# JinfengX/PointCloudPDF

Measured on AMD Instinct MI355X. Metric: points/sec fwd+bwd (PT-v1 Seg50 + PDF U-decoder, 100k-pt scenes), higher is better.
Workload: dtype f32

## Files before the change

include/pdfops.h:

```cpp
#ifndef PDFOPS_H
#define PDFOPS_H

#ifdef __cplusplus
extern "C" {
#endif

#define PDF_OK 0
#define PDF_ERR_BAD_ARG (-1)
#define PDF_ERR_NSAMPLE (-2)
#define PDF_ERR_UNSUPPORTED (-3)
#define PDF_ERR_NOT_CONVERGED (-4)

#define PDF_ABI_VERSION 18
int pdf_abi_version(void);
const char *pdf_build_info(void);
int pdf_dist_fma_mode(void);
#define PDF_MMA_F32 0
#define PDF_MMA_F16 1
#define PDF_MMA_BF16 2

int pdf_knn_query(int m, int nsample, const float *xyz, const float *new_xyz,
                  const int *offset, const int *new_offset, int b,
                  int *idx, float *dist2, void *stream);

long pdf_knn_workspace_bytes(int b, int n, int m);
int pdf_knn_grid_supported(int nsample);
int pdf_knn_query_ws(int m, int nsample, int n, const float *xyz, const float *new_xyz, const int *offset,
                     const int *new_offset, int b, int *idx, float *dist2, void *workspace, long workspace_bytes,
                     void *stream);
int pdf_knn_grid_build(int n, const float *xyz, const int *offset, int b, void *workspace, long workspace_bytes, void *stream);
int pdf_knn_query_grid(int m, int nsample, int n, const float *xyz, const float *new_xyz, const int *offset, const int *new_offset, int b,
                       int *idx, float *dist2, void *workspace, long workspace_bytes, void *stream);
int pdf_knn_query_ws_counted(int m, int nsample, int n, const float *xyz, const float *new_xyz, const int *offset,
                             const int *new_offset, int b, int *idx, float *dist2, void *workspace, long workspace_bytes,
                             unsigned long long *pairs, void *stream);
int pdf_knn_query_list(int m, int nsample, const float *xyz, const float *new_xyz, const int *offset,
                       const int *new_offset, int b, int *idx, float *dist2, const int *qlist, const int *qcount,
                       void *stream);

int pdf_ball_query(int m, int nsample, float min_radius, float max_radius, const float *xyz, const float *new_xyz,
                   const int *offset, const int *new_offset, int b, int *idx, float *dist2, void *stream);

int pdf_random_ball_query(int m, int nsample, float min_radius, float max_radius, const int *order, const float *xyz,
                          const float *new_xyz, const int *offset, const int *new_offset, int b, int *idx, float *dist2,
                          void *stream);

int pdf_farthest_point_sampling(int b, int n, const float *xyz, const int *offset,
                                const int *new_offset, float *tmp, int *idx, void *stream);

int pdf_fps_reference_block_log2(int n);

long pdf_fps_workspace_bytes(int b, int n_total);
long pdf_fps_stats_offset(int b, int n_total);
int pdf_farthest_point_sampling_bucketed(int b, int n, int n_total, const float *xyz, const int *offset,
                                         const int *new_offset, void *workspace, long workspace_bytes,
                                         int *idx, void *stream);

int pdf_grouping_forward(int m, int nsample, int c, const float *input, const int *idx, float *output, void *stream);
int pdf_grouping_backward(int m, int nsample, int c, const float *grad_output, const int *idx, float *grad_input, void *stream);
int pdf_grouping_forward_ordered(int m, int nsample, int c, const float *input, const int *idx, const int *order, float *output, void *stream);
int pdf_group_forward_ordered(int m, int nsample, int c, int with_xyz, const float *feat, const float *xyz, const float *new_xyz,
                              const int *idx, const int *order, float *output, void *stream);
int pdf_interpolation_forward_ordered(int n, int c, int k, const float *input, const int *idx, const float *weight, const int *order,
                                      float *output, void *stream);
int pdf_subtraction_forward_ordered(int n, int nsample, int c, const float *input1, const float *input2, const int *idx, const int *order,
                                    float *output, void *stream);
// ... 59 lines not shown
                       float *running_mean, float *running_var, int training, float eps, float momentum, int relu,
                       float *coef, float *partial, float *y, void *stream);
int pdf_bn_act_backward(long n, int c, const float *gy, const float *x, const float *res, const float *coef,
                        int training, int relu, float *partial, float *sums, float *gx, float *gres, void *stream);
int pdf_bn_coef(long n, int c, const float *x, const float *gamma, const float *beta, float *running_mean,
                float *running_var, int training, float eps, float momentum, float *coef, float *partial, void *stream);
int pdf_bn_apply(long n, int c, const float *x, const float *res, const float *coef, int relu, float *y, void *stream);

long pdf_rowlin_partial_floats(long n, int o);
int pdf_rowlin_partial_rows(long n, int k, int o);
int pdf_rowlin_forward(long n, int k, int o, const float *x, long ldx, const float *w, int transpose_w,
                       const float *bias, const float *scale, const float *shift, int relu, float *y, long ldy,
                       int accumulate, float *partial, int mma_input, void *stream);
long pdf_rowlin_wgrad_ws_floats(long n, int k, int o, int ng);
int pdf_rowlin_wgrad(long n, int k, int o, const float *g, long ldg, const float *x, long ldx,
                     const float *scale, const float *shift, int relu, float *dw, float *db, float *ws, int mma_input, void *stream);
int pdf_bn_coef_from_partial(const float *partial, int rows, long n, int c, const float *gamma, const float *beta,
                             float *running_mean, float *running_var, float eps, float momentum, float *coef, void *stream);

int pdf_rowlin_multi(long n, int k, int o, int nin, int nout, const float *const *x, long ldx, const float *const *w,
                     int transpose_w, const float *const *bias, const float *scale, const float *shift, int relu,
                     float *const *y, long ldy, int accumulate, int mma_input, void *stream);
int pdf_rowlin_wgrad_multi(long n, int k, int o, int ng, const float *const *g, long ldg, const float *x, long ldx,
                           const float *scale, const float *shift, int relu, float *const *dw, float *const *db, float *ws, int mma_input, void *stream);
int pdf_rowlin_wgrad_group(long n, int k, int o, int ng, const float *const *g, long ldg, const float *const *x, long ldx,
                           const float *const *scale, const float *const *shift, const int *relu, float *const *dw,
                           float *const *db, float *ws, int mma_input, void *stream);

int pdf_kpconv_supported(int kp, int cin);
int pdf_kpconv_gather(int n, int m, int kp, int cin, const float *query, const float *support, const int *neighbors, const float *x,
                      const float *k_points, float extent, float *weighted, void *stream);
int pdf_kpconv_scatter(int n, int m, int kp, int cin, const float *query, const float *support, const int *neighbors,
                       const float *grad_weighted, const float *k_points, float extent, float *grad_x, void *stream);
int pdf_rowlin_dgrad_bstats(long n, int k, int o, int nin, const float *const *x, long ldx, const float *const *w, float *y, long ldy,
                            const float *bx, long ldb, const float *bcoef, int brelu, float *partial, int *partial_rows,
                            int mma_input, void *stream);
int pdf_rowlin_forward_bn(long n, int k, int o, const float *x, long ldx, const float *w, const float *bias, const float *scale,
                          const float *shift, int relu, float *y, long ldy, float *partial, const float *gamma, const float *beta,
                          float *running_mean, float *running_var, float eps, float momentum, float *coef, int mma_input, void *stream);
int pdf_bn_act_backward_presummed(long n, int c, const float *gy, const float *x, const float *coef, int training, int relu,
                                  const float *partial, int partial_rows, float *sums, float *gx, void *stream);

int pdf_bn_coef_eval_or_partial(const float *partial, int rows, long n, int c, const float *gamma, const float *beta,
                                float *running_mean, float *running_var, int training, float eps, float momentum,
                                float *coef, void *stream);
int pdf_block_pre_forward(long n, int c, void *const *p, int training, float eps, float momentum, int mma_input, void *stream);
int pdf_block_pre_backward(long n, int c, void *const *p, int training, int mma_input, void *stream);
int pdf_block_post_forward(long n, int c, void *const *p, int training, float eps, float momentum, int mma_input, void *stream);
int pdf_block_post_backward(long n, int c, void *const *p, int training, int mma_input, void *stream);
int pdf_bottleneck_forward(long n, int nsample, int c, void *const *p, int training, float eps, float momentum, int storage_bf16, int mma_input, void *stream);
int pdf_bottleneck_backward(long n, int nsample, int c, void *const *p, int training, int entry_base, int storage_bf16, int mma_input, void *stream);
int pdf_linbn_forward(long n, int k, int o, void *const *p, int training, int relu, float eps, float momentum, int mma_input, void *stream);
int pdf_linbn_backward(long n, int k, int o, void *const *p, int training, int relu, int mma_input, void *stream);

int pdf_rowlin_forward_roww(long n, int k, int o, const float *x, long ldx, const float *w, int transpose_w, float *y, long ldy,
                            int accumulate, const float *roww, long rws, int mma_input, void *stream);
int pdf_rowlin_wgrad_roww(long n, int k, int o, const float *g, long ldg, const float *x, long ldx, float *dw, const float *roww,
                          long rws, float *ws, int mma_input, void *stream);
int pdf_bn_bwd_sums(long n, int c, const float *gy, const float *x, const float *coef, int relu, float *partial, float *sums,
                    void *stream);

int pdf_td_supported(int nsample, int cin, int cout);
int pdf_td_tables(long m, int b, const float *p_src, const float *p_new, const int *idx, const int *new_offset, float *rel4, float *Z,
                  float *scene_sums, long n, const int *inv_off, const int *inv_entry, int entry_base,
                  void *stream);
long pdf_td_gram_floats(int cin);
long pdf_td_fwd_scratch_floats(long n, int cin);
long pdf_td_bwd_scratch_floats(long m, int cin, int cout);
int pdf_td_forward(long n, long m, int cin, int cout, void *const *p, int training, float eps, float momentum, int mma_input, void *stream);
int pdf_td_backward(long n, long m, int cin, int cout, void *const *p, int entry_base, int mma_input, void *stream);

int pdf_seg_sum_rows(long n, int c, const float *src, const int *inv_off, const int *inv_entry, int entry_base, float scale, float *out,
                     void *stream);
int pdf_seg_sum_rows_own(long n, int c, int nsample, const float *src, const int *inv_off, const int *inv_entry, int entry_base, float scale,
                         const int *order, float *out, float *out_own, void *stream);
int pdf_seg_sum_rows_strided(long n, int c, const float *src, long src_stride, const int *inv_off, const int *inv_entry, int entry_base,
                             float scale, float *out, void *stream);
int pdf_seg_sum_rows_x(long n, int c, const float *src, long src_stride, int src_bf16, const int *inv_off, const int *inv_entry, int entry_base,
                       float scale, float *out, void *stream);
int pdf_seg_sum_weighted_x(long n, int c, int nsample, int w_c, const float *src, const float *w, int w_bf16, const int *inv_off,
                           const int *inv_entry, int entry_base, const int *order, float *out, void *stream);
int pdf_seg_sum_weighted_ordered(long n, int c, int nsample, int w_c, const float *src, const float *w, const int *inv_off,
                                 const int *inv_entry, int entry_base, const int *order, float *out, void *stream);
int pdf_seg_sum_weighted(long n, int c, int nsample, int w_c, const float *src, const float *w, const int *inv_off, const int *inv_entry,
                         int entry_base, float *out, void *stream);

long pdf_ce_workspace_floats(void);
int pdf_ce_forward(long n, int c, const float *logits, const long *target, long ignore, float *grad, float *acc, float *loss,
                   void *stream);
int pdf_ce_backward(long n, int c, const float *dlogits, const float *acc, const float *gy, float *grad_out, void *stream);

#define PDF_REDUCE_NONE 0
#define PDF_REDUCE_MEAN 1
#define PDF_REDUCE_SUM 2
long pdf_criteria_workspace_floats(int c);
int pdf_ce_ex_forward(long n, int c, const float *logits, const long *target, const float *weight, float label_smoothing, int reduction,
                      long ignore, float *grad, float *acc, float *loss, void *stream);
int pdf_ce_ex_backward(long n, int c, const float *dlogits, const float *acc, const float *gy, int reduction, float *grad_out, void *stream);
int pdf_focal_forward(long n, int c, const float *logits, const long *target, const float *alpha_vec, float alpha, float gamma, int reduction,
                      long ignore, float *grad, float *acc, float *loss, void *stream);
int pdf_focal_backward(long n, int c, const float *dlogits, const float *acc, const float *gy, float *grad_out, void *stream);
int pdf_dice_forward(long n, int c, const float *logits, const long *target, float smooth, float exponent, long ignore, float *prob,
                     float *acc, float *loss, void *stream);
int pdf_dice_backward(long n, int c, const float *prob, const long *target, long ignore, float exponent, const float *acc, const float *gy,
                      float *grad_out, void *stream);
int pdf_bfocal_forward(long n, const float *pred, const float *target, float alpha, float gamma, int logits, int reduce, float *grad,
// ... 289 lines not shown
```

pointcloudpdf_amd/_native.py:

```python
import ctypes
import os
import threading

import torch

_HERE = os.path.dirname(os.path.abspath(__file__))
DIST_FMA = int(os.environ.get("PDFOPS_DIST_FMA", "0") or 0)
if DIST_FMA not in (0, 1, 2):
    raise RuntimeError(f"PDFOPS_DIST_FMA={DIST_FMA}: expected 0 (as written), 1 or 2 (csrc/pdfops_common.h)")


def library_path(dist_fma=0):
    return os.path.join(_HERE, "lib", "libpdfops.so" if not dist_fma else f"libpdfops_fma{int(dist_fma)}.so")


LIB_PATH = library_path(DIST_FMA)
ABI_VERSION = 18

c_int = ctypes.c_int
c_long = ctypes.c_long
c_void_p = ctypes.c_void_p
c_float = ctypes.c_float
c_double = ctypes.c_double

_PROTOS = {
    "knn_query": "iippppipp",
    "ball_query": "iiffppppipp",
    "random_ball_query": "iiffpppppipp",
    "farthest_point_sampling": "iippppp",
    "grouping_forward": "iiippp",
    "grouping_backward": "iiippp",
    "interpolation_forward": "iiipppp",
    "interpolation_backward": "iiipppp",
    "subtraction_forward": "iiipppp",
    "subtraction_backward": "iiipppp",
    "aggregation_forward": "iiiippppp",
    "aggregation_backward": "iiiipppppppp",
    "attention_relation_step_forward": "iiipppppp",
    "attention_relation_step_backward": "iiippppppppp",
    "attention_fusion_step_forward": "iiippppp",
    "attention_fusion_step_backward": "iiippppppp",
    "attention_step1_forward_v2": "iiiiippppp",
    "attention_step1_backward_v2": "iiiiippppppp",
    "dot_prod_with_idx_forward_v3": "iiiiipppppppp",
    "dot_prod_with_idx_backward_v3": "iiiiipppppppppppp",
    "attention_step2_with_rel_pos_value_forward_v2": "iiiiippppppp",
    "attention_step2_with_rel_pos_value_backward_v2": "iiiiipppppppppp",
    "segment_softmax_forward": "iiippp",
    "segment_softmax_backward": "iiipppp",
}
_HIP_ONLY_PROTOS = {
    "grid_hash": "lippdddippp",
    "grid_hash_f64": "lippdddppp",
    "philox4x64": "llllp",
    "aug_bounds": "ippppp",
    "aug_points": "ilpipppppp",
    "aug_keys": "ilpplp",
    "aug_elastic_noise": "ilpplp",
    "aug_elastic_blur": "ilpppi",
    "aug_elastic_apply": "ilpppppdpp",
    "radius_neighbors_self": "iifppipppl",
    "radius_neighbors_self_adaptive": "iiffppippppl",
    "vote_accumulate": "lipppppp",
    "fragment_bounds": "lliiipppppp",
    "fragment_gather": "lliiipppppipppppppp",
    "fragment_vote": "lliiippppppppp",
    "graph_forest": "lipppppipppl",
    "gmm2_1d": "ipppidd",
    "dot_prod_with_idx_forward_v3_l": "iiiiipppppppp",
    "dot_prod_with_idx_backward_v3_l": "iiiiipppppppppppp",
# ... 612 lines not shown
        lib.pdf_spconv_wgrad_ws_floats.argtypes = [c_long, c_int, c_int, c_int]
        lib.pdf_spconv_colsum_ws_floats.restype = c_long
        lib.pdf_spconv_colsum_ws_floats.argtypes = [c_int]
        lib.pdf_incr_kl_workspace_floats.restype = c_long
        lib.pdf_incr_kl_workspace_floats.argtypes = []
        lib.pdf_incr_kl_forward.restype = c_int
        lib.pdf_incr_kl_forward.argtypes = [c_long, c_int, c_int, c_void_p, c_void_p, c_void_p, c_long, ctypes.c_float, ctypes.c_float,
                                            c_void_p, c_void_p, c_void_p, c_void_p]
        lib.pdf_incr_kl_backward.restype = c_int
        lib.pdf_incr_kl_backward.argtypes = [c_long, c_int, c_void_p, c_void_p, c_void_p, c_void_p, c_void_p]
        lib.pdf_lovasz_workspace_bytes.restype = c_long
        lib.pdf_lovasz_workspace_bytes.argtypes = [c_long, c_int]
        lib.pdf_lovasz_forward.restype = c_int
        lib.pdf_lovasz_forward.argtypes = [c_long, c_int, c_void_p, c_void_p, c_long, c_void_p, c_void_p, c_void_p, c_void_p, c_void_p, c_void_p]
        lib.pdf_lovasz_backward.restype = c_int
        lib.pdf_lovasz_backward.argtypes = [c_long, c_int, c_void_p, c_void_p, ctypes.c_float, c_void_p, c_void_p]
        lib.pdf_openset_metrics_workspace_bytes.restype = c_long
        lib.pdf_openset_metrics_workspace_bytes.argtypes = [c_long, c_int]
        lib.pdf_openset_metrics.restype = c_int
        lib.pdf_openset_metrics.argtypes = [c_long, c_int, c_void_p, c_void_p, c_void_p, c_void_p, c_long, c_void_p, c_int, c_void_p, c_void_p,
                                            c_void_p, c_void_p]
        lib.pdf_knn_rel_moments.restype = c_int
        lib.pdf_knn_rel_moments.argtypes = [c_int, c_long, c_int, c_void_p, c_void_p, c_void_p, c_void_p, c_void_p, c_void_p]
        lib.pdf_knn_rel_moments_ws_doubles.restype = c_long
        lib.pdf_knn_rel_moments_ws_doubles.argtypes = [c_int, c_long]
        lib.pdf_knn_rel_moments_q.restype = c_int
        lib.pdf_knn_rel_moments_q.argtypes = [c_int, c_long, c_int, c_void_p, c_void_p, c_void_p, c_void_p, c_void_p, c_void_p, c_void_p]
        class CopySeg(ctypes.Structure):
            _fields_ = [("src", c_void_p), ("dst", c_void_p), ("nbytes", c_long), ("src_offset", c_void_p), ("sub", c_void_p),
                        ("sub_const", c_int), ("src_elems", c_int)]

        self.CopySeg = CopySeg
        lib.pdf_stage_copy.restype = c_int
        lib.pdf_stage_copy.argtypes = [c_int, c_void_p, c_void_p]
        lib.pdf_scene_morton_keys.restype = c_int
        lib.pdf_scene_morton_keys.argtypes = [c_long, c_int, c_void_p, c_void_p, c_void_p, c_void_p, c_void_p]
        lib.pdf_sgd_chunk.restype = c_int
        lib.pdf_sgd_chunk.argtypes = []
        lib.pdf_sgd_step.restype = c_int
        lib.pdf_sgd_step.argtypes = [c_int, c_void_p, c_void_p, ctypes.c_float, ctypes.c_float, ctypes.c_float, c_void_p, c_void_p]
        lib.pdf_grad_unscale.restype = c_int
        lib.pdf_grad_unscale.argtypes = [c_int, c_void_p, c_void_p, c_void_p, c_void_p, c_void_p]
        lib.pdf_scaler_update.restype = c_int
        lib.pdf_scaler_update.argtypes = [c_void_p, c_void_p, c_void_p, c_void_p, ctypes.c_float, ctypes.c_float, c_int, c_void_p]
        lib.pdf_adam_step.restype = c_int
        lib.pdf_adam_step.argtypes = [c_int, c_int, c_void_p, c_void_p, ctypes.c_double, ctypes.c_double, ctypes.c_double, ctypes.c_double,
                                      ctypes.c_double, c_int, c_void_p, c_void_p]
        lib.pdf_adam_grad_unscale.restype = c_int
        lib.pdf_adam_grad_unscale.argtypes = [c_int, c_void_p, c_void_p, c_void_p, c_void_p, c_void_p]
        lib.pdf_linbn_forward.restype = c_int
        lib.pdf_linbn_forward.argtypes = [c_long, c_int, c_int, c_void_p, c_int, c_int, ctypes.c_float, ctypes.c_float, c_int, c_void_p]
        lib.pdf_linbn_backward.restype = c_int
        lib.pdf_linbn_backward.argtypes = [c_long, c_int, c_int, c_void_p, c_int, c_int, c_int, c_void_p]
        lib.pdf_bottleneck_forward.restype = c_int
        lib.pdf_bottleneck_forward.argtypes = [c_long, c_int, c_int, c_void_p, c_int, ctypes.c_float, ctypes.c_float, c_int, c_int, c_void_p]
        lib.pdf_bottleneck_backward.restype = c_int
        lib.pdf_bottleneck_backward.argtypes = [c_long, c_int, c_int, c_void_p, c_int, c_int, c_int, c_int, c_void_p]
        for nm in ("pre_backward", "post_backward"):
            f = getattr(lib, "pdf_block_" + nm)
            f.restype = c_int
            f.argtypes = [c_long, c_int, c_void_p, c_int, c_int, c_void_p]
        lib.pdf_rowlin_multi.restype = c_int
        lib.pdf_rowlin_multi.argtypes = [c_long, c_int, c_int, c_int, c_int, c_void_p, c_long, c_void_p, c_int, c_void_p, c_void_p, c_void_p,
                                         c_int, c_void_p, c_long, c_int, c_int, c_void_p]
        lib.pdf_kpconv_supported.restype = c_int
        lib.pdf_kpconv_supported.argtypes = [c_int, c_int]
        for nm in ("pdf_kpconv_gather", "pdf_kpconv_scatter"):
            f = getattr(lib, nm)
            f.restype = c_int
            f.argtypes = [c_int, c_int, c_int, c_int, c_void_p, c_void_p, c_void_p, c_void_p, c_void_p, ctypes.c_float, c_void_p, c_void_p]
        lib.pdf_rowlin_wgrad_group.restype = c_int
        lib.pdf_rowlin_wgrad_group.argtypes = [c_long, c_int, c_int, c_int, c_void_p, c_long, c_void_p, c_long, c_void_p, c_void_p, c_void_p,
                                               c_void_p, c_void_p, c_void_p, c_int, c_void_p]
        lib.pdf_rowlin_wgrad_multi.restype = c_int
        lib.pdf_rowlin_wgrad_multi.argtypes = [c_long, c_int, c_int, c_int, c_void_p, c_long, c_void_p, c_long, c_void_p, c_void_p, c_int,
                                               c_void_p, c_void_p, c_void_p, c_int, c_void_p]
        lib.pdf_rowlin_wgrad_ws_floats.restype = c_long
        lib.pdf_rowlin_wgrad_ws_floats.argtypes = [c_long, c_int, c_int, c_int]
        lib.pdf_rowlin_dgrad_bstats.restype = c_int
        lib.pdf_rowlin_dgrad_bstats.argtypes = [c_long, c_int, c_int, c_int, c_void_p, c_long, c_void_p, c_void_p, c_long, c_void_p, c_long,
                                                c_void_p, c_int, c_void_p, ctypes.POINTER(c_int), c_int, c_void_p]
        lib.pdf_bn_act_backward_presummed.restype = c_int
        lib.pdf_bn_act_backward_presummed.argtypes = [c_long, c_int, c_void_p, c_void_p, c_void_p, c_int, c_int, c_void_p, c_int, c_void_p,
                                                      c_void_p, c_void_p]
        lib.pdf_rowlin_partial_floats.restype = c_long
        lib.pdf_rowlin_partial_floats.argtypes = [c_long, c_int]
        lib.pdf_rowlin_partial_rows.restype = c_int
        lib.pdf_rowlin_partial_rows.argtypes = [c_long, c_int, c_int]
        lib.pdf_rowlin_forward.restype = c_int
        lib.pdf_rowlin_forward.argtypes = [c_long, c_int, c_int, c_void_p, c_long, c_void_p, c_int, c_void_p, c_void_p, c_void_p,
                                           c_int, c_void_p, c_long, c_int, c_void_p, c_int, c_void_p]
        lib.pdf_rowlin_wgrad.restype = c_int
        lib.pdf_rowlin_wgrad.argtypes = [c_long, c_int, c_int, c_void_p, c_long, c_void_p, c_long, c_void_p, c_void_p, c_int,
                                         c_void_p, c_void_p, c_void_p, c_int, c_void_p]
        lib.pdf_bn_coef_from_partial.restype = c_int
        lib.pdf_bn_coef_from_partial.argtypes = [c_void_p, c_int, c_long, c_int, c_void_p, c_void_p, c_void_p, c_void_p,
                                                 ctypes.c_float, ctypes.c_float, c_void_p, c_void_p]
        lib.pdf_bn_coef.restype = c_int
        lib.pdf_bn_coef.argtypes = [c_long, c_int, c_void_p, c_void_p, c_void_p, c_void_p, c_void_p, c_int, ctypes.c_float,
                                    ctypes.c_float, c_void_p, c_void_p, c_void_p]
        lib.pdf_bn_apply.restype = c_int
        lib.pdf_bn_apply.argtypes = [c_long, c_int, c_void_p, c_void_p, c_void_p, c_int, c_void_p, c_void_p]
        lib.pdf_bn_supported.restype = c_int
        lib.pdf_bn_supported.argtypes = [c_int]
        lib.pdf_bn_partial_floats.restype = c_long
        lib.pdf_bn_partial_floats.argtypes = [c_long, c_int]
# ... 1695 lines not shown
```

pointcloudpdf_amd/csrc/block.hip:

```cpp
#include "pdfops_common.h"

namespace {
struct Err {
    int rc = 0;
    Err &operator<<(int r) { if (rc == 0 && r != 0) rc = r; return *this; }
};

}

extern "C" int pdf_bn_coef_eval_or_partial(const float *partial, int rows, long n, int c, const float *gamma, const float *beta,
                                           float *running_mean, float *running_var, int training, float eps, float momentum,
                                           float *coef, void *stream) {
    if (training) return pdf_bn_coef_from_partial(partial, rows, n, c, gamma, beta, running_mean, running_var, eps, momentum, coef, stream);
    return pdf_bn_coef(n, c, nullptr, gamma, beta, running_mean, running_var, 0, eps, momentum, coef, nullptr, stream);
}

extern "C" int pdf_block_pre_forward(long n, int c, void *const *p, int training, float eps, float momentum, int mma_input, void *stream) {
    if (n < 1 || !p) return PDF_ERR_BAD_ARG;
    if (!pdf_bn_supported(c)) return PDF_ERR_UNSUPPORTED;
    const float *x = (const float *)p[0], *W1 = (const float *)p[1], *g1 = (const float *)p[2], *b1 = (const float *)p[3];
    float *rm1 = (float *)p[4], *rv1 = (float *)p[5];
    float *z1 = (float *)p[12], *coef1 = (float *)p[13], *partial = (float *)p[17];
    Err e;
    if (training) {
        e << pdf_rowlin_forward_bn(n, c, c, x, c, W1, nullptr, nullptr, nullptr, 0, z1, c, partial, g1, b1, rm1, rv1, eps, momentum, coef1, mma_input, stream);
    } else {
        e << pdf_rowlin_forward(n, c, c, x, c, W1, 0, nullptr, nullptr, nullptr, 0, z1, c, 0, nullptr, mma_input, stream);
        e << pdf_bn_coef_eval_or_partial(partial, 0, n, c, g1, b1, rm1, rv1, 0, eps, momentum, coef1, stream);
    }
    const float *xs[1] = {z1}, *ws[3] = {(const float *)p[6], (const float *)p[8], (const float *)p[10]};
    const float *bs[3] = {(const float *)p[7], (const float *)p[9], (const float *)p[11]};
    float *ys[3] = {(float *)p[14], (float *)p[15], (float *)p[16]};
    e << pdf_rowlin_multi(n, c, c, 1, 3, xs, c, ws, 0, bs, coef1, coef1 + c, 1, ys, c, 0, mma_input, stream);
    return e.rc;
}

static bool inkernel_bn() {
    static const bool on = [] { const char *v = getenv("PDFOPS_INKERNEL_BN"); return !(v && v[0] == '0'); }();
    return on;
}
static bool dgrad_bstats() {
    static const bool on = [] { const char *v = getenv("PDFOPS_DGRAD_BSTATS"); return !(v && v[0] == '0'); }();
    return on;
}

static int block_pre_backward(long n, int c, void *const *p, int training, int accumulate_gx, int mma_input, void *stream, bool defer_wgrad = false) {
    if (n < 1 || !p || !p[14]) return PDF_ERR_BAD_ARG;
    const float *x = (const float *)p[0], *z1 = (const float *)p[1], *coef1 = (const float *)p[2], *W1 = (const float *)p[3];
    float *gx = (float *)p[10], *grads = (float *)p[11], *dy = (float *)p[12], *partial = (float *)p[13], *wslab = (float *)p[14];
    const long cc = (long)c * c;
    float *dW1 = grads, *db1 = grads + cc, *dqkv = db1 + 2 * c;
    Err e;
    const float *gs[3] = {(const float *)p[7], (const float *)p[8], (const float *)p[9]};
// ... 121 lines not shown
                               (float *)p[40], (float *)p[32], storage_bf16, (const int *)p[49], (const double *)p[46], stream);
    void *pre[15] = {p[1], p[2], p[3], p[4], p[5], p[6], p[7], p[35], p[36], p[37], p[29], p[30], p[45], p[40], ws_pre};
    e << block_pre_backward(n, c, pre, training, 1, mma_input, stream, group);
    if (group && e.rc == 0) {
        const long cc = (long)c * c;
        float *gpre = (float *)p[30], *gpost = (float *)p[31];
        float *dW1 = gpre, *dqkv = gpre + cc + 2 * c, *dW3 = gpost;
        const float *coef1 = (const float *)p[3], *coef2 = (const float *)p[26];
        const float *g[5] = {(const float *)p[34], (const float *)p[35], (const float *)p[36], (const float *)p[37], (const float *)p[45]};
        const float *x[5] = {(const float *)p[24], (const float *)p[2], (const float *)p[2], (const float *)p[2], (const float *)p[1]};
        const float *sc[5] = {coef2, coef1, coef1, coef1, nullptr}, *sh[5] = {coef2 + c, coef1 + c, coef1 + c, coef1 + c, nullptr};
        const int relu[5] = {1, 1, 1, 1, 0};
        float *dw[5] = {dW3, dqkv, dqkv + (cc + c), dqkv + 2 * (cc + c), dW1};
        float *db[5] = {nullptr, dqkv + cc, dqkv + (cc + c) + cc, dqkv + 2 * (cc + c) + cc, nullptr};
        const int rc = pdf_rowlin_wgrad_group(n, c, c, 5, g, c, x, c, sc, sh, relu, dw, db, ws_post, mma_input, stream);
        if (rc == PDF_ERR_UNSUPPORTED) {
            e << pdf_rowlin_wgrad(n, c, c, g[0], c, x[0], c, sc[0], sh[0], 1, dw[0], nullptr, ws_post, mma_input, stream);
            e << pdf_rowlin_wgrad_multi(n, c, c, 3, g + 1, c, x[1], c, sc[1], sh[1], 1, dw + 1, db + 1, ws_pre, mma_input, stream);
            e << pdf_rowlin_wgrad(n, c, c, g[4], c, x[4], c, nullptr, nullptr, 0, dw[4], nullptr, ws_pre, mma_input, stream);
        } else {
            e << rc;
        }
    }
    return e.rc;
}

extern "C" int pdf_linbn_forward(long n, int k, int o, void *const *p, int training, int relu, float eps, float momentum, int mma_input, void *stream) {
    if (n < 1 || !p) return PDF_ERR_BAD_ARG;
    if (!pdf_bn_supported(o)) return PDF_ERR_UNSUPPORTED;
    Err e;
    float *z = (float *)p[7], *coef = (float *)p[8], *partial = (float *)p[10];
    if (training) {
        e << pdf_rowlin_forward_bn(n, k, o, (const float *)p[0], k, (const float *)p[1], (const float *)p[2], nullptr, nullptr, 0, z, o, partial,
                                   (const float *)p[3], (const float *)p[4], (float *)p[5], (float *)p[6], eps, momentum, coef, mma_input, stream);
    } else {
        e << pdf_rowlin_forward(n, k, o, (const float *)p[0], k, (const float *)p[1], 0, (const float *)p[2], nullptr, nullptr, 0, z, o, 0, nullptr, mma_input, stream);
        e << pdf_bn_coef_eval_or_partial(partial, 0, n, o, (const float *)p[3], (const float *)p[4], (float *)p[5], (float *)p[6], 0, eps, momentum, coef, stream);
    }
    e << pdf_bn_apply(n, o, z, nullptr, coef, relu, (float *)p[9], stream);
    return e.rc;
}

extern "C" int pdf_linbn_backward(long n, int k, int o, void *const *p, int training, int relu, int mma_input, void *stream) {
    if (n < 1 || !p || !p[9]) return PDF_ERR_BAD_ARG;
    float *grads = (float *)p[6], *gz = (float *)p[7];
    const long ok = (long)o * k;
    Err e;
    e << pdf_bn_act_backward(n, o, (const float *)p[0], (const float *)p[2], nullptr, (const float *)p[3], training, relu, (float *)p[8],
                             grads + ok + o, gz, nullptr, stream);
    if (p[5]) e << pdf_rowlin_forward(n, o, k, gz, o, (const float *)p[4], 1, nullptr, nullptr, nullptr, 0, (float *)p[5], k, 0, nullptr, mma_input, stream);
    e << pdf_rowlin_wgrad(n, k, o, gz, o, (const float *)p[1], k, nullptr, nullptr, 0, grads, grads + ok, (float *)p[9], mma_input, stream);
    return e.rc;
}
```

pointcloudpdf_amd/csrc/fused_layer.hip:

```cpp
#include "fused_layer.h"
#include <algorithm>
#include <cstdlib>

namespace fl {

__host__ __device__ constexpr int tile_stride(int c) { return c / 8 > 32 ? 65 : 33; }
__host__ __device__ constexpr int aux_stride(int c) { return c / 8 <= 16 ? 17 : c / 8 + 1; }
constexpr int MAX_BLOCKS = 512;
static inline int env_blocks(const char *name, int dflt) {
    const char *v = getenv(name);
    const int x = v ? atoi(v) : 0;
    return x > 0 ? x : dflt;
}

struct WaveLds {
    float *tile;
    float *qtile;
    int *rowid;
    float *aux;
    int ts, as;
};

__device__ __forceinline__ void stage_rows(const WaveLds &L, const float *__restrict__ table, int C, int c0, int lane) {
    const int sub = lane >> 3, col = (lane & 7) * 4;
// ... 752 lines not shown
        const Row R = load_row<K>(A, tile, lane);
        if (!R.valid) continue;
        const float *g3 = A.G3 + (size_t)R.row * 3;
#pragma unroll
        for (int a = 0; a < 3; ++a) {
            const float that = (R.t1[a] - A.mean[a]) * A.rstd[a];
            const float gt1 = A.sp[a] * (g3[a] - A.sums[a] * A.inv_rows - that * A.sums[3 + a] * A.inv_rows);
            acc[a] += gt1;
#pragma unroll
            for (int b = 0; b < 3; ++b) acc[3 + a * 3 + b] += gt1 * R.rel[b];
        }
    }
    __shared__ float stage[WPB * 16];
    block_row(stage, 16, [&](RowAcc o) {
#pragma unroll
        for (int e = 0; e < 12; ++e) {
            const float v = pdf_wave_sum_f32(acc[e]);
            if (lane == 0) o[e] = v;
        }
        if (lane == 0) { o[12] = 0.f; o[13] = 0.f; o[14] = 0.f; o[15] = 0.f; }
    });
    store_row(stage, b4_width(), A.partial + (size_t)blockIdx.x * b4_width());
}

constexpr int RED_RL = 16, RED_THREADS = 16 * RED_RL, RED_B = 16;
__device__ __forceinline__ double strided_sum(const float *__restrict__ src, size_t stride, int rl, int rows) {
    double s0 = 0.0, s1 = 0.0, s2 = 0.0, s3 = 0.0;
    for (int r = rl; r < rows; r += RED_B * RED_RL) {
        float v[RED_B];
#pragma unroll
        for (int t = 0; t < RED_B; ++t) v[t] = src[(size_t)min(r + t * RED_RL, rows - 1) * stride];
#pragma unroll
        for (int t = 0; t < RED_B; ++t) v[t] = (r + t * RED_RL < rows) ? v[t] : 0.f;
#pragma unroll
        for (int t = 0; t < RED_B; t += 4) { s0 += (double)v[t]; s1 += (double)v[t + 1]; s2 += (double)v[t + 2]; s3 += (double)v[t + 3]; }
    }
    return (s0 + s1) + (s2 + s3);
}

__device__ __forceinline__ double wave_rows_sum(double v) {
    v += __shfl_xor(v, 16, 64);
    v += __shfl_xor(v, 32, 64);
    return v;
}
constexpr int RED_WAVES = RED_THREADS / 64;

struct BnpClosed {
    const double *mom;
    cfloat_p Wp1, bp1, sp, mean, rstd;
    double rows;
    int col_g;
    float *out4;
};
__global__ __launch_bounds__(RED_THREADS) void k_colsum(const float *__restrict__ partial, int rows, int width, int stride, float *__restrict__ out,
                                                        BnpClosed bc) {
    __shared__ double red[RED_WAVES][17];
    if (blockIdx.x * 16 >= (unsigned)width) {
        __shared__ double col[16];
        const int cl = threadIdx.x & 15, rl = threadIdx.x >> 4;
        const int c = cl < 6 ? cl : bc.col_g + (cl - 6);
        const double v = wave_rows_sum(cl < 15 ? strided_sum(partial + c, (size_t)stride, rl, rows) : 0.0);
        if ((threadIdx.x & 63) < 16) red[threadIdx.x >> 6][cl] = v;
        __syncthreads();
        if (threadIdx.x < 16) {
            double s = 0.0;
#pragma unroll
            for (int k = 0; k < RED_WAVES; ++k) s += red[k][threadIdx.x];
            col[threadIdx.x] = s;
        }
        __syncthreads();
        if (threadIdx.x < 12) {
            const double S[3] = {bc.mom[0], bc.mom[1], bc.mom[2]};
            const double M[3][3] = {{bc.mom[3], bc.mom[4], bc.mom[5]}, {bc.mom[4], bc.mom[6], bc.mom[7]}, {bc.mom[5], bc.mom[7], bc.mom[8]}};
            const int a = threadIdx.x < 3 ? (int)threadIdx.x : ((int)threadIdx.x - 3) / 3, b = threadIdx.x < 3 ? 0 : ((int)threadIdx.x - 3) % 3;
            const double w[3] = {(double)bc.Wp1[a * 3], (double)bc.Wp1[a * 3 + 1], (double)bc.Wp1[a * 3 + 2]};
            const double d = (double)bc.bp1[a] - (double)bc.mean[a], rs = (double)bc.rstd[a], sp = (double)bc.sp[a], R = bc.rows;
            const double s_a = col[a], u_a = col[3 + a];
            double r;
            if (threadIdx.x < 3) {
                const double sum_that = rs * (w[0] * S[0] + w[1] * S[1] + w[2] * S[2] + R * d);
                r = sp * (-(u_a / R) * sum_that);
            } else {
                const double T = rs * (w[0] * M[0][b] + w[1] * M[1][b] + w[2] * M[2][b] + d * S[b]);
                r = sp * (col[6 + 3 * a + b] - s_a * S[b] / R - u_a * T / R);
            }
            bc.out4[threadIdx.x] = (float)r;
        } else if (threadIdx.x < 16) {
            bc.out4[threadIdx.x] = 0.f;
        }
        return;
    }
    const int cl = threadIdx.x & 15, rl = threadIdx.x >> 4;
    const int col = blockIdx.x * 16 + cl;
    const double v = wave_rows_sum(col < width ? strided_sum(partial + col, (size_t)stride, rl, rows) : 0.0);
    if ((threadIdx.x & 63) < 16) red[threadIdx.x >> 6][cl] = v;
    __syncthreads();
    if (rl != 0 || col >= width) return;
    double s = 0.0;
#pragma unroll
    for (int k = 0; k < RED_WAVES; ++k) s += red[k][cl];
    out[col] = (float)s;
}

__global__ __launch_bounds__(RED_THREADS) void k_bn_finalize(const float *__restrict__ partial, int rows, int nch, double count,
                              const float *__restrict__ gamma, const float *__restrict__ beta, float eps, float momentum,
                              float *__restrict__ running_mean, float *__restrict__ running_var,
                              float *__restrict__ scale, float *__restrict__ shift, float *__restrict__ mean_out,
                              float *__restrict__ rstd_out) {
    __shared__ double red[2][RED_WAVES][17];
    const int cl = threadIdx.x & 15, rl = threadIdx.x >> 4;
    const int ch = blockIdx.x * 16 + cl;
    const double a = wave_rows_sum(ch < nch ? strided_sum(partial + ch, 2 * (size_t)nch, rl, rows) : 0.0);
    const double b = wave_rows_sum(ch < nch ? strided_sum(partial + nch + ch, 2 * (size_t)nch, rl, rows) : 0.0);
    if ((threadIdx.x & 63) < 16) { red[0][threadIdx.x >> 6][cl] = a; red[1][threadIdx.x >> 6][cl] = b; }
    __syncthreads();
    if (rl != 0 || ch >= nch) return;
    double s = 0.0, ss = 0.0;
#pragma unroll
    for (int k = 0; k < RED_WAVES; ++k) { s += red[0][k][cl]; ss += red[1][k][cl]; }
    const double mean = s / count;
    double var = ss / count - mean * mean;
    if (var < 0.0) var = 0.0;
    const float rstd = (float)(1.0 / sqrt(var + (double)eps));
    const float sc = gamma[ch] * rstd;
    scale[ch] = sc;
    shift[ch] = beta[ch] - (float)mean * sc;
    mean_out[ch] = (float)mean;
    rstd_out[ch] = rstd;
    if (running_mean) {
        const double unbiased = count > 1.0 ? var * count / (count - 1.0) : var;
        running_mean[ch] = (1.f - momentum) * running_mean[ch] + momentum * (float)mean;
        running_var[ch] = (1.f - momentum) * running_var[ch] + momentum * (float)unbiased;
    }
}

__global__ void k_bn_eval(int nch, const float *__restrict__ gamma, const float *__restrict__ beta, float eps,
                          const float *__restrict__ running_mean, const float *__restrict__ running_var,
                          float *__restrict__ scale, float *__restrict__ shift, float *__restrict__ mean_out,
                          float *__restrict__ rstd_out) {
    const int ch = blockIdx.x * blockDim.x + threadIdx.x;
    if (ch >= nch) return;
    const float rstd = 1.0f / sqrtf(running_var[ch] + eps);
    const float sc = gamma[ch] * rstd;
    scale[ch] = sc;
    shift[ch] = beta[ch] - running_mean[ch] * sc;
    if (mean_out) { mean_out[ch] = running_mean[ch]; rstd_out[ch] = rstd; }
}

void launch_bn_finalize(const float *partial, int rows, int nch, double count, const float *gamma, const float *beta, float eps,
                        float momentum, float *running_mean, float *running_var, float *scale, float *shift, float *mean_out,
                        float *rstd_out, hipStream_t s) {
    k_bn_finalize<<<pdf_divup(nch, 16), RED_THREADS, 0, s>>>(partial, rows, nch, count, gamma, beta, eps, momentum, running_mean, running_var,
                                                     scale, shift, mean_out, rstd_out);
}
void launch_bn_eval(int nch, const float *gamma, const float *beta, float eps, const float *running_mean, const float *running_var,
                    float *scale, float *shift, float *mean_out, float *rstd_out, hipStream_t s) {
    k_bn_eval<<<pdf_divup(nch, 64), 64, 0, s>>>(nch, gamma, beta, eps, running_mean, running_var, scale, shift, mean_out, rstd_out);
}
void launch_colsum(const float *partial, int rows, int width, float *out, hipStream_t s) {
    BnpClosed none;
    none.mom = nullptr; none.out4 = nullptr; none.rows = 0.0; none.col_g = 0;
    none.Wp1 = none.bp1 = none.sp = none.mean = none.rstd = as_const(nullptr);
    k_colsum<<<pdf_divup(width, 16), RED_THREADS, 0, s>>>(partial, rows, width, width, out, none);
}

template <typename KernelT>
static inline void allow_lds(KernelT kernel, size_t lds) {
    if (lds > 64 * 1024) (void)hipFuncSetAttribute(reinterpret_cast<const void *>(kernel), hipFuncAttributeMaxDynamicSharedMemorySize, (int)lds);
}

static inline int grid_for_points(long n, int cap) {
    static const int env_cap = env_blocks("PDFOPS_PT_BLOCKS_MFMA", 0);
    if (env_cap > 0) cap = env_cap;
    long g = (n + WPB - 1) / WPB;
    if (g > cap) g = cap;
    if (g < 1) g = 1;
    return (int)g;
}

enum Pass { P3 = 0, B1 = 1, B2 = 2, B3 = 3, P2 = 4 };
static inline int pass_grid(Pass pass, long n, int dflt_cap) {
    static const int env_cap[5] = {env_blocks("PDFOPS_PT_CAP_P3", 0), env_blocks("PDFOPS_PT_CAP_B1", 0), env_blocks("PDFOPS_PT_CAP_B2", 0),
                                   env_blocks("PDFOPS_PT_CAP_B3", 0), env_blocks("PDFOPS_PT_CAP_P2", 0)};
    return grid_for_points(n, env_cap[pass] > 0 ? env_cap[pass] : dflt_cap);
}

static inline int grid_for_tiles(long ntiles) {
    static const int cap = env_blocks("PDFOPS_PT_BLOCKS_FWD", MAX_BLOCKS);
    long g = (ntiles + WPB - 1) / WPB;
    if (g > cap) g = cap;
    if (g < 1) g = 1;
    return (int)g;
}

}

extern "C" long pdf_pt_layer_partial_floats(int n, int nsample, int c) {
    const long ntiles = ((long)n * nsample + 63) / 64;
    const int g = flm::supported(nsample, c) ? fl::grid_for_points(n, fl::MAX_BLOCKS) : fl::grid_for_tiles(ntiles);
    return (long)g * fl::WPB * 2 * (c > 3 ? c : 3);
}

extern "C" int pdf_pt_layer_supported(int nsample, int c) {
    return ((nsample == 8 || nsample == 16) && (c == 32 || c == 64 || c == 128)) || (nsample == 16 && c == 256) ||
           (c == 512 && flm::supported(nsample, c));
}

namespace fl {

template <int C, int K>
int forward_impl(LayerArgs A, int training, float eps, float momentum, const float *const *bn_params, float *const *bn_buffers,
                 float *bn, float *saved, int *out_stat_rows, hipStream_t s) {
    constexpr int CS = C / 8;
    const long rows = (long)A.N * K;
    const long ntiles = (rows + 63) / 64;
    const int grid = flm::supported(K, C) ? grid_for_points(A.N, MAX_BLOCKS) : grid_for_tiles(ntiles);
// ... 222 lines not shown
```

pointcloudpdf_amd/csrc/gather_ops.hip:

```cpp
#include "pdfops_common.h"

namespace {

constexpr int GB = 256;

template <int V> struct VecT;
template <> struct VecT<1> { using type = float; };
template <> struct VecT<2> { using type = float2; };
template <> struct VecT<4> { using type = float4; };

template <int V> __device__ __forceinline__ typename VecT<V>::type vzero();
template <> __device__ __forceinline__ float vzero<1>() { return 0.f; }
template <> __device__ __forceinline__ float2 vzero<2>() { return make_float2(0.f, 0.f); }
template <> __device__ __forceinline__ float4 vzero<4>() { return make_float4(0.f, 0.f, 0.f, 0.f); }

__device__ __forceinline__ float vget(const float &v, int) { return v; }
__device__ __forceinline__ float vget(const float2 &v, int i) { return i == 0 ? v.x : v.y; }
__device__ __forceinline__ float vget(const float4 &v, int i) { return i == 0 ? v.x : i == 1 ? v.y : i == 2 ? v.z : v.w; }
__device__ __forceinline__ void vset(float &v, int, float x) { v = x; }
__device__ __forceinline__ void vset(float2 &v, int i, float x) { if (i == 0) v.x = x; else v.y = x; }
__device__ __forceinline__ void vset(float4 &v, int i, float x) {
    if (i == 0) v.x = x; else if (i == 1) v.y = x; else if (i == 2) v.z = x; else v.w = x;
}

// ... 288 lines not shown
#pragma unroll
    for (int u = 0; u < U; ++u) v[u] = input[(unsigned long)max(src[u], 0) * cv + col[u]];
#pragma unroll
    for (int u = 0; u < U; ++u)
        if (live[u]) st_stream(output + dst[u], src[u] >= 0 ? v[u] : (v4f)(0.f));
}

template <int U>
__global__ __launch_bounds__(GB) void sub_fwd_ord(unsigned total, FastDiv cvd, FastDiv rowd, int nsample, const int *__restrict__ order,
                                                  const v4f *__restrict__ input1, const v4f *__restrict__ input2,
                                                  const int *__restrict__ idx, v4f *__restrict__ output) {
    const unsigned cv = cvd.d, blk = xcd_chunked_block(blockIdx.x, gridDim.x);
    const unsigned w0 = blk * (GB * U) + threadIdx.x;
    v4f a[U], b[U];
    unsigned long dst[U], row[U];
    unsigned col[U], sq[U], jn[U], q[U];
    int src[U];
    bool live[U];
#pragma unroll
    for (int u = 0; u < U; ++u) {
        const unsigned w = w0 + u * GB;
        live[u] = w < total;
        sq[u] = fdiv(live[u] ? w : 0u, rowd);
        const unsigned rem = (live[u] ? w : 0u) - sq[u] * rowd.d;
        jn[u] = fdiv(rem, cvd); col[u] = rem - jn[u] * cv;
    }
#pragma unroll
    for (int u = 0; u < U; ++u) { q[u] = order ? (unsigned)order[sq[u]] : sq[u]; row[u] = (unsigned long)q[u] * nsample + jn[u]; }
#pragma unroll
    for (int u = 0; u < U; ++u) { src[u] = idx[row[u]]; dst[u] = row[u] * cv + col[u]; a[u] = input1[(unsigned long)q[u] * cv + col[u]]; }
#pragma unroll
    for (int u = 0; u < U; ++u) b[u] = input2[(unsigned long)max(src[u], 0) * cv + col[u]];
#pragma unroll
    for (int u = 0; u < U; ++u)
        if (live[u]) st_stream(output + dst[u], a[u] - (src[u] >= 0 ? b[u] : (v4f)(0.f)));
}

template <int K>
__global__ __launch_bounds__(GB) void interp_fwd_ord(unsigned total, FastDiv cvd, const int *__restrict__ order, const v4f *__restrict__ input,
                                                     const int *__restrict__ idx, const float *__restrict__ weight, v4f *__restrict__ output) {
    const unsigned cv = cvd.d, blk = xcd_chunked_block(blockIdx.x, gridDim.x);
    const unsigned w = blk * GB + threadIdx.x;
    if (w >= total) return;
    const unsigned sq = fdiv(w, cvd), col = w - sq * cv, r = order ? (unsigned)order[sq] : sq;
    int j[K]; float wt[K]; v4f v[K];
#pragma unroll
    for (int i = 0; i < K; ++i) { j[i] = idx[(unsigned long)r * K + i]; wt[i] = weight[(unsigned long)r * K + i]; }
#pragma unroll
    for (int i = 0; i < K; ++i) v[i] = input[(unsigned long)max(j[i], 0) * cv + col];
    v4f acc = (v4f)(0.f);
#pragma unroll
    for (int i = 0; i < K; ++i) acc += (j[i] >= 0 ? v[i] : (v4f)(0.f)) * wt[i];
    st_stream(output + (unsigned long)r * cv + col, acc);
}

__global__ __launch_bounds__(GB) void agg_fwd_ord(unsigned total, FastDiv cvd, int nsample, unsigned wv, const int *__restrict__ order,
                                                  const v4f *__restrict__ input, const v4f *__restrict__ position,
                                                  const v4f *__restrict__ weight, const int *__restrict__ idx, v4f *__restrict__ output) {
    const unsigned cv = cvd.d, blk = xcd_chunked_block(blockIdx.x, gridDim.x);
    const unsigned w = blk * GB + threadIdx.x;
    if (w >= total) return;
    const unsigned sq = fdiv(w, cvd), col = w - sq * cv, wcol = col % wv, r = order ? (unsigned)order[sq] : sq;
    v4f acc = (v4f)(0.f);
    const unsigned long base = (unsigned long)r * nsample;
    int s = 0;
    for (; s + 4 <= nsample; s += 4) {
        int j[4]; v4f in[4], pos[4], wt[4];
#pragma unroll
        for (int t = 0; t < 4; ++t) j[t] = idx[base + s + t];
#pragma unroll
        for (int t = 0; t < 4; ++t) {
            in[t] = input[(unsigned long)max(j[t], 0) * cv + col];
            pos[t] = __builtin_nontemporal_load(position + (base + s + t) * cv + col);
            wt[t] = weight[(base + s + t) * wv + wcol];
        }
#pragma unroll
        for (int t = 0; t < 4; ++t) acc += ((j[t] >= 0 ? in[t] : (v4f)(0.f)) + pos[t]) * wt[t];
    }
    for (; s < nsample; ++s) {
        const int j = idx[base + s];
        const v4f in = input[(unsigned long)max(j, 0) * cv + col];
        acc += ((j >= 0 ? in : (v4f)(0.f)) + __builtin_nontemporal_load(position + (base + s) * cv + col)) * weight[(base + s) * wv + wcol];
    }
    output[(unsigned long)r * cv + col] = acc;
}

template <int U>
__global__ __launch_bounds__(GB) void group_fwd_rows_ord(unsigned total, FastDiv pd, FastDiv nsd, FastDiv qd , int c,
                                                         int with_xyz, const int *__restrict__ order, const float *__restrict__ feat,
                                                         const float *__restrict__ xyz, const float *__restrict__ new_xyz,
                                                         const int *__restrict__ idx, float *__restrict__ output) {
    typedef float u4f __attribute__((ext_vector_type(4), aligned(4)));
    const unsigned pieces = pd.d, cv = c >> 2, oc = c + (with_xyz ? 3 : 0), sh = with_xyz ? 3u : 0u;
    const unsigned blk = xcd_chunked_block(blockIdx.x, gridDim.x);
    const unsigned w0 = blk * (GB * U) + threadIdx.x;
    v4f v[U];
    float *o[U];
    unsigned q[U], m[U], sq[U], jn[U];
    unsigned long r[U];
    int j[U];
    float dx[U][3];
    bool live[U];
#pragma unroll
    for (int u = 0; u < U; ++u) {
        const unsigned w = w0 + u * GB;
        live[u] = w < total;
// ... 317 lines not shown
                                                                            c, order, feat, xyz, new_xyz, idx, output);
        else group_fwd_lds<4, 4><<<(m + ppb - 1) / ppb, GB, lds, s>>>((unsigned)m, ppb, mk_fastdiv((unsigned)nsample), mk_fastdiv((unsigned)(nsample * oc / 4)), c,
                                                                    order, feat, xyz, new_xyz, idx, output);
        return pdf_launch_status();
    }
    if (c % 4 == 0 && rows * (c / 4 + 1) < (1L << 31)) {
        const unsigned pieces = (unsigned)(c / 4 + (with_xyz ? 1 : 0)), total = (unsigned)(rows * pieces);
        constexpr int U = 4;
        group_fwd_rows_ord<U><<<(total + GB * U - 1) / (GB * U), GB, 0, s>>>(total, mk_fastdiv(pieces), mk_fastdiv(nsample), mk_fastdiv(nsample * pieces),
                                                                           c, with_xyz, order, feat, xyz, new_xyz, idx, output);
        return pdf_launch_status();
    }
    if (rows * oc < (1L << 31)) {
        const unsigned total = (unsigned)(rows * oc), total4 = (total + 3) / 4;
        group_fwd32<<<grid_for(total4), GB, 0, s>>>(total4, total, mk_fastdiv(oc), mk_fastdiv(nsample), c, with_xyz, feat, xyz, new_xyz, idx, output);
        return pdf_launch_status();
    }
    group_fwd_kernel<<<grid_for(rows * oc), GB, 0, s>>>(rows, nsample, c, with_xyz, feat, xyz, new_xyz, idx, output);
    return pdf_launch_status();
}

extern "C" int pdf_group_forward(int m, int nsample, int c, int with_xyz, const float *feat, const float *xyz,
                                 const float *new_xyz, const int *idx, float *output, void *stream) {
    return pdf_group_forward_ordered(m, nsample, c, with_xyz, feat, xyz, new_xyz, idx, nullptr, output, stream);
}

extern "C" int pdf_group_backward(int m, int nsample, int c, int with_xyz, const float *grad_output, const int *idx,
                                  float *grad_feat, void *stream) {
    if (m == 0) return PDF_OK;
    if (m < 0 || nsample < 1 || c < 1 || !grad_output || !idx || !grad_feat) return PDF_ERR_BAD_ARG;
    hipStream_t s = static_cast<hipStream_t>(stream);
    const long rows = (long)m * nsample;
    group_bwd_kernel<<<grid_for(rows * c), GB, 0, s>>>(rows, c, with_xyz, grad_output, idx, grad_feat);
    return pdf_launch_status();
}

extern "C" int pdf_interpolation_forward_ordered(int n, int c, int k, const float *input, const int *idx, const float *weight, const int *order,
                                                 float *output, void *stream) {
    if (n == 0) return PDF_OK;
    if (n < 0 || c < 1 || k < 1 || !input || !idx || !weight || !output) return PDF_ERR_BAD_ARG;
    hipStream_t s = static_cast<hipStream_t>(stream);
    const int v = pick_vec(c);
    if (v == 4 && (long)n * (c / 4) < (1L << 31) && (long)n * k < (1L << 31)) {
        const unsigned total = (unsigned)((long)n * (c / 4));
        const FastDiv cvd = mk_fastdiv(c / 4);
        if (k == 3) interp_fwd_ord<3><<<(total + GB - 1) / GB, GB, 0, s>>>(total, cvd, order, (const v4f *)input, idx, weight, (v4f *)output);
        else interp_fwd32<0><<<grid_for(total), GB, 0, s>>>(total, cvd, k, (const v4f *)input, idx, weight, (v4f *)output);
        return pdf_launch_status();
    }
    DISPATCH_VEC(v, (interp_fwd_kernel<V><<<grid_for((long)n * (c / V)), GB, 0, s>>>(n, c / V, k, input, idx, weight, output)));
    return pdf_launch_status();
}

extern "C" int pdf_interpolation_forward(int n, int c, int k, const float *input, const int *idx, const float *weight, float *output, void *stream) {
    return pdf_interpolation_forward_ordered(n, c, k, input, idx, weight, nullptr, output, stream);
}

extern "C" int pdf_interpolation_backward(int n, int c, int k, const float *grad_output, const int *idx, const float *weight, float *grad_input, void *stream) {
    if (n == 0) return PDF_OK;
    if (n < 0 || c < 1 || k < 1 || !grad_output || !idx || !weight || !grad_input) return PDF_ERR_BAD_ARG;
    hipStream_t s = static_cast<hipStream_t>(stream);
    const int v = 1;
    DISPATCH_VEC(v, (interp_bwd_kernel<V><<<grid_for((long)n * (c / V)), GB, 0, s>>>(n, c / V, k, grad_output, idx, weight, grad_input)));
    return pdf_launch_status();
}

extern "C" int pdf_interpolation_weights(int n, int k, const float *dist2, float *weight, void *stream) {
    if (n == 0) return PDF_OK;
    if (n < 0 || k < 1 || !dist2 || !weight) return PDF_ERR_BAD_ARG;
    hipStream_t s = static_cast<hipStream_t>(stream);
    interp_weights_kernel<<<grid_for(n), GB, 0, s>>>(n, k, dist2, weight);
    return pdf_launch_status();
}

extern "C" int pdf_subtraction_forward_ordered(int n, int nsample, int c, const float *input1, const float *input2, const int *idx,
                                               const int *order, float *output, void *stream) {
    if (n == 0) return PDF_OK;
    if (n < 0 || nsample < 1 || c < 1 || !input1 || !input2 || !idx || !output) return PDF_ERR_BAD_ARG;
    hipStream_t s = static_cast<hipStream_t>(stream);
    const int v = pick_vec(c);
    const long rows = (long)n * nsample;
    if (v == 4 && rows * (c / 4) < (1L << 31)) {
        constexpr int U = 4;
        const unsigned total = (unsigned)(rows * (c / 4));
        sub_fwd_ord<U><<<(total + GB * U - 1) / (GB * U), GB, 0, s>>>(total, mk_fastdiv(c / 4), mk_fastdiv((unsigned)nsample * (c / 4)), nsample, order,
                                                                     (const v4f *)input1, (const v4f *)input2, idx, (v4f *)output);
        return pdf_launch_status();
    }
    DISPATCH_VEC(v, (sub_fwd_kernel<V><<<grid_for(rows * (c / V)), GB, 0, s>>>(rows, nsample, c / V, input1, input2, idx, output)));
    return pdf_launch_status();
}

extern "C" int pdf_subtraction_forward(int n, int nsample, int c, const float *input1, const float *input2, const int *idx, float *output, void *stream) {
    return pdf_subtraction_forward_ordered(n, nsample, c, input1, input2, idx, nullptr, output, stream);
}

extern "C" int pdf_subtraction_backward(int n, int nsample, int c, const int *idx, const float *grad_output, float *grad_input1, float *grad_input2, void *stream) {
    if (n == 0) return PDF_OK;
    if (n < 0 || nsample < 1 || c < 1 || !idx || !grad_output || !grad_input1) return PDF_ERR_BAD_ARG;
    hipStream_t s = static_cast<hipStream_t>(stream);
    const int v = grad_input2 ? 1 : pick_vec(c);
    DISPATCH_VEC(v, (sub_bwd_kernel<V><<<grid_for((long)n * (c / V)), GB, 0, s>>>(n, nsample, c / V, idx, grad_output, grad_input1, grad_input2)));
    return pdf_launch_status();
}

extern "C" int pdf_aggregation_forward_ordered(int n, int nsample, int c, int w_c, const float *input, const float *position,
// ... 45 lines not shown
```

pointcloudpdf_amd/csrc/pdfops_common.h:

```cpp
#pragma once
#include <hip/hip_runtime.h>
#include <stdint.h>
#include <atomic>
#include "../../include/pdfops.h"

#define PDF_WAVE 64
#define PDF_MAX_DEVICES_LDS 64

static inline int pdf_launch_status() {
    hipError_t e = hipGetLastError();
    return e == hipSuccess ? PDF_OK : (int)e;
}

struct PdfLdsLimit { std::atomic<int> state[PDF_MAX_DEVICES_LDS]; };
static inline bool pdf_lds_limit_raised(PdfLdsLimit &site, const void *kernel, int bytes) {
    int dev = 0;
    if (hipGetDevice(&dev) != hipSuccess || dev < 0 || dev >= PDF_MAX_DEVICES_LDS) return hipFuncSetAttribute(kernel, hipFuncAttributeMaxDynamicSharedMemorySize, bytes) == hipSuccess;
    int st = site.state[dev].load(std::memory_order_acquire);
    if (st == 0) {
        st = hipFuncSetAttribute(kernel, hipFuncAttributeMaxDynamicSharedMemorySize, bytes) == hipSuccess ? 1 : 2;
        if (st == 2) (void)hipGetLastError();
        site.state[dev].store(st, std::memory_order_release);
    }
    return st == 1;
// ... 39 lines not shown
        v = w > v ? w : v;
    }
    return v;
}
__device__ __forceinline__ float pdf_wave_sum_f32(float v) {
#pragma unroll
    for (int o = 32; o >= 1; o >>= 1) v += __shfl_xor(v, o, 64);
    return v;
}

#ifndef PDF_DIST_FMA
#define PDF_DIST_FMA 0
#endif
__host__ __device__ __forceinline__ float pdf_sqdist3(float dx, float dy, float dz) {
#if PDF_DIST_FMA == 1
    return __builtin_fmaf(dz, dz, __builtin_fmaf(dy, dy, dx * dx));
#elif PDF_DIST_FMA == 2
    return __builtin_fmaf(dz, dz, __builtin_fmaf(dx, dx, dy * dy));
#else
    return dx * dx + dy * dy + dz * dz;
#endif
}

__device__ __forceinline__ unsigned pdf_f32_ordered(float f) {
    unsigned u = __float_as_uint(f);
    return (u & 0x80000000u) ? ~u : (u | 0x80000000u);
}

__device__ __forceinline__ void pdf_atomic_add(float *p, float v) {
    __hip_atomic_fetch_add(p, v, __ATOMIC_RELAXED, __HIP_MEMORY_SCOPE_AGENT);
}

#define PDF_XCDS 8
__device__ __forceinline__ unsigned pdf_xcd_chunked_block(unsigned b, unsigned g) {
    const unsigned q = g / PDF_XCDS, r = g % PDF_XCDS, x = b % PDF_XCDS;
    return (x < r ? x * (q + 1) : r * (q + 1) + (x - r) * q) + b / PDF_XCDS;
}

struct PdfRowsBn {
    const float *rows; int nrows; int c; double count;
    const float *gamma, *beta; float *running_mean, *running_var; float eps, momentum;
    float *coef;
    unsigned long long *gran;
    unsigned *sync;
};
#define PDF_HO_WORDS(c) (2 * (size_t)(c) * 2 + 4)
#define PDF_HO_FLOATS PDF_HO_WORDS(1024)
int pdf_rowlin_forward_stats_ho(long n, int k, int o, const float *x, long ldx, const float *w, const float *bias, const float *scale,
                                const float *shift, int relu, float *y, long ldy, float *rows_out, void *handoff, int *rows, int mma_input,
                                void *stream);
int pdf_bn_apply_rows(long n, int c, const float *x, const float *res, const float *rows, int nrows, const float *gamma, const float *beta,
                      float *running_mean, float *running_var, float eps, float momentum, float *coef, void *handoff, int relu, float *y,
                      void *stream);

__device__ __forceinline__ void pdf_handoff_zero(unsigned long long *gran, int c, unsigned *sync) {
    for (int e = threadIdx.x; e < 2 * c; e += blockDim.x) gran[e] = 0ull;
    if (threadIdx.x == 0) sync[0] = 0u;
}

template <int NT>
__device__ __forceinline__ void pdf_bn_reduce_slice(const PdfRowsBn &b, int sl, double *lds_red) {
    constexpr int RL = NT / 16;
    const int c = b.c, cl = threadIdx.x & 15, rl = threadIdx.x >> 4;
    const int ch = sl * 16 + cl;
    double s = 0.0, ss = 0.0;
    if (ch < c) {
        const float *p0 = b.rows + ch, *p1 = b.rows + c + ch;
        const size_t stride = 2 * (size_t)c;
        for (int r = rl; r < b.nrows; r += 8 * RL) {
            float v0[8], v1[8];
#pragma unroll
            for (int t = 0; t < 8; ++t) {
                const int rr = r + t * RL < b.nrows ? r + t * RL : b.nrows - 1;
                v0[t] = p0[(size_t)rr * stride]; v1[t] = p1[(size_t)rr * stride];
            }
#pragma unroll
            for (int t = 0; t < 8; ++t) {
                const bool ok = r + t * RL < b.nrows;
                s += ok ? (double)v0[t] : 0.0; ss += ok ? (double)v1[t] : 0.0;
            }
        }
    }
    __syncthreads();
    lds_red[(0 * RL + rl) * 17 + cl] = s;
    lds_red[(1 * RL + rl) * 17 + cl] = ss;
    __syncthreads();
    if (rl == 0 && ch < c) {
        double a = 0.0, q = 0.0;
        for (int k = 0; k < RL; ++k) { a += lds_red[(0 * RL + k) * 17 + cl]; q += lds_red[(1 * RL + k) * 17 + cl]; }
        const double mean = a / b.count;
        double var = q / b.count - mean * mean;
        if (var < 0.0) var = 0.0;
        const float rstd = (float)(1.0 / sqrt(var + (double)b.eps));
        const float sc = b.gamma[ch] * rstd, sh = b.beta[ch] - (float)mean * sc;
        b.coef[ch] = sc; b.coef[c + ch] = sh; b.coef[2 * c + ch] = (float)mean; b.coef[3 * c + ch] = rstd;
        if (b.running_mean && b.sync != nullptr) {
            const double unbiased = b.count > 1.0 ? var * b.count / (b.count - 1.0) : var;
            b.running_mean[ch] = (1.f - b.momentum) * b.running_mean[ch] + b.momentum * (float)mean;
            b.running_var[ch] = (1.f - b.momentum) * b.running_var[ch] + b.momentum * (float)unbiased;
        }
        __hip_atomic_store(b.gran + ch, (1ull << 32) | (unsigned long long)__float_as_uint(sc), __ATOMIC_RELAXED, __HIP_MEMORY_SCOPE_AGENT);
        __hip_atomic_store(b.gran + c + ch, (1ull << 32) | (unsigned long long)__float_as_uint(sh), __ATOMIC_RELAXED, __HIP_MEMORY_SCOPE_AGENT);
    }
}

template <int NT>
// ... 22 lines not shown
```

pointcloudpdf_amd/csrc/pointwise.hip:

```cpp
#include "pdfops_common.h"
#include <cstdlib>

namespace pw {

constexpr int PB = 256;
constexpr int MAXB = 1024;

static inline int grid_rows(long n, int c) {
    const long rows_per_block = (long)PB * 4 / c > 0 ? (long)PB * 4 / c : 1;
    static const int short_rows = [] { const char *v = getenv("PDFOPS_BN_ROWS_SHORT"); const int x = v ? atoi(v) : 0; return x > 0 ? x : 4; }();
    const long per = n * c >= (1L << 22) ? 8 : short_rows;
    long g = (n + rows_per_block * per - 1) / (rows_per_block * per);
    if (g > MAXB) g = MAXB;
    if (g < 1) g = 1;
    return (int)g;
}

__global__ __launch_bounds__(PB) void k_bn_stats(long n, int c, const float *__restrict__ x, float *partial) {
    extern __shared__ float red[];
    const int tpr = c / 4;
    const int rpb = PB / tpr;
    const int tr = threadIdx.x / tpr, tc = threadIdx.x % tpr;
    float s[4] = {0.f, 0.f, 0.f, 0.f}, ss[4] = {0.f, 0.f, 0.f, 0.f};
    if (tr < rpb) {
// ... 1 lines not shown
            const float4 v = *reinterpret_cast<const float4 *>(x + r * c + tc * 4);
            s[0] += v.x; s[1] += v.y; s[2] += v.z; s[3] += v.w;
            ss[0] += v.x * v.x; ss[1] += v.y * v.y; ss[2] += v.z * v.z; ss[3] += v.w * v.w;
        }
    }
#pragma unroll
    for (int k = 0; k < 4; ++k) { red[threadIdx.x * 8 + k] = s[k]; red[threadIdx.x * 8 + 4 + k] = ss[k]; }
    __syncthreads();
    if (threadIdx.x < tpr) {
#pragma unroll
        for (int k = 0; k < 8; ++k) {
            float a = 0.f;
            for (int rr = 0; rr < rpb; ++rr) a += red[(rr * tpr + threadIdx.x) * 8 + k];
            const int ch = threadIdx.x * 4 + (k & 3);
            partial[(size_t)blockIdx.x * 2 * c + (k < 4 ? ch : c + ch)] = a;
        }
    }
}

template <bool RES>
__global__ __launch_bounds__(PB) void k_bn_apply(long n4, int c4, const float4 *__restrict__ x, const float4 *__restrict__ scale,
                                                 const float4 *__restrict__ shift, const float4 *__restrict__ res, int relu,
                                                 float4 *__restrict__ y) {
    for (long e = (long)blockIdx.x * PB + threadIdx.x; e < n4; e += (long)gridDim.x * PB) {
        const int cc = (int)(e % c4);
        const float4 v = x[e], sc = scale[cc], sh = shift[cc];
        const float4 r = RES ? res[e] : make_float4(0.f, 0.f, 0.f, 0.f);
        float4 o = make_float4(v.x * sc.x + sh.x + r.x, v.y * sc.y + sh.y + r.y, v.z * sc.z + sh.z + r.z, v.w * sc.w + sh.w + r.w);
        if (relu) { o.x = fmaxf(o.x, 0.f); o.y = fmaxf(o.y, 0.f); o.z = fmaxf(o.z, 0.f); o.w = fmaxf(o.w, 0.f); }
        y[e] = o;
    }
}

template <bool RES>
__global__ __launch_bounds__(PB) void k_bn_apply_rows(long n4, int c4, const float4 *__restrict__ x, PdfRowsBn b, const float4 *__restrict__ res,
                                                      int relu, float4 *__restrict__ y) {
    extern __shared__ __attribute__((aligned(16))) float lds[];
    const int c = 4 * c4;
    double *red = reinterpret_cast<double *>(lds + 2 * c);
    unsigned *word = reinterpret_cast<unsigned *>(red + 2 * (PB / 16) * 17);
    pdf_bn_coef_inkernel<PB>(b, lds, red, word);
    const float4 *scale = reinterpret_cast<const float4 *>(lds), *shift = reinterpret_cast<const float4 *>(lds + c);
    for (long e = (long)blockIdx.x * PB + threadIdx.x; e < n4; e += (long)gridDim.x * PB) {
        const int cc = (int)(e % c4);
        const float4 v = x[e], sc = scale[cc], sh = shift[cc];
        const float4 r = RES ? res[e] : make_float4(0.f, 0.f, 0.f, 0.f);
        float4 o = make_float4(v.x * sc.x + sh.x + r.x, v.y * sc.y + sh.y + r.y, v.z * sc.z + sh.z + r.z, v.w * sc.w + sh.w + r.w);
        if (relu) { o.x = fmaxf(o.x, 0.f); o.y = fmaxf(o.y, 0.f); o.z = fmaxf(o.z, 0.f); o.w = fmaxf(o.w, 0.f); }
        y[e] = o;
    }
}

template <bool RES>
__global__ __launch_bounds__(PB) void k_bn_bwd_reduce(long n, int c, const float *__restrict__ gy, const float *__restrict__ x,
                                                      const float *__restrict__ res, const float *__restrict__ scale,
                                                      const float *__restrict__ shift, const float *__restrict__ mean,
                                                      const float *__restrict__ rstd, int relu, float *partial) {
    extern __shared__ float red[];
    const int tpr = c / 4, rpb = PB / tpr;
    const int tr = threadIdx.x / tpr, tc = threadIdx.x % tpr;
    float s[4] = {0.f, 0.f, 0.f, 0.f}, sx[4] = {0.f, 0.f, 0.f, 0.f};
    if (tr < rpb) {
        float sc[4], sh[4], mu[4], rs[4];
#pragma unroll
        for (int k = 0; k < 4; ++k) { sc[k] = scale[tc * 4 + k]; sh[k] = shift[tc * 4 + k]; mu[k] = mean[tc * 4 + k]; rs[k] = rstd[tc * 4 + k]; }
        for (long r = (long)blockIdx.x * rpb + tr; r < n; r += (long)gridDim.x * rpb) {
            const float4 g4 = *reinterpret_cast<const float4 *>(gy + r * c + tc * 4);
            const float4 x4 = *reinterpret_cast<const float4 *>(x + r * c + tc * 4);
            const float4 r4 = RES ? *reinterpret_cast<const float4 *>(res + r * c + tc * 4) : make_float4(0.f, 0.f, 0.f, 0.f);
            const float g[4] = {g4.x, g4.y, g4.z, g4.w}, xv[4] = {x4.x, x4.y, x4.z, x4.w}, rv[4] = {r4.x, r4.y, r4.z, r4.w};
#pragma unroll
            for (int k = 0; k < 4; ++k) {
                const float pre = xv[k] * sc[k] + sh[k] + rv[k];
                const float gm = (!relu || pre > 0.f) ? g[k] : 0.f;
                s[k] += gm;
                sx[k] += gm * ((xv[k] - mu[k]) * rs[k]);
            }
        }
    }
#pragma unroll
    for (int k = 0; k < 4; ++k) { red[threadIdx.x * 8 + k] = s[k]; red[threadIdx.x * 8 + 4 + k] = sx[k]; }
    __syncthreads();
    if (threadIdx.x < tpr) {
#pragma unroll
        for (int k = 0; k < 8; ++k) {
            float a = 0.f;
            for (int rr = 0; rr < rpb; ++rr) a += red[(rr * tpr + threadIdx.x) * 8 + k];
            const int ch = threadIdx.x * 4 + (k & 3);
            partial[(size_t)blockIdx.x * 2 * c + (k < 4 ? ch : c + ch)] = a;
        }
    }
}

template <bool RES>
__global__ __launch_bounds__(PB) void k_bn_bwd_apply(long n4, int c4, const float4 *__restrict__ gy, const float4 *__restrict__ x,
                                                     const float4 *__restrict__ res, const float4 *__restrict__ scale,
                                                     const float4 *__restrict__ shift, const float4 *__restrict__ mean,
                                                     const float4 *__restrict__ rstd, const float4 *__restrict__ sums, float inv_n,
                                                     int relu, float4 *__restrict__ gx, float4 *__restrict__ gres) {
    for (long e = (long)blockIdx.x * PB + threadIdx.x; e < n4; e += (long)gridDim.x * PB) {
        const int cc = (int)(e % c4);
        const float4 g4 = gy[e], x4 = x[e], sc = scale[cc], sh = shift[cc], mu = mean[cc], rs = rstd[cc];
        const float4 s1 = sums[cc], s2 = sums[c4 + cc];
        const float4 r4 = RES ? res[e] : make_float4(0.f, 0.f, 0.f, 0.f);
        float4 gm, o;
#define PW_ONE(f)                                                                     \
        {                                                                             \
            const float pre = x4.f * sc.f + sh.f + r4.f;                              \
            gm.f = (!relu || pre > 0.f) ? g4.f : 0.f;                                 \
            const float xh = (x4.f - mu.f) * rs.f;                                    \
            o.f = sc.f * (gm.f - s1.f * inv_n - xh * s2.f * inv_n);                   \
        }
        PW_ONE(x) PW_ONE(y) PW_ONE(z) PW_ONE(w)
#undef PW_ONE
        gx[e] = o;
        if (gres) gres[e] = gm;
    }
}

template <bool RES>
__global__ __launch_bounds__(PB) void k_bn_bwd_eval(long n4, int c4, const float4 *__restrict__ gy, const float4 *__restrict__ x,
                                                    const float4 *__restrict__ res, const float4 *__restrict__ scale,
                                                    const float4 *__restrict__ shift, int relu, float4 *__restrict__ gx,
                                                    float4 *__restrict__ gres) {
    for (long e = (long)blockIdx.x * PB + threadIdx.x; e < n4; e += (long)gridDim.x * PB) {
        const int cc = (int)(e % c4);
        const float4 g4 = gy[e], x4 = x[e], sc = scale[cc], sh = shift[cc];
        const float4 r4 = RES ? res[e] : make_float4(0.f, 0.f, 0.f, 0.f);
        float4 gm;
        gm.x = (!relu || x4.x * sc.x + sh.x + r4.x > 0.f) ? g4.x : 0.f;
        gm.y = (!relu || x4.y * sc.y + sh.y + r4.y > 0.f) ? g4.y : 0.f;
        gm.z = (!relu || x4.z * sc.z + sh.z + r4.z > 0.f) ? g4.z : 0.f;
        gm.w = (!relu || x4.w * sc.w + sh.w + r4.w > 0.f) ? g4.w : 0.f;
        gx[e] = make_float4(gm.x * sc.x, gm.y * sc.y, gm.z * sc.z, gm.w * sc.w);
        if (gres) gres[e] = gm;
    }
}

static inline int grid_elems(long n4) {
    long g = (n4 + PB - 1) / PB;
    if (g > 2048) g = 2048;
    if (g < 1) g = 1;
    return (int)g;
}

}

namespace fl {
void launch_bn_finalize(const float *partial, int rows, int nch, double count, const float *gamma, const float *beta, float eps,
                        float momentum, float *running_mean, float *running_var, float *scale, float *shift, float *mean_out,
                        float *rstd_out, hipStream_t s);
void launch_bn_eval(int nch, const float *gamma, const float *beta, float eps, const float *running_mean, const float *running_var,
                    float *scale, float *shift, float *mean_out, float *rstd_out, hipStream_t s);
void launch_colsum(const float *partial, int rows, int width, float *out, hipStream_t s);
}

extern "C" int pdf_bn_supported(int c) { return c >= 4 && c % 4 == 0 && c <= 1024 && (1024 % c == 0); }
extern "C" long pdf_bn_partial_floats(long n, int c) { return (long)pw::grid_rows(n, c) * 2 * c + (long)PDF_HO_FLOATS; }

extern "C" int pdf_bn_act_forward(long n, int c, const float *x, const float *res, const float *gamma, const float *beta,
                                  float *running_mean, float *running_var, int training, float eps, float momentum,
                                  int relu, float *coef, float *partial, float *y, void *stream) {
    if (n < 1 || !x || !gamma || !beta || !coef || !y) return PDF_ERR_BAD_ARG;
    if (!pdf_bn_supported(c)) return PDF_ERR_UNSUPPORTED;
    hipStream_t s = static_cast<hipStream_t>(stream);
    float *scale = coef, *shift = coef + c, *mean = coef + 2 * c, *rstd = coef + 3 * c;
    if (training) {
        if (!partial) return PDF_ERR_BAD_ARG;
        const int g = pw::grid_rows(n, c);
        pw::k_bn_stats<<<g, pw::PB, pw::PB * 8 * sizeof(float), s>>>(n, c, x, partial);
// ... 6 lines not shown
    (res ? pw::k_bn_apply<true> : pw::k_bn_apply<false>)<<<pw::grid_elems(n4), pw::PB, 0, s>>>(n4, c / 4, reinterpret_cast<const float4 *>(x),
                                                        reinterpret_cast<const float4 *>(scale), reinterpret_cast<const float4 *>(shift),
                                                        reinterpret_cast<const float4 *>(res), relu, reinterpret_cast<float4 *>(y));
    return pdf_launch_status();
}

static int bn_act_backward(long n, int c, const float *gy, const float *x, const float *res, const float *coef,
                           int training, int relu, float *partial, float *sums, int sums_zeroed, float *gx, float *gres, void *stream,
                           int presummed = 0) {
    (void)sums_zeroed;
    if (n < 1 || !gy || !x || !coef || !partial || !sums || !gx) return PDF_ERR_BAD_ARG;
    if (!pdf_bn_supported(c)) return PDF_ERR_UNSUPPORTED;
    hipStream_t s = static_cast<hipStream_t>(stream);
    const float *scale = coef, *shift = coef + c, *mean = coef + 2 * c, *rstd = coef + 3 * c;
    const int g = pw::grid_rows(n, c);
    const long n4 = n * (c / 4);
    if (presummed > 0) {
        fl::launch_colsum(partial, presummed, 2 * c, sums, s);
    } else {
        (res ? pw::k_bn_bwd_reduce<true> : pw::k_bn_bwd_reduce<false>)<<<g, pw::PB, pw::PB * 8 * sizeof(float), s>>>(
            n, c, gy, x, res, scale, shift, mean, rstd, relu, partial);
        fl::launch_colsum(partial, g, 2 * c, sums, s);
    }
#define F4(p) reinterpret_cast<const float4 *>(p)
    if (training)
        (res ? pw::k_bn_bwd_apply<true> : pw::k_bn_bwd_apply<false>)<<<pw::grid_elems(n4), pw::PB, 0, s>>>(n4, c / 4, F4(gy), F4(x), F4(res), F4(scale), F4(shift), F4(mean), F4(rstd),
                                                                F4(sums), (float)(1.0 / (double)n), relu, reinterpret_cast<float4 *>(gx),
                                                                reinterpret_cast<float4 *>(gres));
    else
        (res ? pw::k_bn_bwd_eval<true> : pw::k_bn_bwd_eval<false>)<<<pw::grid_elems(n4), pw::PB, 0, s>>>(n4, c / 4, F4(gy), F4(x), F4(res), F4(scale), F4(shift), relu,
                                                               reinterpret_cast<float4 *>(gx), reinterpret_cast<float4 *>(gres));
#undef F4
    return pdf_launch_status();
}

extern "C" int pdf_bn_act_backward(long n, int c, const float *gy, const float *x, const float *res, const float *coef,
                                   int training, int relu, float *partial, float *sums, float *gx, float *gres, void *stream) {
    return bn_act_backward(n, c, gy, x, res, coef, training, relu, partial, sums, 0, gx, gres, stream);
}
extern "C" int pdf_bn_act_backward_presummed(long n, int c, const float *gy, const float *x, const float *coef, int training, int relu,
                                             const float *partial, int partial_rows, float *sums, float *gx, void *stream) {
    if (partial_rows < 1 || !partial) return PDF_ERR_BAD_ARG;
    return bn_act_backward(n, c, gy, x, nullptr, coef, training, relu, const_cast<float *>(partial), sums, 0, gx, nullptr, stream, partial_rows);
}
extern "C" int pdf_bn_coef_from_partial(const float *partial, int rows, long n, int c, const float *gamma, const float *beta,
                                        float *running_mean, float *running_var, float eps, float momentum, float *coef,
                                        void *stream) {
    if (!partial || rows < 1 || n < 1 || c < 1 || !gamma || !beta || !coef) return PDF_ERR_BAD_ARG;
    fl::launch_bn_finalize(partial, rows, c, (double)n, gamma, beta, eps, momentum, running_mean, running_var, coef, coef + c,
                           coef + 2 * c, coef + 3 * c, static_cast<hipStream_t>(stream));
    return pdf_launch_status();
}

extern "C" int pdf_bn_apply(long n, int c, const float *x, const float *res, const float *coef, int relu, float *y, void *stream) {
    if (n < 1 || !x || !coef || !y) return PDF_ERR_BAD_ARG;
    if (!pdf_bn_supported(c)) return PDF_ERR_UNSUPPORTED;
    const long n4 = n * (c / 4);
    (res ? pw::k_bn_apply<true> : pw::k_bn_apply<false>)<<<pw::grid_elems(n4), pw::PB, 0, static_cast<hipStream_t>(stream)>>>(
        n4, c / 4, reinterpret_cast<const float4 *>(x), reinterpret_cast<const float4 *>(coef), reinterpret_cast<const float4 *>(coef + c),
        reinterpret_cast<const float4 *>(res), relu, reinterpret_cast<float4 *>(y));
    return pdf_launch_status();
}

int pdf_bn_apply_rows(long n, int c, const float *x, const float *res, const float *rows, int nrows, const float *gamma, const float *beta,
                      float *running_mean, float *running_var, float eps, float momentum, float *coef, void *handoff, int relu, float *y,
                      void *stream) {
    if (n < 1 || !x || !rows || nrows < 1 || !gamma || !beta || !coef || !handoff || !y) return PDF_ERR_BAD_ARG;
    if (!pdf_bn_supported(c)) return PDF_ERR_UNSUPPORTED;
    PdfRowsBn b;
    b.rows = rows; b.nrows = nrows; b.c = c; b.count = (double)n; b.gamma = gamma; b.beta = beta; b.running_mean = running_mean;
    b.running_var = running_var; b.eps = eps; b.momentum = momentum; b.coef = coef;
    b.gran = static_cast<unsigned long long *>(handoff); b.sync = reinterpret_cast<unsigned *>(b.gran + 2 * (size_t)c);
    const long n4 = n * (c / 4);
    const size_t lds = sizeof(float) * 2 * c + sizeof(double) * 2 * (pw::PB / 16) * 17 + 16;
    (res ? pw::k_bn_apply_rows<true> : pw::k_bn_apply_rows<false>)<<<pw::grid_elems(n4), pw::PB, lds, static_cast<hipStream_t>(stream)>>>(
        n4, c / 4, reinterpret_cast<const float4 *>(x), b, reinterpret_cast<const float4 *>(res), relu, reinterpret_cast<float4 *>(y));
    return pdf_launch_status();
}

extern "C" int pdf_bn_coef(long n, int c, const float *x, const float *gamma, const float *beta, float *running_mean,
                           float *running_var, int training, float eps, float momentum, float *coef, float *partial, void *stream) {
    if (n < 1 || !gamma || !beta || !coef) return PDF_ERR_BAD_ARG;
    if (!pdf_bn_supported(c)) return PDF_ERR_UNSUPPORTED;
    hipStream_t s = static_cast<hipStream_t>(stream);
    if (training) {
        if (!partial || !x) return PDF_ERR_BAD_ARG;
        const int g = pw::grid_rows(n, c);
        pw::k_bn_stats<<<g, pw::PB, pw::PB * 8 * sizeof(float), s>>>(n, c, x, partial);
        fl::launch_bn_finalize(partial, g, c, (double)n, gamma, beta, eps, momentum, running_mean, running_var, coef, coef + c, coef + 2 * c, coef + 3 * c, s);
    } else {
        if (!running_mean || !running_var) return PDF_ERR_BAD_ARG;
        fl::launch_bn_eval(c, gamma, beta, eps, running_mean, running_var, coef, coef + c, coef + 2 * c, coef + 3 * c, s);
    }
    return pdf_launch_status();
}

extern "C" int pdf_bn_bwd_sums(long n, int c, const float *gy, const float *x, const float *coef, int relu, float *partial, float *sums,
                               void *stream) {
    if (n < 1 || !gy || !x || !coef || !partial || !sums) return PDF_ERR_BAD_ARG;
    if (!pdf_bn_supported(c)) return PDF_ERR_UNSUPPORTED;
    hipStream_t s = static_cast<hipStream_t>(stream);
    const int g = pw::grid_rows(n, c);
    pw::k_bn_bwd_reduce<false><<<g, pw::PB, pw::PB * 8 * sizeof(float), s>>>(n, c, gy, x, nullptr, coef, coef + c, coef + 2 * c, coef + 3 * c, relu, partial);
    fl::launch_colsum(partial, g, 2 * c, sums, s);
    return pdf_launch_status();
}
// ... 1 lines not shown
```

pointcloudpdf_amd/csrc/rowlin.hip:

```cpp
#include "pdfops_common.h"
#include <cstdlib>

namespace rl {

typedef float f32x16 __attribute__((ext_vector_type(16)));
constexpr int BM = 128, BN = 64, BK = 32, LDT = 33;

struct FwdArgs {
    long N;
    int K, O;
    const float *X; long ldx;
    const float *W; long wso, wsk;
    const float *bias;
    const float *scale, *shift;
    int relu;
    float *Y; long ldy;
    int accumulate;
    float *partial;
};

template <bool PRE, bool STATS>
__global__ __launch_bounds__(256) void k_rowlin(FwdArgs a) {
    __shared__ float xs[BM * LDT];
    __shared__ float ws[BN * LDT];
// ... 99 lines not shown
    float sc = 1.f, sh = 0.f;
    if (PRE && cv) { sc = a.scale[cc]; sh = a.shift[cc]; }
    const long rb = (long)blockIdx.x * a.rows_per_block;
    const long re = min(rb + a.rows_per_block, a.N);
    f32x16 acc;
#pragma unroll
    for (int r = 0; r < 16; ++r) acc[r] = 0.f;
    float gsum = 0.f;
    for (long r0 = rb + 8 * wave; r0 < re; r0 += 32) {
        float g[4], x[4];
#pragma unroll
        for (int u = 0; u < 4; ++u) {
            const long r = r0 + 2 * u + par;
            g[u] = (r < re && ov) ? a.G[r * a.ldg + oc] : 0.f;
            float v = 0.f;
            if (r < re && cv) {
                v = a.X[r * a.ldx + cc];
                if (PRE) { v = v * sc + sh; if (a.relu) v = fmaxf(v, 0.f); }
            }
            x[u] = v;
        }
#pragma unroll
        for (int u = 0; u < 4; ++u) {
            acc = __builtin_amdgcn_mfma_f32_32x32x2f32(g[u], x[u], acc, 0, 0, 0);
            gsum += g[u];
        }
    }
    __shared__ float comb[4][1024 + 32];
#pragma unroll
    for (int r = 0; r < 16; ++r) {
        const int i = (r & 3) + 8 * (r >> 2) + 4 * (lane >> 5);
        comb[wave][i * 32 + ch] = acc[r];
    }
    gsum += __shfl_xor(gsum, 32, 64);
    if (lane < 32) comb[wave][1024 + ch] = gsum;
    __syncthreads();
    const size_t sidx = blockIdx.x, nsl = gridDim.x;
    float *slab = a.slab + ((size_t)blockIdx.y * nsl + sidx) * 1024;
#pragma unroll
    for (int e = threadIdx.x; e < 1024; e += 256) slab[e] = ((comb[0][e] + comb[1][e]) + comb[2][e]) + comb[3][e];
    if (a.db && c0 == 0 && threadIdx.x < 32)
        a.bslab[((size_t)(o0 / 32) * nsl + sidx) * 32 + threadIdx.x] =
            ((comb[0][1024 + threadIdx.x] + comb[1][1024 + threadIdx.x]) + comb[2][1024 + threadIdx.x]) + comb[3][1024 + threadIdx.x];
}

}

namespace rl2 {
int try_forward(long n, int k, int o, int nin, int nout, const float *const *x, long ldx, const float *const *w, int transpose_w,
                const float *const *bias, const float *scale, const float *shift, int relu, float *const *y, long ldy,
                int accumulate, float *partial, int mma, hipStream_t s, const float *roww = nullptr, long rws = 0, const float *bx = nullptr,
                long ldb = 0, const float *bcoef = nullptr, int brelu = 0, int *partial_rows = nullptr, long ldw = 0, void *handoff = nullptr);
long stats_rows_floats(long n, int o);
int try_wgrad(long n, int k, int o, int ng, const float *const *g, long ldg, const float *x, long ldx, const float *scale,
              const float *shift, int relu, float *const *dw, float *const *db, float *ws, int mma, hipStream_t s, const float *roww = nullptr, long rws = 0);
long wgrad_ws_floats(long n, int k, int o, int ng);
constexpr int WG_MAXG = 5;
struct RArgs {
    const float *slab, *bslab;
    float *dW[WG_MAXG], *db[WG_MAXG];
    int B, tiles_k, tiles, otiles, split, K, O;
};
int try_wgrad_group(long n, int k, int o, int ng, const float *const *g, long ldg, const float *const *x, long ldx, const float *const *scale,
                    const float *const *shift, const int *relu, float *const *dw, float *const *db, float *ws, int mma, hipStream_t s);
void launch_slab_reduce(const RArgs &a, int ng, bool any_bias, hipStream_t s);
int stats_rows(long n);
}

static inline void tiled_wg_plan(long n, int k, int o, int *blocks_oc, long *split, long *rows_per_block) {
    *blocks_oc = ((o + 31) / 32) * ((k + 31) / 32);
    long sp = (2048 + *blocks_oc - 1) / *blocks_oc;
    const long max_split = (n + 255) / 256;
    if (sp > max_split) sp = max_split;
    if (sp < 1) sp = 1;
    *rows_per_block = ((n + sp - 1) / sp + 31) / 32 * 32;
    *split = (n + *rows_per_block - 1) / *rows_per_block;
}

static inline bool rowlin_streams(int k, int o) {
    return (k == 32 || k == 64 || k == 128 || k == 256 || k == 512) && o % 16 == 0 && getenv("PDFOPS_ROWLIN_TILED") == nullptr;
}

extern "C" int pdf_rowlin_partial_rows(long n, int k, int o) {
    return rowlin_streams(k, o) ? rl2::stats_rows(n) : (int)((n + rl::BM - 1) / rl::BM);
}
extern "C" long pdf_rowlin_partial_floats(long n, int o) {
    const long a = (n + rl::BM - 1) / rl::BM * 2 * (long)o, b = rl2::stats_rows_floats(n, o);
    return (a > b ? a : b) + (long)PDF_HO_FLOATS;
}

extern "C" int pdf_rowlin_forward(long n, int k, int o, const float *x, long ldx, const float *w, int transpose_w,
                                  const float *bias, const float *scale, const float *shift, int relu, float *y, long ldy,
                                  int accumulate, float *partial, int mma_input, void *stream) {
    if (mma_input < 0 || mma_input > 2) return PDF_ERR_BAD_ARG;
    if (n < 1 || k < 1 || o < 1 || !x || !w || !y || ldx < k || ldy < o) return PDF_ERR_BAD_ARG;
    if (rowlin_streams(k, o)) {
        if (rl2::try_forward(n, k, o, 1, 1, &x, ldx, &w, transpose_w, &bias, scale, shift, relu, &y, ldy, accumulate, partial,
                             mma_input, static_cast<hipStream_t>(stream)))
            return pdf_launch_status();
        if (partial) return PDF_ERR_BAD_ARG;
    }
    if (!transpose_w && !partial && !scale && k == 1024 && rowlin_streams(512, o) && !(ldx & 3) && !(ldy & 3)) {
        const float *xs[2] = {x, x + 512}, *ws[2] = {w, w + 512};
        if (rl2::try_forward(n, 512, o, 2, 1, xs, ldx, ws, 0, &bias, nullptr, nullptr, 0, &y, ldy, accumulate, nullptr, mma_input, static_cast<hipStream_t>(stream),
                             nullptr, 0, nullptr, 0, nullptr, 0, nullptr, k))
            return pdf_launch_status();
    }
    rl::FwdArgs a;
    a.N = n; a.K = k; a.O = o; a.X = x; a.ldx = ldx; a.W = w;
    a.wso = transpose_w ? 1 : k; a.wsk = transpose_w ? o : 1;
    a.bias = bias; a.scale = scale; a.shift = shift; a.relu = relu; a.Y = y; a.ldy = ldy; a.accumulate = accumulate;
    a.partial = partial;
    const dim3 grid((unsigned)((n + rl::BM - 1) / rl::BM), (unsigned)((o + rl::BN - 1) / rl::BN));
    hipStream_t s = static_cast<hipStream_t>(stream);
    const bool pre = scale != nullptr, stats = partial != nullptr;
    if (pre && stats) rl::k_rowlin<true, true><<<grid, 256, 0, s>>>(a);
    else if (pre) rl::k_rowlin<true, false><<<grid, 256, 0, s>>>(a);
    else if (stats) rl::k_rowlin<false, true><<<grid, 256, 0, s>>>(a);
    else rl::k_rowlin<false, false><<<grid, 256, 0, s>>>(a);
    return pdf_launch_status();
}

extern "C" long pdf_rowlin_wgrad_ws_floats(long n, int k, int o, int ng) {
    if (n < 1 || k < 1 || o < 1 || ng < 1) return 0;
    int blocks_oc; long split, rpb;
    tiled_wg_plan(n, k, o, &blocks_oc, &split, &rpb);
    const long tiled = (long)blocks_oc * split * 4 * 1024 + (long)((o + 31) / 32) * split * 4 * 32;
    const long streaming = rowlin_streams(k, o) ? rl2::wgrad_ws_floats(n, k, o, ng) : 0;
    return tiled > streaming ? tiled : streaming;
}

extern "C" int pdf_bn_coef_from_partial(const float *partial, int rows, long n, int c, const float *gamma, const float *beta,
                                        float *running_mean, float *running_var, float eps, float momentum, float *coef, void *stream);

extern "C" int pdf_rowlin_forward_bn(long n, int k, int o, const float *x, long ldx, const float *w, const float *bias, const float *scale,
                                     const float *shift, int relu, float *y, long ldy, float *partial, const float *gamma, const float *beta,
                                     float *running_mean, float *running_var, float eps, float momentum, float *coef, int mma_input, void *stream) {
    if (mma_input < 0 || mma_input > 2) return PDF_ERR_BAD_ARG;
    if (n < 1 || k < 1 || o < 1 || !x || !w || !y || !partial || !gamma || !beta || !coef || ldx < k || ldy < o) return PDF_ERR_BAD_ARG;
    if (rowlin_streams(k, o)) {
        int rows = 0;
        if (rl2::try_forward(n, k, o, 1, 1, &x, ldx, &w, 0, &bias, scale, shift, relu, &y, ldy, 0, partial, mma_input, static_cast<hipStream_t>(stream),
                             nullptr, 0, nullptr, 0, nullptr, 0, &rows)) {
            return pdf_bn_coef_from_partial(partial, rows, n, o, gamma, beta, running_mean, running_var, eps, momentum, coef, stream);
        }
    }
    const int rc = pdf_rowlin_forward(n, k, o, x, ldx, w, 0, bias, scale, shift, relu, y, ldy, 0, partial, mma_input, stream);
    if (rc) return rc;
    return pdf_bn_coef_from_partial(partial, pdf_rowlin_partial_rows(n, k, o), n, o, gamma, beta, running_mean, running_var, eps, momentum, coef, stream);
}

int pdf_rowlin_forward_stats_ho(long n, int k, int o, const float *x, long ldx, const float *w, const float *bias, const float *scale,
                                const float *shift, int relu, float *y, long ldy, float *rows_out, void *handoff, int *rows, int mma_input,
                                void *stream) {
    if (!rowlin_streams(k, o)) return PDF_ERR_UNSUPPORTED;
    if (!rl2::try_forward(n, k, o, 1, 1, &x, ldx, &w, 0, &bias, scale, shift, relu, &y, ldy, 0, rows_out, mma_input, static_cast<hipStream_t>(stream),
                          nullptr, 0, nullptr, 0, nullptr, 0, rows, 0, handoff))
        return PDF_ERR_UNSUPPORTED;
    return pdf_launch_status();
}

extern "C" int pdf_rowlin_wgrad(long n, int k, int o, const float *g, long ldg, const float *x, long ldx,
                                const float *scale, const float *shift, int relu, float *dw, float *db, float *ws, int mma_input, void *stream) {
    if (mma_input < 0 || mma_input > 2) return PDF_ERR_BAD_ARG;
    if (n < 1 || k < 1 || o < 1 || !g || !x || !dw || !ws || ldg < o || ldx < k) return PDF_ERR_BAD_ARG;
    if (rowlin_streams(k, o) && rl2::try_wgrad(n, k, o, 1, &g, ldg, x, ldx, scale, shift, relu, &dw, &db, ws, mma_input, static_cast<hipStream_t>(stream)))
        return pdf_launch_status();
    rl::WArgs a;
    a.N = n; a.K = k; a.O = o; a.G = g; a.ldg = ldg; a.X = x; a.ldx = ldx; a.scale = scale; a.shift = shift; a.relu = relu;
    a.dW = dw; a.db = db;
    int blocks_oc; long split;
    tiled_wg_plan(n, k, o, &blocks_oc, &split, &a.rows_per_block);
    a.slab = ws;
    a.bslab = ws + (size_t)blocks_oc * split * 1024;
    const dim3 grid((unsigned)split, (unsigned)blocks_oc);
    hipStream_t s = static_cast<hipStream_t>(stream);
    if (scale) rl::k_wgrad<true><<<grid, 256, 0, s>>>(a);
    else rl::k_wgrad<false><<<grid, 256, 0, s>>>(a);
    rl2::RArgs r;
    r.slab = a.slab; r.bslab = a.bslab; r.B = 32; r.tiles_k = (k + 31) / 32; r.tiles = blocks_oc; r.otiles = (o + 31) / 32; r.split = (int)split;
    r.K = k; r.O = o;
    r.dW[0] = dw; r.db[0] = db; r.dW[1] = r.dW[2] = nullptr; r.db[1] = r.db[2] = nullptr;
    rl2::launch_slab_reduce(r, 1, db != nullptr, s);
    return pdf_launch_status();
}

extern "C" int pdf_rowlin_multi(long n, int k, int o, int nin, int nout, const float *const *x, long ldx, const float *const *w,
                                int transpose_w, const float *const *bias, const float *scale, const float *shift, int relu,
                                float *const *y, long ldy, int accumulate, int mma_input, void *stream) {
    if (mma_input < 0 || mma_input > 2) return PDF_ERR_BAD_ARG;
    if (n < 1 || k < 1 || o < 1 || !x || !w || !y || nin < 1 || nout < 1 || nin > 3 || nout > 3 || (nin > 1 && nout > 1)) return PDF_ERR_BAD_ARG;
    if (rowlin_streams(k, o) && rl2::try_forward(n, k, o, nin, nout, x, ldx, w, transpose_w, bias, scale, shift, relu, y, ldy, accumulate,
                                                 nullptr, mma_input, static_cast<hipStream_t>(stream)))
        return pdf_launch_status();
    int rc = 0;
    if (nin == 1) {
        for (int i = 0; i < nout && rc == 0; ++i)
            rc = pdf_rowlin_forward(n, k, o, x[0], ldx, w[i], transpose_w, bias ? bias[i] : nullptr, scale, shift, relu, y[i], ldy, accumulate, nullptr, mma_input, stream);
    } else {
        for (int i = 0; i < nin && rc == 0; ++i)
            rc = pdf_rowlin_forward(n, k, o, x[i], ldx, w[i], transpose_w, (i == 0 && bias) ? bias[0] : nullptr, scale, shift, relu, y[0], ldy,
                                    accumulate || i > 0, nullptr, mma_input, stream);
    }
    return rc;
}

extern "C" int pdf_rowlin_dgrad_bstats(long n, int k, int o, int nin, const float *const *x, long ldx, const float *const *w, float *y, long ldy,
                                       const float *bx, long ldb, const float *bcoef, int brelu, float *partial, int *partial_rows,
                                       int mma_input, void *stream) {
    if (mma_input < 0 || mma_input > 2) return PDF_ERR_BAD_ARG;
    if (n < 1 || k < 1 || o < 1 || !x || !w || !y || nin < 1 || nin > 3 || !bx || !bcoef || !partial || !partial_rows) return PDF_ERR_BAD_ARG;
    if (!rowlin_streams(k, o)) return PDF_ERR_UNSUPPORTED;
    float *ys[1] = {y};
    if (!rl2::try_forward(n, k, o, nin, 1, x, ldx, w, 1, nullptr, nullptr, nullptr, 0, ys, ldy, 0, partial, mma_input, static_cast<hipStream_t>(stream),
                          nullptr, 0, bx, ldb, bcoef, brelu, partial_rows))
        return PDF_ERR_UNSUPPORTED;
    return pdf_launch_status();
}

extern "C" int pdf_rowlin_wgrad_multi(long n, int k, int o, int ng, const float *const *g, long ldg, const float *x, long ldx,
                                      const float *scale, const float *shift, int relu, float *const *dw, float *const *db,
                                      float *ws, int mma_input, void *stream) {
    if (mma_input < 0 || mma_input > 2) return PDF_ERR_BAD_ARG;
    if (n < 1 || k < 1 || o < 1 || ng < 1 || ng > 3 || !g || !x || !dw || !ws) return PDF_ERR_BAD_ARG;
    if (rowlin_streams(k, o) && rl2::try_wgrad(n, k, o, ng, g, ldg, x, ldx, scale, shift, relu, dw, db, ws, mma_input, static_cast<hipStream_t>(stream)))
        return pdf_launch_status();
    int rc = 0;
    for (int i = 0; i < ng && rc == 0; ++i) rc = pdf_rowlin_wgrad(n, k, o, g[i], ldg, x, ldx, scale, shift, relu, dw[i], db ? db[i] : nullptr, ws, mma_input, stream);
    return rc;
}

extern "C" int pdf_rowlin_wgrad_group(long n, int k, int o, int ng, const float *const *g, long ldg, const float *const *x, long ldx,
                                      const float *const *scale, const float *const *shift, const int *relu, float *const *dw,
                                      float *const *db, float *ws, int mma_input, void *stream) {
    if (mma_input < 0 || mma_input > 2) return PDF_ERR_BAD_ARG;
    if (n < 1 || k < 1 || o < 1 || ng < 1 || ng > rl2::WG_MAXG || !g || !x || !scale || !shift || !relu || !dw || !ws) return PDF_ERR_BAD_ARG;
    for (int i = 0; i < ng; ++i) if (!g[i] || !x[i] || !dw[i] || (scale[i] && !shift[i])) return PDF_ERR_BAD_ARG;
    if (!rowlin_streams(k, o) || !rl2::try_wgrad_group(n, k, o, ng, g, ldg, x, ldx, scale, shift, relu, dw, db, ws, mma_input, static_cast<hipStream_t>(stream)))
        return PDF_ERR_UNSUPPORTED;
// ... 23 lines not shown
```

pointcloudpdf_amd/csrc/rowlin2.hip:

```cpp
#define RL2_MAIN_TU
#include "rowlin2_impl.h"

namespace rl2 {
template int try_forward_mp<0>(long, int, int, int, int, const float *const *, long, const float *const *, int, const float *const *, const float *,
                               const float *, int, float *const *, long, int, float *, hipStream_t, const float *, long, const float *, long,
                               const float *, int, int *, long, void *);
template int try_wgrad_mp<0>(long, int, int, int, const float *const *, long, const float *, long, const float *, const float *, int,
                             float *const *, float *const *, float *, hipStream_t, const float *, long);
template int try_wgrad_group_mp<0>(long, int, int, int, const float *const *, long, const float *const *, long, const float *const *, const float *const *, const int *,
                                   float *const *, float *const *, float *, hipStream_t);
extern template int try_wgrad_group_mp<1>(long, int, int, int, const float *const *, long, const float *const *, long, const float *const *, const float *const *, const int *,
                                   float *const *, float *const *, float *, hipStream_t);
extern template int try_wgrad_group_mp<2>(long, int, int, int, const float *const *, long, const float *const *, long, const float *const *, const float *const *, const int *,
                                   float *const *, float *const *, float *, hipStream_t);
extern template int try_forward_mp<1>(long, int, int, int, int, const float *const *, long, const float *const *, int, const float *const *, const float *,
                                      const float *, int, float *const *, long, int, float *, hipStream_t, const float *, long, const float *, long,
                                      const float *, int, int *, long, void *);
extern template int try_forward_mp<2>(long, int, int, int, int, const float *const *, long, const float *const *, int, const float *const *, const float *,
                                      const float *, int, float *const *, long, int, float *, hipStream_t, const float *, long, const float *, long,
                                      const float *, int, int *, long, void *);
extern template int try_wgrad_mp<1>(long, int, int, int, const float *const *, long, const float *, long, const float *, const float *, int,
                                    float *const *, float *const *, float *, hipStream_t, const float *, long);
extern template int try_wgrad_mp<2>(long, int, int, int, const float *const *, long, const float *, long, const float *, const float *, int,
                                    float *const *, float *const *, float *, hipStream_t, const float *, long);

int try_forward(long n, int k, int o, int nin, int nout, const float *const *x, long ldx, const float *const *w, int transpose_w,
                const float *const *bias, const float *scale, const float *shift, int relu, float *const *y, long ldy,
                int accumulate, float *partial, int mma, hipStream_t s, const float *roww, long rws, const float *bx, long ldb, const float *bcoef,
                int brelu, int *partial_rows, long ldw, void *handoff) {
#define RL2_FWD(MP_) try_forward_mp<MP_>(n, k, o, nin, nout, x, ldx, w, transpose_w, bias, scale, shift, relu, y, ldy, accumulate, partial, s, roww, rws, \
                                         bx, ldb, bcoef, brelu, partial_rows, ldw, handoff)
    switch (mma) {
    case 1: return RL2_FWD(1);
    case 2: return RL2_FWD(2);
    default: return RL2_FWD(0);
    }
#undef RL2_FWD
}

int try_wgrad(long n, int k, int o, int ng, const float *const *g, long ldg, const float *x, long ldx, const float *scale,
              const float *shift, int relu, float *const *dw, float *const *db, float *ws, int mma, hipStream_t s, const float *roww, long rws) {
    switch (mma) {
    case 1: return try_wgrad_mp<1>(n, k, o, ng, g, ldg, x, ldx, scale, shift, relu, dw, db, ws, s, roww, rws);
    case 2: return try_wgrad_mp<2>(n, k, o, ng, g, ldg, x, ldx, scale, shift, relu, dw, db, ws, s, roww, rws);
    default: return try_wgrad_mp<0>(n, k, o, ng, g, ldg, x, ldx, scale, shift, relu, dw, db, ws, s, roww, rws);
    }
}

int try_wgrad_group(long n, int k, int o, int ng, const float *const *g, long ldg, const float *const *x, long ldx, const float *const *scale,
                    const float *const *shift, const int *relu, float *const *dw, float *const *db, float *ws, int mma, hipStream_t s) {
    switch (mma) {
    case 1: return try_wgrad_group_mp<1>(n, k, o, ng, g, ldg, x, ldx, scale, shift, relu, dw, db, ws, s);
    case 2: return try_wgrad_group_mp<2>(n, k, o, ng, g, ldg, x, ldx, scale, shift, relu, dw, db, ws, s);
    default: return try_wgrad_group_mp<0>(n, k, o, ng, g, ldg, x, ldx, scale, shift, relu, dw, db, ws, s);
    }
}
}
```

pointcloudpdf_amd/csrc/rowlin2_bf16.hip:

```cpp
#include "rowlin2_impl.h"

namespace rl2 {
template int try_forward_mp<2>(long, int, int, int, int, const float *const *, long, const float *const *, int, const float *const *, const float *,
                               const float *, int, float *const *, long, int, float *, hipStream_t, const float *, long, const float *, long,
                               const float *, int, int *, long, void *);
template int try_wgrad_mp<2>(long, int, int, int, const float *const *, long, const float *, long, const float *, const float *, int,
                             float *const *, float *const *, float *, hipStream_t, const float *, long);
template int try_wgrad_group_mp<2>(long, int, int, int, const float *const *, long, const float *const *, long, const float *const *, const float *const *, const int *,
                                   float *const *, float *const *, float *, hipStream_t);
}
```

pointcloudpdf_amd/csrc/rowlin2_f16.hip:

```cpp
#include "rowlin2_impl.h"

namespace rl2 {
template int try_forward_mp<1>(long, int, int, int, int, const float *const *, long, const float *const *, int, const float *const *, const float *,
                               const float *, int, float *const *, long, int, float *, hipStream_t, const float *, long, const float *, long,
                               const float *, int, int *, long, void *);
template int try_wgrad_mp<1>(long, int, int, int, const float *const *, long, const float *, long, const float *, const float *, int,
                             float *const *, float *const *, float *, hipStream_t, const float *, long);
template int try_wgrad_group_mp<1>(long, int, int, int, const float *const *, long, const float *const *, long, const float *const *, const float *const *, const int *,
                                   float *const *, float *const *, float *, hipStream_t);
}
```

pointcloudpdf_amd/csrc/rowlin2_impl.h:

```cpp
#pragma once
#include "pdfops_common.h"
#include <algorithm>
#include <cstdlib>
#include <cstring>

namespace rl2 {

typedef float f32x4 __attribute__((ext_vector_type(4)));

typedef _Float16 h16x4 __attribute__((ext_vector_type(4)));
typedef __bf16 b16x4 __attribute__((ext_vector_type(4)));
typedef short s16x4 __attribute__((ext_vector_type(4)));
template <int MP> struct Mma;
template <> struct Mma<0> {
    typedef f32x4 frag;
    static __device__ __forceinline__ frag cvt(f32x4 v) { return v; }
};
template <> struct Mma<1> {
    typedef h16x4 frag;
    static __device__ __forceinline__ frag cvt(f32x4 v) { return __builtin_convertvector(v, h16x4); }
    static __device__ __forceinline__ f32x4 mma(frag a, frag b, f32x4 acc) { return __builtin_amdgcn_mfma_f32_16x16x16f16(a, b, acc, 0, 0, 0); }
};
template <> struct Mma<2> {
    typedef s16x4 frag;
// ... 414 lines not shown
            for (int t = 0; t < 4; ++t)
#pragma unroll
                for (int c = 0; c < VW; ++c) {
                    gsum[c] += gv[t][c];
#pragma unroll
                    for (int c2 = 0; c2 < VW; ++c2)
                        acc[c][c2] = __builtin_amdgcn_mfma_f32_16x16x4f32(gv[t][c], xv[t][c2], acc[c][c2], 0, 0, 0);
                }
        } else {
            typename Mma<MP>::frag ga[VW], xa[VW];
#pragma unroll
            for (int c = 0; c < VW; ++c) {
                gsum[c] += (gv[0][c] + gv[1][c]) + (gv[2][c] + gv[3][c]);
                ga[c] = Mma<MP>::cvt(f32x4{gv[0][c], gv[1][c], gv[2][c], gv[3][c]});
                xa[c] = Mma<MP>::cvt(f32x4{xv[0][c], xv[1][c], xv[2][c], xv[3][c]});
            }
#pragma unroll
            for (int c = 0; c < VW; ++c)
#pragma unroll
                for (int c2 = 0; c2 < VW; ++c2) acc[c][c2] = Mma<MP>::mma(ga[c], xa[c2], acc[c][c2]);
        }
    }
#pragma unroll
    for (int c = 0; c < VW; ++c)
#pragma unroll
        for (int c2 = 0; c2 < VW; ++c2)
#pragma unroll
            for (int r = 0; r < 4; ++r) red[wave][(VW * (4 * nq + r) + c) * B + VW * li + c2] = acc[c][c2][r];
    float *db = a.db[blockIdx.z];
    const bool want_db = db && kb == 0;
    if (want_db) {
#pragma unroll
        for (int c = 0; c < VW; ++c) {
            float g = gsum[c];
            g += __shfl_xor(g, 16, 64);
            g += __shfl_xor(g, 32, 64);
            if (nq == 0) redb[wave][VW * li + c] = g;
        }
    }
    __syncthreads();
    float *slab = a.slab + (((size_t)blockIdx.z * gridDim.y + blockIdx.y) * gridDim.x + blockIdx.x) * (B * B);
    for (int e = threadIdx.x; e < B * B; e += 256) slab[e] = (red[0][e] + red[1][e]) + (red[2][e] + red[3][e]);
    if (want_db && threadIdx.x < B)
        a.bslab[(((size_t)blockIdx.z * (a.O / B) + ob / B) * gridDim.x + blockIdx.x) * B + threadIdx.x] =
            (redb[0][threadIdx.x] + redb[1][threadIdx.x]) + (redb[2][threadIdx.x] + redb[3][threadIdx.x]);
}

struct RArgs {
    const float *slab, *bslab;
    float *dW[WG_MAXG], *db[WG_MAXG];
    int B, tiles_k, tiles, otiles, split, K, O;
};
void launch_slab_reduce(const RArgs &a, int ng, bool any_bias, hipStream_t s);
template <int L>
__global__ __launch_bounds__(64 * L) void k_slab_reduce(RArgs a) {
    __shared__ float red[L][64];
    const int e = threadIdx.x & 63, l = threadIdx.x >> 6, z = blockIdx.z;
    const int ei = blockIdx.x * 64 + e;
    const bool bias = (int)blockIdx.y >= a.tiles;
    const int t = bias ? (int)blockIdx.y - a.tiles : (int)blockIdx.y;
    const int len = bias ? a.B : a.B * a.B;
    if (bias && (int)blockIdx.x * 64 >= len) return;
    const float *src = bias ? a.bslab + ((size_t)z * a.otiles + t) * a.split * a.B : a.slab + ((size_t)z * a.tiles + t) * a.split * (size_t)(a.B * a.B);
    float s = 0.f;
    if (ei < len) {
        int k = l;
        for (; k + 3 * L < a.split; k += 4 * L) {
            const float v0 = src[(size_t)k * len + ei], v1 = src[(size_t)(k + L) * len + ei];
            const float v2 = src[(size_t)(k + 2 * L) * len + ei], v3 = src[(size_t)(k + 3 * L) * len + ei];
            s = (((s + v0) + v1) + v2) + v3;
        }
        for (; k < a.split; k += L) s += src[(size_t)k * len + ei];
    }
    red[l][e] = s;
    __syncthreads();
    if (l != 0 || ei >= len) return;
#pragma unroll
    for (int k = 1; k < L; ++k) s += red[k][e];
    if (bias) {
        const int o = t * a.B + ei;
        if (a.db[z] && o < a.O) a.db[z][o] = s;
    } else {
        const int o = (t / a.tiles_k) * a.B + ei / a.B, kk = (t % a.tiles_k) * a.B + ei % a.B;
        if (o < a.O && kk < a.K) a.dW[z][(size_t)o * a.K + kk] = s;
    }
}

#ifdef RL2_MAIN_TU
void launch_slab_reduce(const RArgs &a, int ng, bool any_bias, hipStream_t s) {
    const dim3 grid((unsigned)((a.B * a.B + 63) / 64), (unsigned)(a.tiles + (any_bias ? a.otiles : 0)), (unsigned)ng);
    if (a.split > 32) k_slab_reduce<16><<<grid, 64 * 16, 0, s>>>(a);
    else if (a.split > 4) k_slab_reduce<4><<<grid, 64 * 4, 0, s>>>(a);
    else k_slab_reduce<1><<<grid, 64, 0, s>>>(a);
}
#endif

struct WgPlan { int vw, b, nblk; long split, rows_per_block; };
static WgPlan wg_plan(long n, int k, int o, int ng) {
    WgPlan p;
    p.vw = (k % 64 == 0 && o % 64 == 0) ? 4 : ((k % 32 == 0 && o % 32 == 0) ? 2 : 0);
    p.b = 16 * p.vw;
    if (!p.vw) { p.nblk = 0; p.split = 0; p.rows_per_block = 0; return p; }
    p.nblk = (o / p.b) * (k / p.b) * ng;
    static const int target = [] { const char *v = getenv("PDFOPS_WG_BLOCKS"); const int x = v ? atoi(v) : 0; return x > 0 ? x : 512; }();
    long split = (target + p.nblk - 1) / p.nblk;
    const long max_split = (n + 255) / 256;
    if (split > max_split) split = max_split;
    if (split < 1) split = 1;
    p.rows_per_block = ((n + split - 1) / split + 63) / 64 * 64;
    p.split = (n + p.rows_per_block - 1) / p.rows_per_block;
    return p;
}
#ifdef RL2_MAIN_TU
long wgrad_ws_floats(long n, int k, int o, int ng) {
    const WgPlan p = wg_plan(n, k, o, ng);
    if (!p.vw) return 0;
    return (long)p.nblk * p.split * p.b * p.b + (long)ng * (o / p.b) * p.split * p.b;
}
#endif

static inline bool aligned16(const void *p) { return (reinterpret_cast<uintptr_t>(p) & 15) == 0; }

constexpr long GROUP_MAX_ROWS = 16384;
static bool group_form_wanted(const FwdArgs &a, int k, int blocks) {
    if (blocks % GROUP_GN) return false;
    if (const char *f = getenv("PDFOPS_RL_FORM")) {
        if (!strcmp(f, "slab")) return false;
        if (!strcmp(f, "group")) return true;
    }
    return a.N <= GROUP_MAX_ROWS && !(k == 128 && blocks * 16 > a.O);
}

template <int K, int GN, int NIN, bool PRE, int ST, int MP>
static bool launch_group_kernel(const FwdArgs &a, dim3 grid, hipStream_t s) {
    constexpr int lds = group_lds_bytes<K, GN, NIN, MP>();
    static PdfLdsLimit site;
    if (!pdf_lds_limit_raised(site, reinterpret_cast<const void *>(&k_fwd_group<K, GN, NIN, PRE, ST, MP>), lds)) return false;
    k_fwd_group<K, GN, NIN, PRE, ST, MP><<<grid, 256, lds, s>>>(a);
    return true;
}

template <int K, int GN, int NIN, int MP>
static bool launch_fwd_group(const FwdArgs &a, int blocks, int gx, hipStream_t s) {
    const bool pre = a.scale != nullptr, stats = a.partial != nullptr, bst = stats && a.bx != nullptr;
    const dim3 grid((unsigned)gx, (unsigned)(blocks / GN));
    if (bst) return launch_group_kernel<K, GN, NIN, false, 2, MP>(a, grid, s);
// ... 37 lines not shown
    if (nin < 1 || nout < 1 || (nin > 1 && nout > 1) || nin > 3 || nout > 3) return 0;
    if (nin == 2 && (scale || bx)) return 0;
    if (partial && !bx && (nin != 1 || nout != 1)) return 0;
    if (bx && (!partial || nout != 1 || scale || !bcoef || (ldb & 3) || !aligned16(bx) || !aligned16(bcoef))) return 0;
    if ((ldx & 3) || (ldy & 3) || (o & 15)) return 0;
    for (int i = 0; i < (nin > 1 ? nin : nout); ++i) if (!aligned16(w[i])) return 0;
    if (scale && (!aligned16(scale) || !aligned16(shift))) return 0;
    for (int i = 0; i < nin; ++i) if (!aligned16(x[i])) return 0;
    for (int i = 0; i < nout; ++i) if (!aligned16(y[i])) return 0;
    FwdArgs a;
    a.N = n; a.O = o; a.ldx = ldx; a.ldy = ldy; a.scale = scale; a.shift = shift; a.relu = relu; a.accumulate = accumulate;
    a.partial = partial; a.roww = roww; a.rws = rws;
    a.bx = bx; a.ldb = ldb; a.bcoef = bcoef; a.brelu = brelu;
    a.ho_gran = static_cast<unsigned long long *>(handoff);
    a.ho_sync = handoff ? reinterpret_cast<unsigned *>(a.ho_gran + 2 * (size_t)o) : nullptr;
    a.wso = transpose_w ? 1 : (ldw ? ldw : k); a.wsk = transpose_w ? o : 1;
    for (int i = 0; i < 3; ++i) {
        a.X[i] = i < nin ? x[i] : nullptr;
        a.W[i] = i < (nin > 1 ? nin : nout) ? w[i] : nullptr;
        a.bias[i] = (bias && i < nout) ? bias[i] : nullptr;
        a.Y[i] = i < nout ? y[i] : nullptr;
    }
    const int cols = o * nout;
#define PDF_RL2(K_, NOB_, NIN_) do { if (cols % (NOB_ * 16) == 0) { \
        const int r_ = launch_fwd<K_, NOB_, NIN_, MP>(a, cols / (NOB_ * 16), s); \
        if (partial_rows) *partial_rows = r_; \
        return 1; } } while (0)
    if (nin == 1) {
        switch (k) {
        case 32: if (!partial) PDF_RL2(32, 6, 1); PDF_RL2(32, 2, 1); PDF_RL2(32, 1, 1); break;
        case 64: PDF_RL2(64, 4, 1); PDF_RL2(64, 1, 1); break;
        case 128: if (!bx) PDF_RL2(128, 4, 1); else PDF_RL2(128, 2, 1); PDF_RL2(128, 1, 1); break;
        case 256: PDF_RL2(256, 2, 1); PDF_RL2(256, 1, 1); break;
        case 512: PDF_RL2(512, 1, 1); break;
        default: break;
        }
    } else if (nin == 2) {
        if (k == 512) PDF_RL2(512, 1, 2);
    } else if (nin == 3) {
        switch (k) {
        case 32: PDF_RL2(32, 2, 3); break;
        case 64: PDF_RL2(64, 2, 3); break;
        case 128: PDF_RL2(128, 1, 3); break;
        case 256: PDF_RL2(256, 1, 3); break;
        default: break;
        }
    }
#undef PDF_RL2
    return 0;
}

template <int MP>
int try_wgrad_mp(long n, int k, int o, int ng, const float *const *g, long ldg, const float *x, long ldx, const float *scale,
                 const float *shift, int relu, float *const *dw, float *const *db, float *ws, hipStream_t s, const float *roww, long rws) {
    if (ng < 1 || ng > 3 || !ws) return 0;
    const WgPlan p = wg_plan(n, k, o, ng);
    const int vw = p.vw;
    if (!vw) return 0;
    if ((ldg % vw) || (ldx % vw) || !aligned16(x)) return 0;
    if (scale && (!aligned16(scale) || !aligned16(shift))) return 0;
    for (int i = 0; i < ng; ++i) if (!aligned16(g[i])) return 0;
    WArgs a;
    a.N = n; a.K = k; a.O = o; a.ldg = ldg; a.X = x; a.ldx = ldx; a.scale = scale; a.shift = shift; a.relu = relu; a.roww = roww; a.rws = rws;
    a.per_z = 0;
    bool any_bias = false;
    for (int i = 0; i < WG_MAXG; ++i) {
        a.G[i] = i < ng ? g[i] : nullptr; a.dW[i] = i < ng ? dw[i] : nullptr; a.db[i] = (db && i < ng) ? db[i] : nullptr;
        a.Xz[i] = nullptr; a.scalez[i] = a.shiftz[i] = nullptr; a.reluz[i] = 0;
        any_bias = any_bias || a.db[i] != nullptr;
    }
    const int b = p.b;
    a.rows_per_block = p.rows_per_block;
    a.slab = ws;
    a.bslab = ws + (size_t)p.nblk * p.split * b * b;
    const dim3 grid((unsigned)p.split, (unsigned)((o / b) * (k / b)), (unsigned)ng);
#define PDF_WG(VW_) do { \
        if (roww) { if (scale) k_wg<VW_, true, true, MP><<<grid, 256, 0, s>>>(a); else k_wg<VW_, false, true, MP><<<grid, 256, 0, s>>>(a); } \
        else      { if (scale) k_wg<VW_, true, false, MP><<<grid, 256, 0, s>>>(a); else k_wg<VW_, false, false, MP><<<grid, 256, 0, s>>>(a); } } while (0)
    if (vw == 4) PDF_WG(4); else PDF_WG(2);
#undef PDF_WG
    RArgs r;
    r.slab = a.slab; r.bslab = a.bslab; r.B = b; r.tiles_k = k / b; r.tiles = (o / b) * (k / b); r.otiles = o / b; r.split = (int)p.split; r.K = k; r.O = o;
    for (int i = 0; i < WG_MAXG; ++i) { r.dW[i] = a.dW[i]; r.db[i] = a.db[i]; }
    launch_slab_reduce(r, ng, any_bias, s);
    return 1;
}

template <int MP>
int try_wgrad_group_mp(long n, int k, int o, int ng, const float *const *g, long ldg, const float *const *x, long ldx,
                       const float *const *scale, const float *const *shift, const int *relu, float *const *dw, float *const *db,
                       float *ws, hipStream_t s) {
    if (ng < 1 || ng > WG_MAXG || !ws) return 0;
    const WgPlan p = wg_plan(n, k, o, ng);
    const int vw = p.vw;
    if (!vw) return 0;
    if ((ldg % vw) || (ldx % vw)) return 0;
    for (int i = 0; i < ng; ++i) {
        if (!aligned16(g[i]) || !aligned16(x[i])) return 0;
        if (scale[i] && (!aligned16(scale[i]) || !aligned16(shift[i]))) return 0;
    }
    WArgs a;
    a.N = n; a.K = k; a.O = o; a.ldg = ldg; a.X = nullptr; a.ldx = ldx; a.scale = a.shift = nullptr; a.relu = 0; a.roww = nullptr; a.rws = 0;
    a.per_z = 1;
    bool any_bias = false;
    for (int i = 0; i < WG_MAXG; ++i) {
        const bool on = i < ng;
        a.G[i] = on ? g[i] : nullptr; a.Xz[i] = on ? x[i] : nullptr;
        a.scalez[i] = on ? scale[i] : nullptr; a.shiftz[i] = on ? shift[i] : nullptr; a.reluz[i] = on ? relu[i] : 0;
        a.dW[i] = on ? dw[i] : nullptr; a.db[i] = (on && db) ? db[i] : nullptr;
        any_bias = any_bias || a.db[i] != nullptr;
    }
    const int b = p.b;
    a.rows_per_block = p.rows_per_block;
    a.slab = ws;
    a.bslab = ws + (size_t)p.nblk * p.split * b * b;
    const dim3 grid((unsigned)p.split, (unsigned)((o / b) * (k / b)), (unsigned)ng);
    if (vw == 4) k_wg<4, true, false, MP><<<grid, 256, 0, s>>>(a); else k_wg<2, true, false, MP><<<grid, 256, 0, s>>>(a);
    RArgs r;
    r.slab = a.slab; r.bslab = a.bslab; r.B = b; r.tiles_k = k / b; r.tiles = (o / b) * (k / b); r.otiles = o / b; r.split = (int)p.split; r.K = k; r.O = o;
    for (int i = 0; i < WG_MAXG; ++i) { r.dW[i] = a.dW[i]; r.db[i] = a.db[i]; }
    launch_slab_reduce(r, ng, any_bias, s);
    return 1;
}

#ifdef RL2_MAIN_TU
int stats_rows(long n) { return fwd_row_blocks(n); }
#endif

}
```

pointcloudpdf_amd/dense.py:

```python
import ctypes
import os
from ctypes import c_void_p

import torch

def _amp_fwd(fn):
    import functools

    from . import _native
    inner = torch.amp.custom_fwd(fn, device_type="cuda", cast_inputs=torch.float32)

    @functools.wraps(fn)
    def wrapped(ctx, *args, **kwargs):
        ctx._pdf_mma = _native.current_mma_input()
        return inner(ctx, *args, **kwargs)

    return wrapped


def _amp_bwd(fn):
    import functools

    from . import _native
    inner = torch.amp.custom_bwd(fn, device_type="cuda")
# ... 675 lines not shown
        if rc != 0:
            raise RuntimeError(f"pdf_linbn_forward failed with status {rc}")
        ctx.save_for_backward(x, z, coef, W)
        ctx.cfg = (training, relu, b is not None)
        return y

    @staticmethod
    @_amp_bwd
    def backward(ctx, gy):
        x, z, coef, W = ctx.saved_tensors
        training, relu, has_bias = ctx.cfg
        be = _be()
        lib = be.lib
        n, k = x.shape
        o = W.shape[0]
        e = lambda *shape: torch.empty(shape, dtype=torch.float32, device=x.device)
        need_gx = ctx.needs_input_grad[3]
        gx = e(n, k) if need_gx else None
        grads, gz = e(o * k + 3 * o), e(n, o)
        partial = e(int(lib.pdf_bn_partial_floats(n, o)))
        gy = gy.contiguous()
        ws = be.wgrad_workspace(n, k, o, 1, x.device)
        ptrs = [gy.data_ptr(), x.data_ptr(), z.data_ptr(), coef.data_ptr(), W.data_ptr(), gx.data_ptr() if need_gx else None, grads.data_ptr(),
                gz.data_ptr(), partial.data_ptr(), ws.data_ptr()]
        rc = lib.pdf_linbn_backward(n, k, o, (c_void_p * len(ptrs))(*ptrs), int(training), int(relu), _mma(), be._stream())
        if rc != 0:
            raise RuntimeError(f"pdf_linbn_backward failed with status {rc}")
        ok = o * k
        return (None, None, None, gx, grads[:ok].view(o, k), grads[ok:ok + o] if has_bias else None, grads[ok + 2 * o:ok + 3 * o], grads[ok + o:ok + 2 * o])


LINBN = True


def linbn_ok(lin, bn, x):
    if not LINBN:
        return False
    if not (x.is_cuda and x.dim() == 2 and x.dtype == torch.float32 and x.is_contiguous() and type(bn) is torch.nn.BatchNorm1d and bn.affine
            and bn.track_running_stats and bn.momentum is not None):
        return False
    k, o = lin.in_features, lin.out_features
    if k not in (32, 64, 128, 256, 512) or o % 16 or not _be().bn_supported(o):
        return False
    if torch.is_grad_enabled() and not bn.training and any(p.requires_grad for p in list(lin.parameters()) + list(bn.parameters())):
        return False
    return True


def linear_bn_act(lin, bn, x, relu):
    y = _LinBnFn.apply(lin, bn, relu, x, lin.weight, lin.bias, bn.weight, bn.bias)
    if bn.training:
        bump_counters([bn.num_batches_tracked])
    return y
```

pointcloudpdf_amd/point_transformer.py:

```python
import os

import torch

import torch.nn as nn
import torch.nn.functional as F

from . import _native, pointops
from . import dense
from .dense import _amp_bwd, _amp_fwd, bn_act as _bn_act, linear as _lin
from .geometry import Geometry, tag_of
from .registry import MODELS


def _seq(seq, x):
    mods = list(seq)
    i = 0
    while i < len(mods):
        m = mods[i]
        if (isinstance(m, nn.Linear) and i + 1 < len(mods) and isinstance(mods[i + 1], nn.BatchNorm1d) and x.dim() == 2
                and dense.linbn_ok(m, mods[i + 1], x)):
            relu = i + 2 < len(mods) and isinstance(mods[i + 2], nn.ReLU)
            x = dense.linear_bn_act(m, mods[i + 1], x, relu)
            i += 3 if relu else 2
            continue
# ... 200 lines not shown
    def backward(ctx, g):
        if ctx.offset is None:
            return torch.cat([(g[i:i + 1] / n).expand(n, -1) for i, n in enumerate(ctx.sizes)], 0), None, None
        g = g.contiguous()
        out = torch.empty((ctx.n, g.shape[1]), dtype=g.dtype, device=g.device)
        _native.backend_for(g)._call("scene_repeat_rows", len(ctx.sizes), ctx.offset, ctx.n, g.shape[1], g, 1, out)
        return out, None, None


class _RowsPerScene(torch.autograd.Function):

    @staticmethod
    @_amp_fwd
    def forward(ctx, rows, offset, sizes_dev, sizes_host, total):
        ctx.sizes = [int(v) for v in sizes_host]
        be = _scene_rows_kernels(rows)
        if be is None:
            ctx.offset = None
            return torch.repeat_interleave(rows, sizes_dev, dim=0, output_size=total)
        rows = rows.contiguous()
        ctx.offset = offset = offset.int().contiguous()
        out = torch.empty((total, rows.shape[1]), dtype=rows.dtype, device=rows.device)
        be._call("scene_repeat_rows", len(ctx.sizes), offset, total, rows.shape[1], rows, 0, out)
        return out

    @staticmethod
    @_amp_bwd
    def backward(ctx, g):
        if ctx.offset is None:
            return torch.cat([ch.sum(0, keepdim=True) for ch in g.split(ctx.sizes, dim=0)], 0), None, None, None, None
        g = g.contiguous()
        out = torch.empty((len(ctx.sizes), g.shape[1]), dtype=g.dtype, device=g.device)
        _native.backend_for(g)._call("scene_sum_rows", len(ctx.sizes), ctx.offset, g.shape[1], g, g.shape[1], 0, out)
        return out, None, None, None, None


class TransitionUp(nn.Module):

    def __init__(self, in_planes, out_planes=None):
        super().__init__()
        if out_planes is None:
            self.linear1 = nn.Sequential(nn.Linear(2 * in_planes, in_planes), nn.BatchNorm1d(in_planes), nn.ReLU(inplace=True))
            self.linear2 = nn.Sequential(nn.Linear(in_planes, in_planes), nn.ReLU(inplace=True))
        else:
            self.linear1 = nn.Sequential(nn.Linear(out_planes, out_planes), nn.BatchNorm1d(out_planes), nn.ReLU(inplace=True))
            self.linear2 = nn.Sequential(nn.Linear(in_planes, out_planes), nn.BatchNorm1d(out_planes), nn.ReLU(inplace=True))

    @staticmethod
    def _scene_sizes(p, o):
        tag = tag_of(p)
        ends = tag[0].offset_host(tag[1]) if tag is not None else [int(v) for v in o.detach().cpu().tolist()]
        return [ends[0]] + [ends[i] - ends[i - 1] for i in range(1, len(ends))]

    def forward(self, pxo1, pxo2=None):
        if pxo2 is None:
            p, x, o = pxo1
            sizes = self._scene_sizes(p, o)
            means = _SceneMean.apply(x, o, sizes)
            ctx = _seq(self.linear2, means)
            tag = tag_of(p)
            sizes_dev = tag[0].sizes(tag[1]) if tag is not None else torch.diff(o.long(), prepend=o.new_zeros(1).long())
            rep = _RowsPerScene.apply(ctx, o, sizes_dev, sizes, x.shape[0])
            x = _seq(self.linear1, torch.cat((x, rep), 1))
        else:
            p1, x1, o1 = pxo1
            p2, x2, o2 = pxo2
            x = _seq(self.linear1, x1) + pointops.interpolation(p2, p1, _seq(self.linear2, x2), o2, o1)
        return x


class Bottleneck(nn.Module):

    expansion = 1

    def __init__(self, in_planes, planes, share_planes=8, nsample=16):
        super().__init__()
        self.linear1 = nn.Linear(in_planes, planes, bias=False)
        self.bn1 = nn.BatchNorm1d(planes)
        self.transformer = PointTransformerLayer(planes, planes, share_planes, nsample)
        self.bn2 = nn.BatchNorm1d(planes)
        self.linear3 = nn.Linear(planes, planes * self.expansion, bias=False)
        self.bn3 = nn.BatchNorm1d(planes * self.expansion)
        self.relu = nn.ReLU(inplace=True)

    def _apply(self, fn, *a, **kw):
        self.__dict__.pop("_pdf_params", None)
        return super()._apply(fn, *a, **kw)

    matrix_core = os.environ.get("PDFOPS_MATRIX_CORE", "1") != "0"

    def forward(self, pxo):
        p, x, o = pxo
        identity = x
        t = self.transformer
        if self.matrix_core and dense.fused_ok(x, self.bn1, self.bn2, self.bn3):
            return [p, dense.bottleneck(self, p, x, o), o]
        x = _bn_act(self.bn1, _lin(self.linear1, x), None, True)
        x = _bn_act(self.bn2, self.transformer([p, x, o]), None, True)
        x = _bn_act(self.bn3, _lin(self.linear3, x), identity, True)
        return [p, x, o]


class PointTransformerSeg(nn.Module):

    def __init__(self, block, blocks, in_channels=6, num_classes=13):
        super().__init__()
        self.in_channels = in_channels
        self.in_planes, planes = in_channels, [32, 64, 128, 256, 512]
        share_planes = 8
        stride, nsample = [1, 4, 4, 4, 4], [8, 16, 16, 16, 16]
        self.strides, self.nsamples = stride, nsample
        for i in range(5):
            setattr(self, f"enc{i + 1}", self._make_enc(block, planes[i], blocks[i], share_planes, stride[i], nsample[i]))
        for i in range(4, -1, -1):
            setattr(self, f"dec{i + 1}", self._make_dec(block, planes[i], 1, share_planes, nsample[i], is_head=(i == 4)))
        self.cls = nn.Sequential(
            nn.Linear(planes[0], planes[0]), nn.BatchNorm1d(planes[0]), nn.ReLU(inplace=True), nn.Linear(planes[0], num_classes)
        )
        self._last_geometry = None

# ... 60 lines not shown
```

Baseline: 13.84 million.

## Fuse TransitionUp decoder join into paired linear+BN kernels with fused interpolation

Adds a fused TransitionUp path for the two-input decoder join. Both linear layers run their forward passes, and their BatchNorm finalize steps are merged into one launch. A single join kernel then applies BN+ReLU to both branches, interpolates the coarse branch and adds the result. Backward likewise pairs the BN-backward, colsum and slab-reduce wgrad launches across both branches. The aim is to cut kernel launches and the intermediate activation round-trips for BN outputs and the interpolation. The cost is a fairly large new code path with a fallback when its conditions are not met.

```diff
diff --git a/include/pdfops.h b/include/pdfops.h
--- a/include/pdfops.h
+++ b/include/pdfops.h
@@ -11,7 +11,7 @@
 #define PDF_ERR_UNSUPPORTED (-3)
 #define PDF_ERR_NOT_CONVERGED (-4)
 
-#define PDF_ABI_VERSION 18
+#define PDF_ABI_VERSION 19
 int pdf_abi_version(void);
 const char *pdf_build_info(void);
 int pdf_dist_fma_mode(void);
@@ -177,6 +177,13 @@
 int pdf_bottleneck_backward(long n, int nsample, int c, void *const *p, int training, int entry_base, int storage_bf16, int mma_input, void *stream);
 int pdf_linbn_forward(long n, int k, int o, void *const *p, int training, int relu, float eps, float momentum, int mma_input, void *stream);
 int pdf_linbn_backward(long n, int k, int o, void *const *p, int training, int relu, int mma_input, void *stream);
+int pdf_transition_up_supported(int k1, int k2, int o);
+int pdf_transition_up_forward(long n1, int k1, long n2, int k2, int o, void *const *p, int training, float eps, float momentum, int mma_input,
+                              void *stream);
+int pdf_transition_up_backward(long n1, int k1, long n2, int k2, int o, void *const *p, int entry_base, int mma_input, void *stream);
+int pdf_bn_coef_from_partial2(int rows0, long n0, int c0, int rows1, long n1, int c1, void *const *p, float eps, float momentum, void *stream);
+int pdf_bn_act_backward2(long n0, int c0, long n1, int c1, void *const *p, int relu, void *stream);
+int pdf_rowlin_wgrad2(long n0, int k0, int o0, long n1, int k1, int o1, void *const *p, int mma_input, void *stream);
 
 int pdf_rowlin_forward_roww(long n, int k, int o, const float *x, long ldx, const float *w, int transpose_w, float *y, long ldy,
                             int accumulate, const float *roww, long rws, int mma_input, void *stream);
diff --git a/pointcloudpdf_amd/_native.py b/pointcloudpdf_amd/_native.py
--- a/pointcloudpdf_amd/_native.py
+++ b/pointcloudpdf_amd/_native.py
@@ -15,7 +15,7 @@
 
 
 LIB_PATH = library_path(DIST_FMA)
-ABI_VERSION = 18
+ABI_VERSION = 19
 
 c_int = ctypes.c_int
 c_long = ctypes.c_long
@@ -734,6 +734,18 @@
         lib.pdf_linbn_forward.argtypes = [c_long, c_int, c_int, c_void_p, c_int, c_int, ctypes.c_float, ctypes.c_float, c_int, c_void_p]
         lib.pdf_linbn_backward.restype = c_int
         lib.pdf_linbn_backward.argtypes = [c_long, c_int, c_int, c_void_p, c_int, c_int, c_int, c_void_p]
+        lib.pdf_transition_up_supported.restype = c_int
+        lib.pdf_transition_up_supported.argtypes = [c_int, c_int, c_int]
+        lib.pdf_transition_up_forward.restype = c_int
+        lib.pdf_transition_up_forward.argtypes = [c_long, c_int, c_long, c_int, c_int, c_void_p, c_int, ctypes.c_float, ctypes.c_float, c_int, c_void_p]
+        lib.pdf_transition_up_backward.restype = c_int
+        lib.pdf_transition_up_backward.argtypes = [c_long, c_int, c_long, c_int, c_int, c_void_p, c_int, c_int, c_void_p]
+        lib.pdf_bn_coef_from_partial2.restype = c_int
+        lib.pdf_bn_coef_from_partial2.argtypes = [c_int, c_long, c_int, c_int, c_long, c_int, c_void_p, ctypes.c_float, ctypes.c_float, c_void_p]
+        lib.pdf_bn_act_backward2.restype = c_int
+        lib.pdf_bn_act_backward2.argtypes = [c_long, c_int, c_long, c_int, c_void_p, c_int, c_void_p]
+        lib.pdf_rowlin_wgrad2.restype = c_int
+        lib.pdf_rowlin_wgrad2.argtypes = [c_long, c_int, c_int, c_long, c_int, c_int, c_void_p, c_int, c_void_p]
         lib.pdf_bottleneck_forward.restype = c_int
         lib.pdf_bottleneck_forward.argtypes = [c_long, c_int, c_int, c_void_p, c_int, ctypes.c_float, ctypes.c_float, c_int, c_int, c_void_p]
         lib.pdf_bottleneck_backward.restype = c_int
diff --git a/pointcloudpdf_amd/csrc/block.hip b/pointcloudpdf_amd/csrc/block.hip
--- a/pointcloudpdf_amd/csrc/block.hip
+++ b/pointcloudpdf_amd/csrc/block.hip
@@ -1,4 +1,5 @@
 #include "pdfops_common.h"
+#include <initializer_list>
 
 namespace {
 struct Err {
@@ -226,3 +227,75 @@
     e << pdf_rowlin_wgrad(n, k, o, gz, o, (const float *)p[1], k, nullptr, nullptr, 0, grads, grads + ok, (float *)p[9], mma_input, stream);
     return e.rc;
 }
+
+extern "C" int pdf_transition_up_supported(int k1, int k2, int o) {
+    return pdf_rowlin_streams(k1, o) && pdf_rowlin_streams(k2, o) && k1 % 32 == 0 && k2 % 32 == 0 && o % 32 == 0 && pdf_bn_supported(o);
+}
+static bool tu_aligned(void *const *p, std::initializer_list<int> which) {
+    uintptr_t all = 0;
+    for (int i : which) all |= reinterpret_cast<uintptr_t>(p[i]);
+    return (all & 15) == 0;
+}
+static bool tu_sizes_ok(long n1, long n2, int o) {
+    return n1 * (o / 4) < (1L << 31) && n2 * (o / 4) < (1L << 31) && n1 * 3 < (1L << 31);
+}
+
+extern "C" int pdf_transition_up_forward(long n1, int k1, long n2, int k2, int o, void *const *p, int training, float eps, float momentum,
+                                         int mma_input, void *stream) {
+    if (n1 < 1 || n2 < 1 || !p || mma_input < 0 || mma_input > 2) return PDF_ERR_BAD_ARG;
+    for (int i = 0; i < 24; ++i)
+        if (!p[i] && i != 2 && i != 9 && i != 16) return PDF_ERR_BAD_ARG;
+    if (!training || !pdf_transition_up_supported(k1, k2, o) || !tu_sizes_ok(n1, n2, o) || !tu_aligned(p, {0, 1, 7, 8, 17, 18, 20, 21, 23})) return PDF_ERR_UNSUPPORTED;
+    Err e;
+    PdfBnFinalize2 f;
+    const long n[2] = {n1, n2};
+    const int k[2] = {k1, k2};
+    for (int i = 0; i < 2; ++i) {
+        void *const *t = p + 7 * i;
+        float *z = (float *)p[17 + 3 * i], *partial = (float *)p[19 + 3 * i];
+        e << pdf_rowlin_forward(n[i], k[i], o, (const float *)t[0], k[i], (const float *)t[1], 0, (const float *)t[2], nullptr, nullptr, 0, z, o, 0, partial,
+                                mma_input, stream);
+        f.partial[i] = partial; f.rows[i] = pdf_rowlin_partial_rows(n[i], k[i], o); f.nch[i] = o; f.count[i] = (double)n[i];
+        f.gamma[i] = (const float *)t[3]; f.beta[i] = (const float *)t[4]; f.running_mean[i] = (float *)t[5]; f.running_var[i] = (float *)t[6];
+        f.coef[i] = (float *)p[18 + 3 * i];
+    }
+    f.split = 0;
+    if (e.rc) return e.rc;
+    e << pdf_bn_finalize2(f, eps, momentum, stream);
+    e << pdf_tu_join(n1, o, (const float *)p[17], (const float *)p[18], (const float *)p[20], (const float *)p[21], (const int *)p[14],
+                     (const float *)p[15], (const int *)p[16], (float *)p[23], stream);
+    return e.rc;
+}
+
+extern "C" int pdf_transition_up_backward(long n1, int k1, long n2, int k2, int o, void *const *p, int entry_base, int mma_input, void *stream) {
+    if (n1 < 1 || n2 < 1 || !p || mma_input < 0 || mma_input > 2) return PDF_ERR_BAD_ARG;
+    for (int i = 0; i < 24; ++i)
+        if (!p[i] && i != 12 && i != 13 && i != 14) return PDF_ERR_BAD_ARG;
+    if (!pdf_transition_up_supported(k1, k2, o) || !tu_sizes_ok(n1, n2, o) || !tu_aligned(p, {0, 1, 2, 3, 5, 6, 7, 15, 16, 17, 18, 19})) return PDF_ERR_UNSUPPORTED;
+    const float *g = (const float *)p[0];
+    float *g2 = (float *)p[17];
+    const long n[2] = {n1, n2};
+    const int k[2] = {k1, k2};
+    Err e;
+    e << pdf_seg_sum_weighted_ordered(n2, o, 3, 1, g, (const float *)p[9], (const int *)p[10], (const int *)p[11], entry_base, (const int *)p[12], g2, stream);
+    if (e.rc) return e.rc;
+    PdfBnBwd2 b;
+    PdfWgrad2 w;
+    for (int i = 0; i < 2; ++i) {
+        void *const *t = p + 1 + 4 * i;
+        float *grads = (float *)p[15 + i];
+        const long ok = (long)o * k[i];
+        b.n[i] = n[i]; b.c[i] = o; b.gy[i] = i ? g2 : g; b.x[i] = (const float *)t[1]; b.coef[i] = (const float *)t[2];
+        b.partial[i] = (float *)p[20 + i]; b.sums[i] = grads + ok + o; b.gx[i] = (float *)p[18 + i];
+        w.n[i] = n[i]; w.k[i] = k[i]; w.o[i] = o; w.g[i] = b.gx[i]; w.x[i] = (const float *)t[0]; w.dw[i] = grads; w.db[i] = grads + ok;
+        w.ws[i] = (float *)p[22 + i];
+    }
+    b.split = 0;
+    e << pdf_bn_backward2(b, 1, stream);
+    for (int i = 0; i < 2; ++i)
+        if (p[13 + i])
+            e << pdf_rowlin_forward(n[i], o, k[i], b.gx[i], o, (const float *)p[4 + 4 * i], 1, nullptr, nullptr, nullptr, 0, (float *)p[13 + i], k[i], 0, nullptr,
+                                    mma_input, stream);
+    e << pdf_rowlin_wgrad_pair(w, mma_input, stream);
+    return e.rc;
+}
diff --git a/pointcloudpdf_amd/csrc/fused_layer.hip b/pointcloudpdf_amd/csrc/fused_layer.hip
--- a/pointcloudpdf_amd/csrc/fused_layer.hip
+++ b/pointcloudpdf_amd/csrc/fused_layer.hip
@@ -828,6 +828,20 @@
     int col_g;
     float *out4;
 };
+__device__ __forceinline__ void colsum_block(const float *__restrict__ partial, int rows, int width, int stride, float *__restrict__ out,
+                                             unsigned block, double (*red)[17]) {
+    const int cl = threadIdx.x & 15, rl = threadIdx.x >> 4;
+    const int col = block * 16 + cl;
+    const double v = wave_rows_sum(col < width ? strided_sum(partial + col, (size_t)stride, rl, rows) : 0.0);
+    if ((threadIdx.x & 63) < 16) red[threadIdx.x >> 6][cl] = v;
+    __syncthreads();
+    if (rl != 0 || col >= width) return;
+    double s = 0.0;
+#pragma unroll
+    for (int k = 0; k < RED_WAVES; ++k) s += red[k][cl];
+    out[col] = (float)s;
+}
+
 __global__ __launch_bounds__(RED_THREADS) void k_colsum(const float *__restrict__ partial, int rows, int width, int stride, float *__restrict__ out,
                                                         BnpClosed bc) {
     __shared__ double red[RED_WAVES][17];
@@ -866,26 +880,16 @@
         }
         return;
     }
-    const int cl = threadIdx.x & 15, rl = threadIdx.x >> 4;
-    const int col = blockIdx.x * 16 + cl;
-    const double v = wave_rows_sum(col < width ? strided_sum(partial + col, (size_t)stride, rl, rows) : 0.0);
-    if ((threadIdx.x & 63) < 16) red[threadIdx.x >> 6][cl] = v;
-    __syncthreads();
-    if (rl != 0 || col >= width) return;
-    double s = 0.0;
-#pragma unroll
-    for (int k = 0; k < RED_WAVES; ++k) s += red[k][cl];
-    out[col] = (float)s;
-}
-
-__global__ __launch_bounds__(RED_THREADS) void k_bn_finalize(const float *__restrict__ partial, int rows, int nch, double count,
+    colsum_block(partial, rows, width, stride, out, blockIdx.x, red);
+}
+
+__device__ __forceinline__ void bn_finalize_block(const float *__restrict__ partial, int rows, int nch, double count,
                               const float *__restrict__ gamma, const float *__restrict__ beta, float eps, float momentum,
                               float *__restrict__ running_mean, float *__restrict__ running_var,
                               float *__restrict__ scale, float *__restrict__ shift, float *__restrict__ mean_out,
-                              float *__restrict__ rstd_out) {
-    __shared__ double red[2][RED_WAVES][17];
+                              float *__restrict__ rstd_out, unsigned block, double (*red)[RED_WAVES][17]) {
     const int cl = threadIdx.x & 15, rl = threadIdx.x >> 4;
-    const int ch = blockIdx.x * 16 + cl;
+    const int ch = block * 16 + cl;
     const double a = wave_rows_sum(ch < nch ? strided_sum(partial + ch, 2 * (size_t)nch, rl, rows) : 0.0);
     const double b = wave_rows_sum(ch < nch ? strided_sum(partial + nch + ch, 2 * (size_t)nch, rl, rows) : 0.0);
     if ((threadIdx.x & 63) < 16) { red[0][threadIdx.x >> 6][cl] = a; red[1][threadIdx.x >> 6][cl] = b; }
@@ -909,6 +913,27 @@
         running_var[ch] = (1.f - momentum) * running_var[ch] + momentum * (float)unbiased;
     }
 }
+__global__ __launch_bounds__(RED_THREADS) void k_bn_finalize(const float *__restrict__ partial, int rows, int nch, double count,
+                              const float *__restrict__ gamma, const float *__restrict__ beta, float eps, float momentum,
+                              float *__restrict__ running_mean, float *__restrict__ running_var,
+                              float *__restrict__ scale, float *__restrict__ shift, float *__restrict__ mean_out,
+                              float *__restrict__ rstd_out) {
+    __shared__ double red[2][RED_WAVES][17];
+    bn_finalize_block(partial, rows, nch, count, gamma, beta, eps, momentum, running_mean, running_var, scale, shift, mean_out, rstd_out,
+                      blockIdx.x, red);
+}
+
+__global__ __launch_bounds__(RED_THREADS) void k_bn_finalize2(PdfBnFinalize2 q, float eps, float momentum) {
+    __shared__ double red[2][RED_WAVES][17];
+    const int i = blockIdx.x >= (unsigned)q.split ? 1 : 0;
+    bn_finalize_block(q.partial[i], q.rows[i], q.nch[i], q.count[i], q.gamma[i], q.beta[i], eps, momentum, q.running_mean[i], q.running_var[i],
+                      q.coef[i], q.coef[i] + q.nch[i], q.coef[i] + 2 * q.nch[i], q.coef[i] + 3 * q.nch[i], blockIdx.x - (i ? q.split : 0), red);
+}
+__global__ __launch_bounds__(RED_THREADS) void k_colsum2(PdfColsum2 q) {
+    __shared__ double red[RED_WAVES][17];
+    const int i = blockIdx.x >= (unsigned)q.split ? 1 : 0;
+    colsum_block(q.partial[i], q.rows[i], q.width[i], q.width[i], q.out[i], blockIdx.x - (i ? q.split : 0), red);
+}
 
 __global__ void k_bn_eval(int nch, const float *__restrict__ gamma, const float *__restrict__ beta, float eps,
                           const float *__restrict__ running_mean, const float *__restrict__ running_var,
@@ -938,6 +963,15 @@
     none.mom = nullptr; none.out4 = nullptr; none.rows = 0.0; none.col_g = 0;
     none.Wp1 = none.bp1 = none.sp = none.mean = none.rstd = as_const(nullptr);
     k_colsum<<<pdf_divup(width, 16), RED_THREADS, 0, s>>>(partial, rows, width, width, out, none);
+}
+
+void launch_bn_finalize2(PdfBnFinalize2 q, float eps, float momentum, hipStream_t s) {
+    q.split = pdf_divup(q.nch[0], 16);
+    k_bn_finalize2<<<q.split + pdf_divup(q.nch[1], 16), RED_THREADS, 0, s>>>(q, eps, momentum);
+}
+void launch_colsum2(PdfColsum2 q, hipStream_t s) {
+    q.split = pdf_divup(q.width[0], 16);
+    k_colsum2<<<q.split + pdf_divup(q.width[1], 16), RED_THREADS, 0, s>>>(q);
 }
 
 template <typename KernelT>
diff --git a/pointcloudpdf_amd/csrc/gather_ops.hip b/pointcloudpdf_amd/csrc/gather_ops.hip
--- a/pointcloudpdf_amd/csrc/gather_ops.hip
+++ b/pointcloudpdf_amd/csrc/gather_ops.hip
@@ -364,6 +364,41 @@
 #pragma unroll
     for (int i = 0; i < K; ++i) acc += (j[i] >= 0 ? v[i] : (v4f)(0.f)) * wt[i];
     st_stream(output + (unsigned long)r * cv + col, acc);
+}
+
+__device__ __forceinline__ v4f tu_norm_relu(v4f z, v4f s, v4f t) {
+    v4f o;
+#pragma unroll
+    for (int e = 0; e < 4; ++e) o[e] = fmaxf(__fadd_rn(__fmaf_rn(z[e], s[e], t[e]), 0.f), 0.f);
+    return o;
+}
+template <int K>
+__global__ __launch_bounds__(GB) void k_tu_join(unsigned total, FastDiv cvd, const int *__restrict__ order, const v4f *__restrict__ z1,
+                                                const v4f *__restrict__ coef1, const v4f *__restrict__ z2, const v4f *__restrict__ coef2,
+                                                const int *__restrict__ idx, const float *__restrict__ weight, v4f *__restrict__ output) {
+    const unsigned cv = cvd.d, blk = xcd_chunked_block(blockIdx.x, gridDim.x);
+    const unsigned w = blk * GB + threadIdx.x;
+    if (w >= total) return;
+    const unsigned sq = fdiv(w, cvd), col = w - sq * cv, r = order ? (unsigned)order[sq] : sq;
+    int j[K]; float wt[K]; v4f v[K];
+#pragma unroll
+    for (int i = 0; i < K; ++i) { j[i] = idx[(unsigned long)r * K + i]; wt[i] = weight[(unsigned long)r * K + i]; }
+#pragma unroll
+    for (int i = 0; i < K; ++i) v[i] = z2[(unsigned long)max(j[i], 0) * cv + col];
+    const v4f own = z1[(unsigned long)r * cv + col];
+    const v4f s1 = coef1[col], t1 = coef1[cv + col], s2 = coef2[col], t2 = coef2[cv + col];
+    v4f acc = (v4f)(0.f);
+#pragma unroll
+    for (int i = 0; i < K; ++i) {
+        const v4f a = j[i] >= 0 ? tu_norm_relu(v[i], s2, t2) : (v4f)(0.f);
+#pragma unroll
+        for (int e = 0; e < 4; ++e) acc[e] = __fmaf_rn(a[e], wt[i], acc[e]);
+    }
+    const v4f y1 = tu_norm_relu(own, s1, t1);
+    v4f o;
+#pragma unroll
+    for (int e = 0; e < 4; ++e) o[e] = __fadd_rn(y1[e], acc[e]);
+    st_stream(output + (unsigned long)r * cv + col, o);
 }
 
 __global__ __launch_bounds__(GB) void agg_fwd_ord(unsigned total, FastDiv cvd, int nsample, unsigned wv, const int *__restrict__ order,
@@ -787,6 +822,16 @@
     return pdf_launch_status();
 }
 
+int pdf_tu_join(long n1, int o, const float *z1, const float *coef1, const float *z2, const float *coef2, const int *idx, const float *weight,
+                const int *order, float *out, void *stream) {
+    if (n1 < 1 || !z1 || !coef1 || !z2 || !coef2 || !idx || !weight || !out) return PDF_ERR_BAD_ARG;
+    if (o < 4 || (o & 3) || n1 * (o / 4) >= (1L << 31) || n1 * 3 >= (1L << 31)) return PDF_ERR_UNSUPPORTED;
+    const unsigned total = (unsigned)(n1 * (o / 4));
+    k_tu_join<3><<<(total + GB - 1) / GB, GB, 0, static_cast<hipStream_t>(stream)>>>(total, mk_fastdiv(o / 4), order, (const v4f *)z1, (const v4f *)coef1,
+                                                                                    (const v4f *)z2, (const v4f *)coef2, idx, weight, (v4f *)out);
+    return pdf_launch_status();
+}
+
 extern "C" int pdf_interpolation_forward(int n, int c, int k, const float *input, const int *idx, const float *weight, float *output, void *stream) {
     return pdf_interpolation_forward_ordered(n, c, k, input, idx, weight, nullptr, output, stream);
 }
diff --git a/pointcloudpdf_amd/csrc/pdfops_common.h b/pointcloudpdf_amd/csrc/pdfops_common.h
--- a/pointcloudpdf_amd/csrc/pdfops_common.h
+++ b/pointcloudpdf_amd/csrc/pdfops_common.h
@@ -115,6 +115,39 @@
 int pdf_bn_apply_rows(long n, int c, const float *x, const float *res, const float *rows, int nrows, const float *gamma, const float *beta,
                       float *running_mean, float *running_var, float eps, float momentum, float *coef, void *handoff, int relu, float *y,
                       void *stream);
+
+struct PdfBnFinalize2 {
+    const float *partial[2]; int rows[2], nch[2]; double count[2];
+    const float *gamma[2], *beta[2]; float *running_mean[2], *running_var[2], *coef[2];
+    int split;
+};
+struct PdfColsum2 {
+    const float *partial[2]; int rows[2], width[2]; float *out[2];
+    int split;
+};
+struct PdfBnBwd2 {
+    long n[2]; int c[2];
+    const float *gy[2], *x[2], *coef[2];
+    float *partial[2];
+    float *sums[2];
+    float *gx[2];
+    int split;
+};
+namespace fl {
+void launch_bn_finalize2(PdfBnFinalize2 q, float eps, float momentum, hipStream_t s);
+void launch_colsum2(PdfColsum2 q, hipStream_t s);
+}
+int pdf_bn_finalize2(PdfBnFinalize2 q, float eps, float momentum, void *stream);
+int pdf_bn_backward2(PdfBnBwd2 q, int relu, void *stream);
+struct PdfWgrad2 {
+    long n[2]; int k[2], o[2];
+    const float *g[2], *x[2];
+    float *dw[2], *db[2], *ws[2];
+};
+int pdf_rowlin_wgrad_pair(const PdfWgrad2 &q, int mma_input, void *stream);
+int pdf_rowlin_streams(int k, int o);
+int pdf_tu_join(long n1, int o, const float *z1, const float *coef1, const float *z2, const float *coef2, const int *idx, const float *weight,
+                const int *order, float *out, void *stream);
 
 __device__ __forceinline__ void pdf_handoff_zero(unsigned long long *gran, int c, unsigned *sync) {
     for (int e = threadIdx.x; e < 2 * c; e += blockDim.x) gran[e] = 0ull;
diff --git a/pointcloudpdf_amd/csrc/pointwise.hip b/pointcloudpdf_amd/csrc/pointwise.hip
--- a/pointcloudpdf_amd/csrc/pointwise.hip
+++ b/pointcloudpdf_amd/csrc/pointwise.hip
@@ -77,11 +77,11 @@
 }
 
 template <bool RES>
-__global__ __launch_bounds__(PB) void k_bn_bwd_reduce(long n, int c, const float *__restrict__ gy, const float *__restrict__ x,
-                                                      const float *__restrict__ res, const float *__restrict__ scale,
-                                                      const float *__restrict__ shift, const float *__restrict__ mean,
-                                                      const float *__restrict__ rstd, int relu, float *partial) {
-    extern __shared__ float red[];
+__device__ __forceinline__ void bn_bwd_reduce_block(long n, int c, const float *__restrict__ gy, const float *__restrict__ x,
+                                                    const float *__restrict__ res, const float *__restrict__ scale,
+                                                    const float *__restrict__ shift, const float *__restrict__ mean,
+                                                    const float *__restrict__ rstd, int relu, float *partial, unsigned block, unsigned nblocks,
+                                                    float *red) {
     const int tpr = c / 4, rpb = PB / tpr;
     const int tr = threadIdx.x / tpr, tc = threadIdx.x % tpr;
     float s[4] = {0.f, 0.f, 0.f, 0.f}, sx[4] = {0.f, 0.f, 0.f, 0.f};
@@ -89,7 +89,7 @@
         float sc[4], sh[4], mu[4], rs[4];
 #pragma unroll
         for (int k = 0; k < 4; ++k) { sc[k] = scale[tc * 4 + k]; sh[k] = shift[tc * 4 + k]; mu[k] = mean[tc * 4 + k]; rs[k] = rstd[tc * 4 + k]; }
-        for (long r = (long)blockIdx.x * rpb + tr; r < n; r += (long)gridDim.x * rpb) {
+        for (long r = (long)block * rpb + tr; r < n; r += (long)nblocks * rpb) {
             const float4 g4 = *reinterpret_cast<const float4 *>(gy + r * c + tc * 4);
             const float4 x4 = *reinterpret_cast<const float4 *>(x + r * c + tc * 4);
             const float4 r4 = RES ? *reinterpret_cast<const float4 *>(res + r * c + tc * 4) : make_float4(0.f, 0.f, 0.f, 0.f);
@@ -112,18 +112,34 @@
             float a = 0.f;
             for (int rr = 0; rr < rpb; ++rr) a += red[(rr * tpr + threadIdx.x) * 8 + k];
             const int ch = threadIdx.x * 4 + (k & 3);
-            partial[(size_t)blockIdx.x * 2 * c + (k < 4 ? ch : c + ch)] = a;
-        }
-    }
-}
-
-template <bool RES>
-__global__ __launch_bounds__(PB) void k_bn_bwd_apply(long n4, int c4, const float4 *__restrict__ gy, const float4 *__restrict__ x,
-                                                     const float4 *__restrict__ res, const float4 *__restrict__ scale,
-                                                     const float4 *__restrict__ shift, const float4 *__restrict__ mean,
-                                                     const float4 *__restrict__ rstd, const float4 *__restrict__ sums, float inv_n,
-                                                     int relu, float4 *__restrict__ gx, float4 *__restrict__ gres) {
-    for (long e = (long)blockIdx.x * PB + threadIdx.x; e < n4; e += (long)gridDim.x * PB) {
+            partial[(size_t)block * 2 * c + (k < 4 ? ch : c + ch)] = a;
+        }
+    }
+}
+template <bool RES>
+__global__ __launch_bounds__(PB) void k_bn_bwd_reduce(long n, int c, const float *__restrict__ gy, const float *__restrict__ x,
+                                                      const float *__restrict__ res, const float *__restrict__ scale,
+                                                      const float *__restrict__ shift, const float *__restrict__ mean,
+                                                      const float *__restrict__ rstd, int relu, float *partial) {
+    extern __shared__ float red[];
+    bn_bwd_reduce_block<RES>(n, c, gy, x, res, scale, shift, mean, rstd, relu, partial, blockIdx.x, gridDim.x, red);
+}
+__global__ __launch_bounds__(PB) void k_bn_bwd_reduce2(PdfBnBwd2 q, int relu) {
+    extern __shared__ float red[];
+    const int i = blockIdx.x >= (unsigned)q.split ? 1 : 0;
+    const float *coef = q.coef[i];
+    const int c = q.c[i];
+    bn_bwd_reduce_block<false>(q.n[i], c, q.gy[i], q.x[i], nullptr, coef, coef + c, coef + 2 * c, coef + 3 * c, relu, q.partial[i],
+                               blockIdx.x - (i ? q.split : 0), i ? gridDim.x - q.split : q.split, red);
+}
+
+template <bool RES>
+__device__ __forceinline__ void bn_bwd_apply_block(long n4, int c4, const float4 *__restrict__ gy, const float4 *__restrict__ x,
+                                                   const float4 *__restrict__ res, const float4 *__restrict__ scale,
+                                                   const float4 *__restrict__ shift, const float4 *__restrict__ mean,
+                                                   const float4 *__restrict__ rstd, const float4 *__restrict__ sums, float inv_n,
+                                                   int relu, float4 *__restrict__ gx, float4 *__restrict__ gres, unsigned block, unsigned nblocks) {
+    for (long e = (long)block * PB + threadIdx.x; e < n4; e += (long)nblocks * PB) {
         const int cc = (int)(e % c4);
         const float4 g4 = gy[e], x4 = x[e], sc = scale[cc], sh = shift[cc], mu = mean[cc], rs = rstd[cc];
         const float4 s1 = sums[cc], s2 = sums[c4 + cc];
@@ -141,6 +157,23 @@
         gx[e] = o;
         if (gres) gres[e] = gm;
     }
+}
+template <bool RES>
+__global__ __launch_bounds__(PB) void k_bn_bwd_apply(long n4, int c4, const float4 *__restrict__ gy, const float4 *__restrict__ x,
+                                                     const float4 *__restrict__ res, const float4 *__restrict__ scale,
+                                                     const float4 *__restrict__ shift, const float4 *__restrict__ mean,
+                                                     const float4 *__restrict__ rstd, const float4 *__restrict__ sums, float inv_n,
+                                                     int relu, float4 *__restrict__ gx, float4 *__restrict__ gres) {
+    bn_bwd_apply_block<RES>(n4, c4, gy, x, res, scale, shift, mean, rstd, sums, inv_n, relu, gx, gres, blockIdx.x, gridDim.x);
+}
+__global__ __launch_bounds__(PB) void k_bn_bwd_apply2(PdfBnBwd2 q, float inv_n0, float inv_n1, int relu) {
+    const int i = blockIdx.x >= (unsigned)q.split ? 1 : 0;
+    const int c = q.c[i];
+    const float4 *coef = reinterpret_cast<const float4 *>(q.coef[i]);
+    bn_bwd_apply_block<false>(q.n[i] * (c / 4), c / 4, reinterpret_cast<const float4 *>(q.gy[i]), reinterpret_cast<const float4 *>(q.x[i]), nullptr,
+                              coef, coef + c / 4, coef + 2 * (c / 4), coef + 3 * (c / 4), reinterpret_cast<const float4 *>(q.sums[i]),
+                              i ? inv_n1 : inv_n0, relu, reinterpret_cast<float4 *>(q.gx[i]), nullptr,
+                              blockIdx.x - (i ? q.split : 0), i ? gridDim.x - q.split : q.split);
 }
 
 template <bool RES>
@@ -253,6 +286,63 @@
     return pdf_launch_status();
 }
 
+int pdf_bn_finalize2(PdfBnFinalize2 q, float eps, float momentum, void *stream) {
+    for (int i = 0; i < 2; ++i) {
+        if (!q.partial[i] || q.rows[i] < 1 || q.count[i] < 1.0 || !q.gamma[i] || !q.beta[i] || !q.coef[i]) return PDF_ERR_BAD_ARG;
+        if (!pdf_bn_supported(q.nch[i])) return PDF_ERR_UNSUPPORTED;
+    }
+    fl::launch_bn_finalize2(q, eps, momentum, static_cast<hipStream_t>(stream));
+    return pdf_launch_status();
+}
+int pdf_bn_backward2(PdfBnBwd2 q, int relu, void *stream) {
+    for (int i = 0; i < 2; ++i) {
+        if (q.n[i] < 1 || !q.gy[i] || !q.x[i] || !q.coef[i] || !q.partial[i] || !q.sums[i] || !q.gx[i]) return PDF_ERR_BAD_ARG;
+        if (!pdf_bn_supported(q.c[i])) return PDF_ERR_UNSUPPORTED;
+    }
+    hipStream_t s = static_cast<hipStream_t>(stream);
+    const int g0 = pw::grid_rows(q.n[0], q.c[0]), g1 = pw::grid_rows(q.n[1], q.c[1]);
+    q.split = g0;
+    pw::k_bn_bwd_reduce2<<<g0 + g1, pw::PB, pw::PB * 8 * sizeof(float), s>>>(q, relu);
+    PdfColsum2 cs;
+    for (int i = 0; i < 2; ++i) { cs.partial[i] = q.partial[i]; cs.rows[i] = i ? g1 : g0; cs.width[i] = 2 * q.c[i]; cs.out[i] = q.sums[i]; }
+    fl::launch_colsum2(cs, s);
+    const int a0 = pw::grid_elems(q.n[0] * (q.c[0] / 4)), a1 = pw::grid_elems(q.n[1] * (q.c[1] / 4));
+    q.split = a0;
+    pw::k_bn_bwd_apply2<<<a0 + a1, pw::PB, 0, s>>>(q, (float)(1.0 / (double)q.n[0]), (float)(1.0 / (double)q.n[1]), relu);
+    return pdf_launch_status();
+}
+
+extern "C" int pdf_bn_coef_from_partial2(int rows0, long n0, int c0, int rows1, long n1, int c1, void *const *p, float eps, float momentum,
+                                         void *stream) {
+    if (!p || n0 < 1 || n1 < 1) return PDF_ERR_BAD_ARG;
+    PdfBnFinalize2 q;
+    const int rows[2] = {rows0, rows1}, c[2] = {c0, c1};
+    const long n[2] = {n0, n1};
+    for (int i = 0; i < 2; ++i) {
+        void *const *t = p + 6 * i;
+        q.partial[i] = (const float *)t[0]; q.rows[i] = rows[i]; q.nch[i] = c[i]; q.count[i] = (double)n[i];
+        q.gamma[i] = (const float *)t[1]; q.beta[i] = (const float *)t[2]; q.running_mean[i] = (float *)t[3]; q.running_var[i] = (float *)t[4];
+        q.coef[i] = (float *)t[5];
+        if (!t[3] != !t[4]) return PDF_ERR_BAD_ARG;
+    }
+    q.split = 0;
+    return pdf_bn_finalize2(q, eps, momentum, stream);
+}
+extern "C" int pdf_bn_act_backward2(long n0, int c0, long n1, int c1, void *const *p, int relu, void *stream) {
+    if (!p) return PDF_ERR_BAD_ARG;
+    PdfBnBwd2 q;
+    const int c[2] = {c0, c1};
+    const long n[2] = {n0, n1};
+    for (int i = 0; i < 2; ++i) {
+        void *const *t = p + 6 * i;
+        q.n[i] = n[i]; q.c[i] = c[i];
+        q.gy[i] = (const float *)t[0]; q.x[i] = (const float *)t[1]; q.coef[i] = (const float *)t[2];
+        q.partial[i] = (float *)t[3]; q.sums[i] = (float *)t[4]; q.gx[i] = (float *)t[5];
+    }
+    q.split = 0;
+    return pdf_bn_backward2(q, relu, stream);
+}
+
 extern "C" int pdf_bn_apply(long n, int c, const float *x, const float *res, const float *coef, int relu, float *y, void *stream) {
     if (n < 1 || !x || !coef || !y) return PDF_ERR_BAD_ARG;
     if (!pdf_bn_supported(c)) return PDF_ERR_UNSUPPORTED;
diff --git a/pointcloudpdf_amd/csrc/rowlin.hip b/pointcloudpdf_amd/csrc/rowlin.hip
--- a/pointcloudpdf_amd/csrc/rowlin.hip
+++ b/pointcloudpdf_amd/csrc/rowlin.hip
@@ -175,8 +175,6 @@
                 int accumulate, float *partial, int mma, hipStream_t s, const float *roww = nullptr, long rws = 0, const float *bx = nullptr,
                 long ldb = 0, const float *bcoef = nullptr, int brelu = 0, int *partial_rows = nullptr, long ldw = 0, void *handoff = nullptr);
 long stats_rows_floats(long n, int o);
-int try_wgrad(long n, int k, int o, int ng, const float *const *g, long ldg, const float *x, long ldx, const float *scale,
-              const float *shift, int relu, float *const *dw, float *const *db, float *ws, int mma, hipStream_t s, const float *roww = nullptr, long rws = 0);
 long wgrad_ws_floats(long n, int k, int o, int ng);
 constexpr int WG_MAXG = 5;
 struct RArgs {
@@ -184,6 +182,10 @@
     float *dW[WG_MAXG], *db[WG_MAXG];
     int B, tiles_k, tiles, otiles, split, K, O;
 };
+int try_wgrad(long n, int k, int o, int ng, const float *const *g, long ldg, const float *x, long ldx, const float *scale,
+              const float *shift, int relu, float *const *dw, float *const *db, float *ws, int mma, hipStream_t s, const float *roww = nullptr, long rws = 0,
+              RArgs *defer = nullptr);
+void launch_slab_reduce2(const RArgs &a0, bool bias0, const RArgs &a1, bool bias1, hipStream_t s);
 int try_wgrad_group(long n, int k, int o, int ng, const float *const *g, long ldg, const float *const *x, long ldx, const float *const *scale,
                     const float *const *shift, const int *relu, float *const *dw, float *const *db, float *ws, int mma, hipStream_t s);
 void launch_slab_reduce(const RArgs &a, int ng, bool any_bias, hipStream_t s);
@@ -203,6 +205,8 @@
 static inline bool rowlin_streams(int k, int o) {
     return (k == 32 || k == 64 || k == 128 || k == 256 || k == 512) && o % 16 == 0 && getenv("PDFOPS_ROWLIN_TILED") == nullptr;
 }
+
+int pdf_rowlin_streams(int k, int o) { return rowlin_streams(k, o) ? 1 : 0; }
 
 extern "C" int pdf_rowlin_partial_rows(long n, int k, int o) {
     return rowlin_streams(k, o) ? rl2::stats_rows(n) : (int)((n + rl::BM - 1) / rl::BM);
@@ -308,6 +312,35 @@
     return pdf_launch_status();
 }
 
+int pdf_rowlin_wgrad_pair(const PdfWgrad2 &q, int mma_input, void *stream) {
+    if (mma_input < 0 || mma_input > 2) return PDF_ERR_BAD_ARG;
+    for (int i = 0; i < 2; ++i) {
+        if (q.n[i] < 1 || q.k[i] < 1 || q.o[i] < 1 || !q.g[i] || !q.x[i] || !q.dw[i] || !q.ws[i]) return PDF_ERR_BAD_ARG;
+        if (!rowlin_streams(q.k[i], q.o[i]) || (q.k[i] % 32) || (q.o[i] % 32)) return PDF_ERR_UNSUPPORTED;
+        if ((reinterpret_cast<uintptr_t>(q.g[i]) | reinterpret_cast<uintptr_t>(q.x[i])) & 15) return PDF_ERR_UNSUPPORTED;
+    }
+    hipStream_t s = static_cast<hipStream_t>(stream);
+    rl2::RArgs r[2];
+    for (int i = 0; i < 2; ++i) {
+        const float *g = q.g[i];
+        float *dw = q.dw[i], *db = q.db[i];
+        if (!rl2::try_wgrad(q.n[i], q.k[i], q.o[i], 1, &g, q.o[i], q.x[i], q.k[i], nullptr, nullptr, 0, &dw, &db, q.ws[i], mma_input, s, nullptr, 0, &r[i]))
+            return PDF_ERR_UNSUPPORTED;
+    }
+    rl2::launch_slab_reduce2(r[0], q.db[0] != nullptr, r[1], q.db[1] != nullptr, s);
+    return pdf_launch_status();
+}
+extern "C" int pdf_rowlin_wgrad2(long n0, int k0, int o0, long n1, int k1, int o1, void *const *p, int mma_input, void *stream) {
+    if (!p) return PDF_ERR_BAD_ARG;
+    PdfWgrad2 q;
+    q.n[0] = n0; q.k[0] = k0; q.o[0] = o0; q.n[1] = n1; q.k[1] = k1; q.o[1] = o1;
+    for (int i = 0; i < 2; ++i) {
+        void *const *t = p + 5 * i;
+        q.g[i] = (const float *)t[0]; q.x[i] = (const float *)t[1]; q.dw[i] = (float *)t[2]; q.db[i] = (float *)t[3]; q.ws[i] = (float *)t[4];
+    }
+    return pdf_rowlin_wgrad_pair(q, mma_input, stream);
+}
+
 extern "C" int pdf_rowlin_multi(long n, int k, int o, int nin, int nout, const float *const *x, long ldx, const float *const *w,
                                 int transpose_w, const float *const *bias, const float *scale, const float *shift, int relu,
                                 float *const *y, long ldy, int accumulate, int mma_input, void *stream) {
diff --git a/pointcloudpdf_amd/csrc/rowlin2.hip b/pointcloudpdf_amd/csrc/rowlin2.hip
--- a/pointcloudpdf_amd/csrc/rowlin2.hip
+++ b/pointcloudpdf_amd/csrc/rowlin2.hip
@@ -6,7 +6,7 @@
                                const float *, int, float *const *, long, int, float *, hipStream_t, const float *, long, const float *, long,
                                const float *, int, int *, long, void *);
 template int try_wgrad_mp<0>(long, int, int, int, const float *const *, long, const float *, long, const float *, const float *, int,
-                             float *const *, float *const *, float *, hipStream_t, const float *, long);
+                             float *const *, float *const *, float *, hipStream_t, const float *, long, RArgs *);
 template int try_wgrad_group_mp<0>(long, int, int, int, const float *const *, long, const float *const *, long, const float *const *, const float *const *, const int *,
                                    float *const *, float *const *, float *, hipStream_t);
 extern template int try_wgrad_group_mp<1>(long, int, int, int, const float *const *, long, const float *const *, long, const float *const *, const float *const *, const int *,
@@ -20,9 +20,9 @@
                                       const float *, int, float *const *, long, int, float *, hipStream_t, const float *, long, const float *, long,
                                       const float *, int, int *, long, void *);
 extern template int try_wgrad_mp<1>(long, int, int, int, const float *const *, long, const float *, long, const float *, const float *, int,
-                                    float *const *, float *const *, float *, hipStream_t, const float *, long);
+                                    float *const *, float *const *, float *, hipStream_t, const float *, long, RArgs *);
 extern template int try_wgrad_mp<2>(long, int, int, int, const float *const *, long, const float *, long, const float *, const float *, int,
-                                    float *const *, float *const *, float *, hipStream_t, const float *, long);
+                                    float *const *, float *const *, float *, hipStream_t, const float *, long, RArgs *);
 
 int try_forward(long n, int k, int o, int nin, int nout, const float *const *x, long ldx, const float *const *w, int transpose_w,
                 const float *const *bias, const float *scale, const float *shift, int relu, float *const *y, long ldy,
@@ -39,11 +39,12 @@
 }
 
 int try_wgrad(long n, int k, int o, int ng, const float *const *g, long ldg, const float *x, long ldx, const float *scale,
-              const float *shift, int relu, float *const *dw, float *const *db, float *ws, int mma, hipStream_t s, const float *roww, long rws) {
+              const float *shift, int relu, float *const *dw, float *const *db, float *ws, int mma, hipStream_t s, const float *roww, long rws,
+              RArgs *defer) {
     switch (mma) {
-    case 1: return try_wgrad_mp<1>(n, k, o, ng, g, ldg, x, ldx, scale, shift, relu, dw, db, ws, s, roww, rws);
-    case 2: return try_wgrad_mp<2>(n, k, o, ng, g, ldg, x, ldx, scale, shift, relu, dw, db, ws, s, roww, rws);
-    default: return try_wgrad_mp<0>(n, k, o, ng, g, ldg, x, ldx, scale, shift, relu, dw, db, ws, s, roww, rws);
+    case 1: return try_wgrad_mp<1>(n, k, o, ng, g, ldg, x, ldx, scale, shift, relu, dw, db, ws, s, roww, rws, defer);
+    case 2: return try_wgrad_mp<2>(n, k, o, ng, g, ldg, x, ldx, scale, shift, relu, dw, db, ws, s, roww, rws, defer);
+    default: return try_wgrad_mp<0>(n, k, o, ng, g, ldg, x, ldx, scale, shift, relu, dw, db, ws, s, roww, rws, defer);
     }
 }
 
diff --git a/pointcloudpdf_amd/csrc/rowlin2_bf16.hip b/pointcloudpdf_amd/csrc/rowlin2_bf16.hip
--- a/pointcloudpdf_amd/csrc/rowlin2_bf16.hip
+++ b/pointcloudpdf_amd/csrc/rowlin2_bf16.hip
@@ -5,7 +5,7 @@
                                const float *, int, float *const *, long, int, float *, hipStream_t, const float *, long, const float *, long,
                                const float *, int, int *, long, void *);
 template int try_wgrad_mp<2>(long, int, int, int, const float *const *, long, const float *, long, const float *, const float *, int,
-                             float *const *, float *const *, float *, hipStream_t, const float *, long);
+                             float *const *, float *const *, float *, hipStream_t, const float *, long, RArgs *);
 template int try_wgrad_group_mp<2>(long, int, int, int, const float *const *, long, const float *const *, long, const float *const *, const float *const *, const int *,
                                    float *const *, float *const *, float *, hipStream_t);
 }
diff --git a/pointcloudpdf_amd/csrc/rowlin2_f16.hip b/pointcloudpdf_amd/csrc/rowlin2_f16.hip
--- a/pointcloudpdf_amd/csrc/rowlin2_f16.hip
+++ b/pointcloudpdf_amd/csrc/rowlin2_f16.hip
@@ -5,7 +5,7 @@
                                const float *, int, float *const *, long, int, float *, hipStream_t, const float *, long, const float *, long,
                                const float *, int, int *, long, void *);
 template int try_wgrad_mp<1>(long, int, int, int, const float *const *, long, const float *, long, const float *, const float *, int,
-                             float *const *, float *const *, float *, hipStream_t, const float *, long);
+                             float *const *, float *const *, float *, hipStream_t, const float *, long, RArgs *);
 template int try_wgrad_group_mp<1>(long, int, int, int, const float *const *, long, const float *const *, long, const float *const *, const float *const *, const int *,
                                    float *const *, float *const *, float *, hipStream_t);
 }
diff --git a/pointcloudpdf_amd/csrc/rowlin2_impl.h b/pointcloudpdf_amd/csrc/rowlin2_impl.h
--- a/pointcloudpdf_amd/csrc/rowlin2_impl.h
+++ b/pointcloudpdf_amd/csrc/rowlin2_impl.h
@@ -490,18 +490,18 @@
     int B, tiles_k, tiles, otiles, split, K, O;
 };
 void launch_slab_reduce(const RArgs &a, int ng, bool any_bias, hipStream_t s);
-template <int L>
-__global__ __launch_bounds__(64 * L) void k_slab_reduce(RArgs a) {
-    __shared__ float red[L][64];
-    const int e = threadIdx.x & 63, l = threadIdx.x >> 6, z = blockIdx.z;
-    const int ei = blockIdx.x * 64 + e;
-    const bool bias = (int)blockIdx.y >= a.tiles;
-    const int t = bias ? (int)blockIdx.y - a.tiles : (int)blockIdx.y;
+void launch_slab_reduce2(const RArgs &a0, bool bias0, const RArgs &a1, bool bias1, hipStream_t s);
+template <int L, bool WIDE>
+__device__ __forceinline__ void slab_reduce_block(const RArgs &a, int bx, int by, int z, float (*red)[64]) {
+    const int e = threadIdx.x & 63, l = threadIdx.x >> 6;
+    const int ei = bx * 64 + e;
+    const bool bias = by >= a.tiles;
+    const int t = bias ? by - a.tiles : by;
     const int len = bias ? a.B : a.B * a.B;
-    if (bias && (int)blockIdx.x * 64 >= len) return;
+    if (bias && bx * 64 >= len) return;
     const float *src = bias ? a.bslab + ((size_t)z * a.otiles + t) * a.split * a.B : a.slab + ((size_t)z * a.tiles + t) * a.split * (size_t)(a.B * a.B);
     float s = 0.f;
-    if (ei < len) {
+    if (ei < len && (!WIDE || l < L)) {
         int k = l;
         for (; k + 3 * L < a.split; k += 4 * L) {
             const float v0 = src[(size_t)k * len + ei], v1 = src[(size_t)(k + L) * len + ei];
@@ -523,6 +523,25 @@
         if (o < a.O && kk < a.K) a.dW[z][(size_t)o * a.K + kk] = s;
     }
 }
+template <int L>
+__global__ __launch_bounds__(64 * L) void k_slab_reduce(RArgs a) {
+    __shared__ float red[L][64];
+    slab_reduce_block<L, false>(a, (int)blockIdx.x, (int)blockIdx.y, (int)blockIdx.z, red);
+}
+static inline int slab_reduce_lanes(int split) { return split > 32 ? 16 : (split > 4 ? 4 : 1); }
+
+struct RArgs2 { RArgs a[2]; int L[2], gx[2], ysplit; };
+template <int LMAX>
+__global__ __launch_bounds__(64 * LMAX) void k_slab_reduce2(RArgs2 q) {
+    __shared__ float red[LMAX][64];
+    const int i = (int)blockIdx.y >= q.ysplit ? 1 : 0;
+    const int bx = (int)blockIdx.x, by = (int)blockIdx.y - (i ? q.ysplit : 0);
+    if (bx >= q.gx[i]) return;
+    const int L = q.L[i];
+    if (LMAX >= 16 && L == 16) slab_reduce_block<16, true>(q.a[i], bx, by, 0, red);
+    else if (LMAX >= 4 && L == 4) slab_reduce_block<4, true>(q.a[i], bx, by, 0, red);
+    else slab_reduce_block<1, true>(q.a[i], bx, by, 0, red);
+}
 
 #ifdef RL2_MAIN_TU
 void launch_slab_reduce(const RArgs &a, int ng, bool any_bias, hipStream_t s) {
@@ -530,6 +549,23 @@
     if (a.split > 32) k_slab_reduce<16><<<grid, 64 * 16, 0, s>>>(a);
     else if (a.split > 4) k_slab_reduce<4><<<grid, 64 * 4, 0, s>>>(a);
     else k_slab_reduce<1><<<grid, 64, 0, s>>>(a);
+}
+void launch_slab_reduce2(const RArgs &a0, bool bias0, const RArgs &a1, bool bias1, hipStream_t s) {
+    RArgs2 q;
+    q.a[0] = a0; q.a[1] = a1;
+    const bool bias[2] = {bias0, bias1};
+    int gy[2];
+    for (int i = 0; i < 2; ++i) {
+        q.L[i] = slab_reduce_lanes(q.a[i].split);
+        q.gx[i] = (q.a[i].B * q.a[i].B + 63) / 64;
+        gy[i] = q.a[i].tiles + (bias[i] ? q.a[i].otiles : 0);
+    }
+    q.ysplit = gy[0];
+    const dim3 grid((unsigned)std::max(q.gx[0], q.gx[1]), (unsigned)(gy[0] + gy[1]), 1u);
+    const int lmax = std::max(q.L[0], q.L[1]);
+    if (lmax == 16) k_slab_reduce2<16><<<grid, 64 * 16, 0, s>>>(q);
+    else if (lmax == 4) k_slab_reduce2<4><<<grid, 64 * 4, 0, s>>>(q);
+    else k_slab_reduce2<1><<<grid, 64, 0, s>>>(q);
 }
 #endif
 
@@ -673,7 +709,8 @@
 
 template <int MP>
 int try_wgrad_mp(long n, int k, int o, int ng, const float *const *g, long ldg, const float *x, long ldx, const float *scale,
-                 const float *shift, int relu, float *const *dw, float *const *db, float *ws, hipStream_t s, const float *roww, long rws) {
+                 const float *shift, int relu, float *const *dw, float *const *db, float *ws, hipStream_t s, const float *roww, long rws,
+                 RArgs *defer) {
     if (ng < 1 || ng > 3 || !ws) return 0;
     const WgPlan p = wg_plan(n, k, o, ng);
     const int vw = p.vw;
@@ -703,7 +740,8 @@
     RArgs r;
     r.slab = a.slab; r.bslab = a.bslab; r.B = b; r.tiles_k = k / b; r.tiles = (o / b) * (k / b); r.otiles = o / b; r.split = (int)p.split; r.K = k; r.O = o;
     for (int i = 0; i < WG_MAXG; ++i) { r.dW[i] = a.dW[i]; r.db[i] = a.db[i]; }
-    launch_slab_reduce(r, ng, any_bias, s);
+    if (defer) *defer = r;
+    else launch_slab_reduce(r, ng, any_bias, s);
     return 1;
 }
 
diff --git a/pointcloudpdf_amd/dense.py b/pointcloudpdf_amd/dense.py
--- a/pointcloudpdf_amd/dense.py
+++ b/pointcloudpdf_amd/dense.py
@@ -751,3 +751,90 @@
     if bn.training:
         bump_counters([bn.num_batches_tracked])
     return y
+
+
+class _TransitionUpFn(torch.autograd.Function):
+    @staticmethod
+    @_amp_fwd
+    def forward(ctx, bn1, bn2, idx, weight, x1, W1, b1, g1, be1, x2, W2, b2, g2, be2):
+        from . import _native
+
+        be = _be()
+        _rcd(x1, x2, W1, W2, idx, weight)
+        lib = be.lib
+        (n1, k1), (n2, k2), o = x1.shape, x2.shape, W1.shape[0]
+        e = lambda *shape: torch.empty(shape, dtype=torch.float32, device=x1.device)
+        z1, coef1, z2, coef2, out = e(n1, o), e(4 * o), e(n2, o), e(4 * o), e(n1, o)
+        part1, part2 = e(int(lib.pdf_rowlin_partial_floats(n1, o))), e(int(lib.pdf_rowlin_partial_floats(n2, o)))
+        order = _native.order_of(idx)
+        P = lambda t: None if t is None else t.data_ptr()
+        ptrs = [P(x1), P(W1), P(b1), P(g1), P(be1), P(bn1.running_mean), P(bn1.running_var),
+                P(x2), P(W2), P(b2), P(g2), P(be2), P(bn2.running_mean), P(bn2.running_var),
+                P(idx), P(weight), P(order), P(z1), P(coef1), P(part1), P(z2), P(coef2), P(part2), P(out)]
+        rc = lib.pdf_transition_up_forward(n1, k1, n2, k2, o, (c_void_p * len(ptrs))(*ptrs), 1, ctypes.c_float(bn1.eps), ctypes.c_float(bn1.momentum),
+                                           _mma(), be._stream())
+        if rc != 0:
+            raise RuntimeError(f"pdf_transition_up_forward failed with status {rc}")
+        ctx.save_for_backward(x1, z1, coef1, W1, x2, z2, coef2, W2, idx, weight)
+        ctx.has_bias = (b1 is not None, b2 is not None)
+        return out
+
+    @staticmethod
+    @_amp_bwd
+    def backward(ctx, g):
+        from . import _native
+
+        x1, z1, coef1, W1, x2, z2, coef2, W2, idx, weight = ctx.saved_tensors
+        be = _be()
+        lib = be.lib
+        (n1, k1), (n2, k2), o = x1.shape, x2.shape, W1.shape[0]
+        e = lambda *shape: torch.empty(shape, dtype=torch.float32, device=x1.device)
+        need1, need2 = ctx.needs_input_grad[4], ctx.needs_input_grad[9]
+        gx1 = e(n1, k1) if need1 else None
+        gx2 = e(n2, k2) if need2 else None
+        grads1, grads2 = e(o * k1 + 3 * o), e(o * k2 + 3 * o)
+        g2, gz1, gz2 = e(n2, o), e(n1, o), e(n2, o)
+        part1, part2 = e(int(lib.pdf_bn_partial_floats(n1, o))), e(int(lib.pdf_bn_partial_floats(n2, o)))
+        ws1, ws2 = be.wgrad_workspace(n1, k1, o, 1, x1.device), be.wgrad_workspace(n2, k2, o, 1, x1.device)
+        g = g.contiguous()
+        inv_off, inv_entry, entry_base = _native.inverse_table(idx, n2)
+        src_order = _native.src_order_of(idx, n2)
+        P = lambda t: None if t is None else t.data_ptr()
+        ptrs = [P(g), P(x1), P(z1), P(coef1), P(W1), P(x2), P(z2), P(coef2), P(W2), P(weight), P(inv_off), P(inv_entry), P(src_order),
+                P(gx1), P(gx2), P(grads1), P(grads2), P(g2), P(gz1), P(gz2), P(part1), P(part2), P(ws1), P(ws2)]
+        rc = lib.pdf_transition_up_backward(n1, k1, n2, k2, o, (c_void_p * len(ptrs))(*ptrs), int(entry_base), _mma(), be._stream())
+        if rc != 0:
+            raise RuntimeError(f"pdf_transition_up_backward failed with status {rc}")
+
+        def split(grads, k, has_bias):
+            ok = o * k
+            return grads[:ok].view(o, k), grads[ok:ok + o] if has_bias else None, grads[ok + 2 * o:ok + 3 * o], grads[ok + o:ok + 2 * o]
+
+        return (None, None, None, None, gx1, *split(grads1, k1, ctx.has_bias[0]), gx2, *split(grads2, k2, ctx.has_bias[1]))
+
+
+TUFUSED = True
+
+
+def tu_ok(lin1, bn1, lin2, bn2, x1, x2, idx, weight):
+    if not (TUFUSED and linbn_ok(lin1, bn1, x1) and linbn_ok(lin2, bn2, x2)):
+        return False
+    if not (bn1.training and bn2.training and bn1.eps == bn2.eps and bn1.momentum == bn2.momentum and lin1.out_features == lin2.out_features):
+        return False
+    if not (idx.is_cuda and idx.dtype == torch.int32 and idx.dim() == 2 and idx.shape[1] == 3 and idx.is_contiguous() and idx.shape[0] == x1.shape[0]
+            and weight.is_cuda and weight.dtype == torch.float32 and weight.shape == idx.shape and weight.is_contiguous()):
+        return False
+    if x1.shape[0] < 1 or x2.shape[0] < 1 or any(p.dtype != torch.float32 or not p.is_contiguous() for p in (lin1.weight, lin2.weight)):
+        return False
+    from . import _native
+
+    be = _be()
+    if _native.backend_for(x1) is not be or not getattr(be, "use_inverse", False):
+        return False
+    return bool(be.lib.pdf_transition_up_supported(lin1.in_features, lin2.in_features, lin1.out_features))
+
+
+def transition_up(lin1, bn1, lin2, bn2, x1, x2, idx, weight):
+    out = _TransitionUpFn.apply(bn1, bn2, idx, weight, x1, lin1.weight, lin1.bias, bn1.weight, bn1.bias, x2, lin2.weight, lin2.bias, bn2.weight, bn2.bias)
+    bump_counters([bn1.num_batches_tracked, bn2.num_batches_tracked])
+    return out
diff --git a/pointcloudpdf_amd/point_transformer.py b/pointcloudpdf_amd/point_transformer.py
--- a/pointcloudpdf_amd/point_transformer.py
+++ b/pointcloudpdf_amd/point_transformer.py
@@ -276,6 +276,20 @@
         ends = tag[0].offset_host(tag[1]) if tag is not None else [int(v) for v in o.detach().cpu().tolist()]
         return [ends[0]] + [ends[i] - ends[i - 1] for i in range(1, len(ends))]
 
+    def _join_fused(self, p1, x1, o1, p2, x2, o2):
+        l1, l2 = self.linear1, self.linear2
+        if not (dense.TUFUSED and len(l1) == 3 and len(l2) == 3 and x1.is_cuda and x1.dtype == torch.float32 and x2.dtype == torch.float32
+                and x1.dim() == 2 and x2.dim() == 2 and isinstance(l1[0], nn.Linear) and isinstance(l2[0], nn.Linear)
+                and isinstance(l1[2], nn.ReLU) and isinstance(l2[2], nn.ReLU) and p1.is_contiguous() and p2.is_contiguous()
+                and l1[1].training and l2[1].training and dense.linbn_ok(l1[0], l1[1], x1) and dense.linbn_ok(l2[0], l2[1], x2)):
+            return None
+        from .pointops import _ops
+
+        idx, weight = _ops._interp_tables(p2, p1, o2, o1, 3)
+        if not dense.tu_ok(l1[0], l1[1], l2[0], l2[1], x1, x2, idx, weight):
+            return None
+        return dense.transition_up(l1[0], l1[1], l2[0], l2[1], x1, x2, idx, weight)
+
     def forward(self, pxo1, pxo2=None):
         if pxo2 is None:
             p, x, o = pxo1
@@ -289,7 +303,9 @@
         else:
             p1, x1, o1 = pxo1
             p2, x2, o2 = pxo2
-            x = _seq(self.linear1, x1) + pointops.interpolation(p2, p1, _seq(self.linear2, x2), o2, o1)
+            x = self._join_fused(p1, x1, o1, p2, x2, o2)
+            if x is None:
+                x = _seq(self.linear1, x1) + pointops.interpolation(p2, p1, _seq(self.linear2, x2), o2, o1)
         return x
 
 
```

Result: faster. 14.11 million, median of 6 (+1.9%).
